# NSAPH-Projects/weather2alert

Hardware: AMD Instinct MI355X
Metric: env_steps_per_sec (higher is better)
Workload: dtype f32 tables, fp64 logit accumulation, f32 sigmoid/reward

## Files before the change

### include/w2a.h

```cpp
#ifndef W2A_H
#define W2A_H

#include <stddef.h>
#include <stdint.h>

#ifdef __cplusplus
extern "C" {
#endif

#define W2A_ABI_VERSION 18
#define W2A_ROW_FLOATS 32

enum {
  W2A_OK = 0,
  W2A_ERR_ARG = -1,
  W2A_ERR_SCHEMA = -2,
  W2A_ERR_HIP = -3,
  W2A_ERR_STATE = -4
};

enum {
  W2A_ST_BAD_EPISODE = 1,
  W2A_ST_BAD_ACTION = 2,
  W2A_ST_STEP_AFTER_DONE = 4,
// ... 88 lines not shown
typedef struct w2a_policy {
  int32_t kind;
  float p;
  int32_t obs_col;
  float threshold;
  int32_t obs_lag;
  int32_t require_budget;
  const uint8_t *table;
  int32_t table_R;
  uint64_t seed;
} w2a_policy;
int w2a_rollout(w2a_env *env, const w2a_policy *policy, int32_t n_steps, float *ret_out, int32_t *alerts_out,
                int32_t *attempts_over_budget, uint32_t *alert_mask, uint32_t *attempt_mask, int32_t mask_words,
                float *last_return, float *ret_snapshot, void *stream);
typedef struct w2a_linear_policy {
  const float *weight;
  const float *bias;
  const int32_t *group;
  int32_t n_groups;
  int32_t sample;
  int32_t require_budget;
  uint64_t seed;
} w2a_linear_policy;
int w2a_rollout_linear(w2a_env *env, const w2a_linear_policy *policy, int32_t n_steps, float *obs, float *ret_out,
                       int32_t *alerts_out, int32_t *attempts_over_budget, uint32_t *alert_mask, uint32_t *attempt_mask,
                       int32_t mask_words, float *last_return, float *ret_snapshot, void *stream);
enum { W2A_MLP_TANH = 0, W2A_MLP_RELU = 1 };
#define W2A_MLP_STRIDE(width, n_layers) \
  (W2A_ROW_FLOATS * (width) + (width) + ((n_layers) == 2 ? (width) * (width) + (width) : 0) + (width) + 4)
#define W2A_MLP_HEADS_STRIDE(width, n_layers) (W2A_MLP_STRIDE(width, n_layers) + (width))
typedef struct w2a_mlp_policy {
  const float *params;
  const int32_t *group;
  const int32_t *order;
  int32_t n_groups;
  int32_t n_layers;
  int32_t width;
  int32_t activation;
  int32_t sample;
  int32_t require_budget;
  uint64_t seed;
} w2a_mlp_policy;
int w2a_rollout_mlp(w2a_env *env, const w2a_mlp_policy *policy, int32_t n_steps, float *obs, float *ret_out,
                    int32_t *alerts_out, int32_t *attempts_over_budget, uint32_t *alert_mask, uint32_t *attempt_mask,
                    int32_t mask_words, float *last_return, float *ret_snapshot, void *stream);
enum { W2A_TRAJ_VALID = 1, W2A_TRAJ_TERMINATED = 2, W2A_TRAJ_ALERT = 4 };
typedef struct w2a_trajectory {
  float *obs;
  float *logit;
  float *reward;
  uint8_t *action;
  uint8_t *flags;
} w2a_trajectory;
int w2a_rollout_linear_record(w2a_env *env, const w2a_linear_policy *policy, int32_t n_steps, float *obs,
                              float *ret_out, int32_t *alerts_out, int32_t *attempts_over_budget, uint32_t *alert_mask,
                              uint32_t *attempt_mask, int32_t mask_words, float *last_return, float *ret_snapshot,
                              void *stream, const w2a_trajectory *traj);
int w2a_rollout_mlp_record(w2a_env *env, const w2a_mlp_policy *policy, int32_t n_steps, float *obs, float *ret_out,
                           int32_t *alerts_out, int32_t *attempts_over_budget, uint32_t *alert_mask,
                           uint32_t *attempt_mask, int32_t mask_words, float *last_return, float *ret_snapshot,
                           void *stream, const w2a_trajectory *traj);
int w2a_posterior_returns(w2a_env *env, const w2a_state_view *start, const uint32_t *alert_mask, int32_t mask_words,
                          int32_t n_steps, float *out, void *stream);
size_t w2a_hindsight_workspace_bytes(const w2a_env *env, int32_t n_steps, int32_t max_remaining, int32_t big_envs);
int w2a_hindsight_optimum(w2a_env *env, const w2a_state_view *start, int32_t n_steps, float *ret_out,
                          uint32_t *alert_mask, int32_t mask_words, int32_t *alerts_out, void *workspace,
                          size_t workspace_bytes, void *stream);
enum { W2A_PG_BASELINE_NONE = 0, W2A_PG_BASELINE_NO_ALERT = 1 };
size_t w2a_policy_gradient_workspace_bytes(int64_t num_envs, int32_t n_steps);
int w2a_policy_gradient_linear(w2a_env *env, const w2a_linear_policy *policy, int32_t baseline, int32_t n_steps,
                               const float *obs, float *grad, void *workspace, size_t workspace_bytes, void *stream);
size_t w2a_policy_gradient_mlp_workspace_bytes(int64_t num_envs, int32_t n_steps, int32_t n_groups, int32_t width,
                                               int32_t n_layers);
int w2a_policy_gradient_mlp(w2a_env *env, const w2a_mlp_policy *policy, int32_t baseline, int32_t n_steps,
                            const float *obs, float *grad, void *workspace, size_t workspace_bytes, void *stream);
int w2a_imitation_gradient_linear(w2a_env *env, const w2a_linear_policy *policy, const uint32_t *alert_mask,
                                  int32_t mask_words, const float *env_weight, int32_t n_steps, const float *obs,
                                  float *grad, float *loglik, int32_t *days, void *stream);
size_t w2a_imitation_gradient_mlp_workspace_bytes(int64_t num_envs, int32_t n_steps, int32_t n_groups, int32_t width,
                                                  int32_t n_layers);
int w2a_imitation_gradient_mlp(w2a_env *env, const w2a_mlp_policy *policy, const uint32_t *alert_mask,
                               int32_t mask_words, const float *env_weight, int32_t n_steps, const float *obs,
                               float *grad, float *loglik, int32_t *days, void *workspace, size_t workspace_bytes,
                               void *stream);
int w2a_imitation_gradient_linear_weighted(w2a_env *env, const w2a_linear_policy *policy, const uint32_t *alert_mask,
                                           int32_t mask_words, const float *env_weight, const float *day_weight,
                                           int32_t day_weight_days, int32_t n_steps, const float *obs, float *grad,
                                           float *loglik, int32_t *days, void *stream);
int w2a_imitation_gradient_mlp_weighted(w2a_env *env, const w2a_mlp_policy *policy, const uint32_t *alert_mask,
                                        int32_t mask_words, const float *env_weight, const float *day_weight,
                                        int32_t day_weight_days, int32_t n_steps, const float *obs, float *grad,
                                        float *loglik, int32_t *days, void *workspace, size_t workspace_bytes,
                                        void *stream);
int w2a_surrogate_gradient_linear(w2a_env *env, const w2a_linear_policy *policy, const uint32_t *alert_mask,
                                  int32_t mask_words, const float *env_weight, const float *advantage,
                                  int32_t advantage_days, const float *old_log_prob, int32_t old_log_prob_days,
                                  double clip, double entropy_coef, int32_t n_steps, const float *obs, float *grad,
                                  float *surrogate, int32_t *clipped_days, float *approx_kl, float *entropy,
                                  int32_t *days, float *log_prob, void *stream);
size_t w2a_surrogate_gradient_mlp_workspace_bytes(int64_t num_envs, int32_t n_steps, int32_t n_groups, int32_t width,
                                                  int32_t n_layers);
int w2a_surrogate_gradient_mlp(w2a_env *env, const w2a_mlp_policy *policy, const uint32_t *alert_mask,
                               int32_t mask_words, const float *env_weight, const float *advantage,
                               int32_t advantage_days, const float *old_log_prob, int32_t old_log_prob_days,
                               double clip, double entropy_coef, int32_t n_steps, const float *obs, float *grad,
                               float *surrogate, int32_t *clipped_days, float *approx_kl, float *entropy,
                               int32_t *days, float *log_prob, void *workspace, size_t workspace_bytes, void *stream);
size_t w2a_value_gradient_linear_workspace_bytes(int64_t num_envs, int32_t n_steps);
int w2a_value_gradient_linear(w2a_env *env, const w2a_linear_policy *value, const uint32_t *alert_mask,
                              int32_t mask_words, const float *env_weight, int32_t n_steps, const float *obs,
                              float *grad, float *sq_error, int32_t *days, float *ret, float *advantage,
                              void *workspace, size_t workspace_bytes, void *stream);
size_t w2a_value_gradient_mlp_workspace_bytes(int64_t num_envs, int32_t n_steps, int32_t n_groups, int32_t width,
                                              int32_t n_layers);
int w2a_value_gradient_mlp(w2a_env *env, const w2a_mlp_policy *value, const uint32_t *alert_mask, int32_t mask_words,
                           const float *env_weight, int32_t n_steps, const float *obs, float *grad, float *sq_error,
                           int32_t *days, float *ret, float *advantage, void *workspace, size_t workspace_bytes,
                           void *stream);
size_t w2a_value_gradient_linear_gae_workspace_bytes(int64_t num_envs, int32_t n_steps);
int w2a_value_gradient_linear_gae(w2a_env *env, const w2a_linear_policy *value, const uint32_t *alert_mask,
                                  int32_t mask_words, const float *env_weight, int32_t n_steps, const float *obs,
                                  float *grad, float *sq_error, int32_t *days, float *ret, float *advantage,
                                  double gamma, double lambda, int32_t bootstrap, float *value_target,
                                  const float *target, int32_t target_days, void *workspace, size_t workspace_bytes,
                                  void *stream);
size_t w2a_value_gradient_mlp_gae_workspace_bytes(int64_t num_envs, int32_t n_steps, int32_t n_groups, int32_t width,
                                                  int32_t n_layers);
int w2a_value_gradient_mlp_gae(w2a_env *env, const w2a_mlp_policy *value, const uint32_t *alert_mask,
                               int32_t mask_words, const float *env_weight, int32_t n_steps, const float *obs,
                               float *grad, float *sq_error, int32_t *days, float *ret, float *advantage, double gamma,
                               double lambda, int32_t bootstrap, float *value_target, const float *target,
                               int32_t target_days, void *workspace, size_t workspace_bytes, void *stream);
size_t w2a_rollout_order_workspace_bytes(int64_t num_envs, int64_t table_rows);
int w2a_rollout_order_attach(w2a_env *env, void *workspace, size_t workspace_bytes);
int w2a_rollout_order(w2a_env *env, void *workspace, size_t workspace_bytes, void *stream);

size_t w2a_rollout_mfma_workspace_bytes(int64_t num_envs, int64_t table_rows, int32_t S, int32_t n_samples);
int w2a_rollout_mfma_prepare(w2a_env *env, void *workspace, size_t workspace_bytes, void *stream);

int w2a_rollout_posterior_mean(w2a_env *env, const w2a_policy *policy, int32_t n_steps, float *ret_out,
                               int32_t *alerts_out, int32_t *attempts_over_budget, uint32_t *alert_mask,
                               uint32_t *attempt_mask, int32_t mask_words, float *last_return, float *ret_snapshot,
                               void *stream);

int w2a_policy_actions(w2a_env *env, const w2a_policy *policy, int32_t *actions, int32_t *alerts,
                       int32_t *attempts_over_budget, uint32_t *alert_mask, uint32_t *attempt_mask, int32_t mask_words,
                       void *stream);

int w2a_get_state(w2a_env *env, const w2a_state_view *view, void *stream);

enum { W2A_Q_LOCKSTEP = 6,
       W2A_Q_LOCKSTEP_DAY = 0, W2A_Q_PACKED_ELIGIBLE = 1, W2A_Q_PACKED_CURRENT = 2, W2A_Q_CANONICAL_CURRENT = 3,
       W2A_Q_LAST_ROLLOUT_KERNEL = 4 ,
       W2A_Q_LAST_STEP_KERNEL = 5     };
int w2a_query(w2a_env *env, int what);

int w2a_invalidate(w2a_env *env, void *stream);

int w2a_read_status(w2a_env *env, int32_t *status_out, void *stream);

int w2a_alert_gate(w2a_env *env, int32_t obs_col, float threshold, const float *thresholds, int32_t n_steps,
                   uint32_t *allowed_days, int32_t allowed_words, void *stream);
int w2a_rollout_linear_gated(w2a_env *env, const w2a_linear_policy *policy, int32_t n_steps, float *obs, float *ret_out,
                             int32_t *alerts_out, int32_t *attempts_over_budget, uint32_t *alert_mask,
                             uint32_t *attempt_mask, int32_t mask_words, float *last_return, float *ret_snapshot,
                             void *stream, const w2a_trajectory *traj, const uint32_t *allowed_days,
                             int32_t allowed_words);
int w2a_policy_gradient_linear_gated(w2a_env *env, const w2a_linear_policy *policy, int32_t baseline, int32_t n_steps,
                                     const float *obs, float *grad, void *workspace, size_t workspace_bytes,
                                     void *stream, const uint32_t *allowed_days, int32_t allowed_words);
int w2a_imitation_gradient_linear_gated(w2a_env *env, const w2a_linear_policy *policy, const uint32_t *alert_mask,
                                        int32_t mask_words, const float *env_weight, const float *day_weight,
                                        int32_t day_weight_days, int32_t n_steps, const float *obs, float *grad,
                                        float *loglik, int32_t *days, void *stream, const uint32_t *allowed_days,
                                        int32_t allowed_words);
int w2a_surrogate_gradient_linear_gated(w2a_env *env, const w2a_linear_policy *policy, const uint32_t *alert_mask,
                                        int32_t mask_words, const float *env_weight, const float *advantage,
                                        int32_t advantage_days, const float *old_log_prob, int32_t old_log_prob_days,
                                        double clip, double entropy_coef, int32_t n_steps, const float *obs,
                                        float *grad, float *surrogate, int32_t *clipped_days, float *approx_kl,
                                        float *entropy, int32_t *days, float *log_prob, void *stream,
                                        const uint32_t *allowed_days, int32_t allowed_words);
int w2a_rollout_mlp_gated(w2a_env *env, const w2a_mlp_policy *policy, int32_t n_steps, float *obs, float *ret_out,
                          int32_t *alerts_out, int32_t *attempts_over_budget, uint32_t *alert_mask,
                          uint32_t *attempt_mask, int32_t mask_words, float *last_return, float *ret_snapshot,
                          void *stream, const w2a_trajectory *traj, const uint32_t *allowed_days, int32_t allowed_words);
int w2a_policy_gradient_mlp_gated(w2a_env *env, const w2a_mlp_policy *policy, int32_t baseline, int32_t n_steps,
                                  const float *obs, float *grad, void *workspace, size_t workspace_bytes, void *stream,
                                  const uint32_t *allowed_days, int32_t allowed_words);
int w2a_imitation_gradient_mlp_gated(w2a_env *env, const w2a_mlp_policy *policy, const uint32_t *alert_mask,
                                     int32_t mask_words, const float *env_weight, const float *day_weight,
                                     int32_t day_weight_days, int32_t n_steps, const float *obs, float *grad,
                                     float *loglik, int32_t *days, void *workspace, size_t workspace_bytes,
                                     void *stream, const uint32_t *allowed_days, int32_t allowed_words);
int w2a_surrogate_gradient_mlp_gated(w2a_env *env, const w2a_mlp_policy *policy, const uint32_t *alert_mask,
                                     int32_t mask_words, const float *env_weight, const float *advantage,
                                     int32_t advantage_days, const float *old_log_prob, int32_t old_log_prob_days,
                                     double clip, double entropy_coef, int32_t n_steps, const float *obs, float *grad,
                                     float *surrogate, int32_t *clipped_days, float *approx_kl, float *entropy,
                                     int32_t *days, float *log_prob, void *workspace, size_t workspace_bytes,
                                     void *stream, const uint32_t *allowed_days, int32_t allowed_words);
int w2a_hindsight_optimum_gated(w2a_env *env, const w2a_state_view *start, int32_t n_steps, float *ret_out,
                                uint32_t *alert_mask, int32_t mask_words, int32_t *alerts_out, void *workspace,
                                size_t workspace_bytes, void *stream, const uint32_t *allowed_days,
                                int32_t allowed_words);

int w2a_fisher_vector_product_linear(w2a_env *env, const w2a_linear_policy *policy, const float *vec_weight,
                                     const float *vec_bias, const uint32_t *alert_mask, int32_t mask_words,
                                     const float *env_weight, int32_t n_steps, const float *obs, float *fv,
                                     float *quadratic, int32_t *days, void *stream, const uint32_t *allowed_days,
                                     int32_t allowed_words);
size_t w2a_fisher_vector_product_mlp_workspace_bytes(int64_t num_envs, int32_t n_steps, int32_t n_groups, int32_t width,
                                                     int32_t n_layers);
int w2a_fisher_vector_product_mlp(w2a_env *env, const w2a_mlp_policy *policy, const float *vector,
                                  const uint32_t *alert_mask, int32_t mask_words, const float *env_weight,
                                  int32_t n_steps, const float *obs, float *fv, float *quadratic, int32_t *days,
                                  void *workspace, size_t workspace_bytes, void *stream, const uint32_t *allowed_days,
                                  int32_t allowed_words);
enum { W2A_Q_LOSS_SQUARED = 0, W2A_Q_LOSS_HUBER = 1 };
size_t w2a_q_gradient_mlp_workspace_bytes(int64_t num_envs, int32_t n_steps, int32_t n_groups, int32_t width,
                                          int32_t n_layers);
int w2a_q_gradient_mlp(w2a_env *env, const w2a_mlp_policy *q, const w2a_mlp_policy *target_net,
                       const uint32_t *alert_mask, int32_t mask_words, const float *env_weight, int32_t n_steps,
                       const float *obs, float *grad, float *loss_out, int32_t *days, float *ret, double gamma,
                       int32_t double_q, int32_t loss, double huber_delta, int32_t bootstrap, float *td_error,
                       float *td_target, void *workspace, size_t workspace_bytes, void *stream);

#ifdef __cplusplus
}
#endif
#endif
```

### weather2alert_amd/_ffi.py

```python
from __future__ import annotations

import ctypes as C
import os

from . import build as _build

ROW_FLOATS = 32

OK = 0
ST_BAD_EPISODE, ST_BAD_ACTION, ST_STEP_AFTER_DONE, ST_STALE_GRAPH = 1, 2, 4, 8
ACT_I32, ACT_I64, ACT_U8 = 0, 1, 2
STEP_AUTORESET, STEP_NO_OBS, STEP_CLASSIC, STEP_REWARD_GIVEN, STEP_WIDE, STEP_SKIP_FINISHED, STEP_UNPACKED, STEP_NEXT_STEP, STEP_NO_CAPTURE = 1, 2, 8, 16, 32, 64, 128, 256, 512
S64_MIN_ENVS = 131072
ABI_VERSION = 18
FIX_BITS = {"alert_2wks": 1, "lag": 2, "penalty": 4, "obs": 8, "augment": 16}
BUDGET_FIXED, BUDGET_LESS_THAN, BUDGET_CENTERED = 0, 1, 2

SYMBOLS = [
    "w2a_abi_version", "w2a_last_error", "w2a_state_bytes", "w2a_create", "w2a_destroy", "w2a_reset",
    "w2a_reset_device_rng", "w2a_set_autoreset", "w2a_step", "w2a_get_state", "w2a_read_status",
    "w2a_sort_workspace_bytes", "w2a_sort_episodes", "w2a_reset_device_rng_sorted", "w2a_observe", "w2a_rollout", "w2a_rollout_order_workspace_bytes", "w2a_rollout_order_attach", "w2a_rollout_order", "w2a_rollout_posterior_mean", "w2a_policy_actions", "w2a_set_semantics",
    "w2a_group_workspace_bytes", "w2a_group_by_column", "w2a_posterior_mean_reward", "w2a_set_posterior_kernel", "w2a_invalidate", "w2a_query", "w2a_rollout_mfma_workspace_bytes", "w2a_rollout_mfma_prepare",
    "w2a_rollout_linear", "w2a_rollout_mlp", "w2a_rollout_linear_record", "w2a_rollout_mlp_record",
    "w2a_posterior_returns", "w2a_hindsight_workspace_bytes", "w2a_hindsight_optimum",
    "w2a_policy_gradient_workspace_bytes", "w2a_policy_gradient_linear",
    "w2a_policy_gradient_mlp_workspace_bytes", "w2a_policy_gradient_mlp",
    "w2a_imitation_gradient_linear", "w2a_imitation_gradient_mlp_workspace_bytes", "w2a_imitation_gradient_mlp",
    "w2a_imitation_gradient_linear_weighted", "w2a_imitation_gradient_mlp_weighted",
    "w2a_value_gradient_linear_workspace_bytes", "w2a_value_gradient_linear",
    "w2a_value_gradient_mlp_workspace_bytes", "w2a_value_gradient_mlp",
    "w2a_value_gradient_linear_gae_workspace_bytes", "w2a_value_gradient_linear_gae",
    "w2a_value_gradient_mlp_gae_workspace_bytes", "w2a_value_gradient_mlp_gae",
    "w2a_surrogate_gradient_linear", "w2a_surrogate_gradient_mlp_workspace_bytes", "w2a_surrogate_gradient_mlp",
    "w2a_alert_gate", "w2a_rollout_linear_gated", "w2a_policy_gradient_linear_gated",
    "w2a_imitation_gradient_linear_gated", "w2a_surrogate_gradient_linear_gated", "w2a_hindsight_optimum_gated",
    "w2a_rollout_mlp_gated", "w2a_policy_gradient_mlp_gated", "w2a_imitation_gradient_mlp_gated",
    "w2a_surrogate_gradient_mlp_gated",
    "w2a_fisher_vector_product_linear", "w2a_fisher_vector_product_mlp_workspace_bytes",
    "w2a_fisher_vector_product_mlp",
    "w2a_q_gradient_mlp_workspace_bytes", "w2a_q_gradient_mlp",
]
Q_LOCKSTEP_DAY, Q_PACKED_ELIGIBLE, Q_PACKED_CURRENT, Q_CANONICAL_CURRENT, Q_LAST_ROLLOUT_KERNEL, Q_LAST_STEP_KERNEL, Q_LOCKSTEP = 0, 1, 2, 3, 4, 5, 6
ROLLOUT_KERNELS = {0: "k_rollout", 1: "k_rollout64", 2: "k_rollout_mfma", 3: "k_rollout_linear", 4: "k_rollout_mlp"}
PM_KERNELS = {"vector": 0, "matrix": 1, "matrix_i8": 2}
POLICY_KINDS = {"never": 0, "always": 1, "bernoulli": 2, "threshold": 3, "table": 4}


class Policy(C.Structure):
    _fields_ = [("kind", C.c_int32), ("p", C.c_float), ("obs_col", C.c_int32), ("threshold", C.c_float),
                ("obs_lag", C.c_int32), ("require_budget", C.c_int32), ("table", C.c_void_p),
                ("table_R", C.c_int32), ("seed", C.c_uint64)]


class LinearPolicy(C.Structure):
    _fields_ = [("weight", C.c_void_p), ("bias", C.c_void_p), ("group", C.c_void_p), ("n_groups", C.c_int32),
                ("sample", C.c_int32), ("require_budget", C.c_int32), ("seed", C.c_uint64)]


class MlpPolicy(C.Structure):
    _fields_ = [("params", C.c_void_p), ("group", C.c_void_p), ("order", C.c_void_p), ("n_groups", C.c_int32),
                ("n_layers", C.c_int32), ("width", C.c_int32), ("activation", C.c_int32), ("sample", C.c_int32),
                ("require_budget", C.c_int32), ("seed", C.c_uint64)]


MLP_ACTIVATIONS = {"tanh": 0, "relu": 1}


class Trajectory(C.Structure):
    _fields_ = [("obs", C.c_void_p), ("logit", C.c_void_p), ("reward", C.c_void_p), ("action", C.c_void_p),
                ("flags", C.c_void_p)]


TRAJ_VALID, TRAJ_TERMINATED, TRAJ_ALERT = 1, 2, 4
Q_LOSSES = {"squared": 0, "huber": 1}
PG_BASELINES = {"none": 0, "no_alert": 1}


class Tables(C.Structure):
    _fields_ = [
        ("X", C.c_void_p), ("n_days", C.c_void_p), ("B0", C.c_void_p), ("W", C.c_void_p),
        ("fips_to_weather", C.c_void_p), ("sim_cnt", C.c_void_p),
        ("T", C.c_int32), ("S_w", C.c_int32), ("Y", C.c_int32), ("S", C.c_int32), ("n_samples", C.c_int32),
        ("n_obs", C.c_int32), ("obs_slot", C.c_int32 * ROW_FLOATS), ("slot_heat_qi", C.c_int32),
        ("sim_ptr", C.c_void_p), ("sim_idx", C.c_void_p), ("slot_alerts_2wks", C.c_int32),
        ("gate_bits", C.c_void_p), ("gate_words", C.c_int32),
    ]


STATE_FIELDS = ["t", "used", "streak", "hist14", "last_actual", "at_budget", "budget", "n_days", "county_w",
                "year_i", "coef_col", "sample", "sticky_budget", "episode_no", "finished", "episode_return"]


class StateView(C.Structure):
    _fields_ = [(k, C.c_void_p) for k in STATE_FIELDS]


class W2AError(RuntimeError):
    pass


_lib = None


def lib_path() -> str:
    return os.environ.get("W2A_LIB") or _build.LIB


def load(build_if_missing: bool = True):
    global _lib
    if _lib is not None:
        return _lib
    path = lib_path()
    if build_if_missing and not os.environ.get("W2A_LIB") and _build.needs_build():
        try:
            _build.build_lib()
        except Exception as e:
            raise W2AError(f"libw2a.so is out of date (or missing) and could not be rebuilt: {e}") from e
    if not os.path.exists(path):
        raise W2AError(f"{path} not found: run `python -m weather2alert_amd.build` (there is no CPU fallback)")
    lib = C.CDLL(path)
    vp, i32, i64, u64 = C.c_void_p, C.c_int32, C.c_int64, C.c_uint64
    lib.w2a_abi_version.restype = C.c_int
    lib.w2a_abi_version.argtypes = []
    lib.w2a_last_error.restype = C.c_char_p
    lib.w2a_last_error.argtypes = []
    lib.w2a_state_bytes.restype = C.c_size_t
    lib.w2a_state_bytes.argtypes = [i64]
    lib.w2a_create.restype = C.c_int
    lib.w2a_create.argtypes = [C.POINTER(Tables), i64, i64, vp, C.c_size_t, vp, C.POINTER(vp)]
    lib.w2a_destroy.restype = None
    lib.w2a_destroy.argtypes = [vp]
    lib.w2a_reset.restype = C.c_int
    lib.w2a_reset.argtypes = [vp, vp, vp, vp, vp, vp, vp, vp, vp]
    lib.w2a_reset_device_rng.restype = C.c_int
    lib.w2a_reset_device_rng.argtypes = [vp, u64, i32, C.c_int, i32, C.c_int, C.c_int, C.c_int, vp, vp, vp]
    lib.w2a_set_autoreset.restype = C.c_int
    lib.w2a_set_autoreset.argtypes = [vp, u64, i32, C.c_int, i32, C.c_int, C.c_int]
    lib.w2a_step.restype = C.c_int
    lib.w2a_step.argtypes = [vp, vp, C.c_int, vp, vp, vp, vp, C.c_int, vp]
    lib.w2a_get_state.restype = C.c_int
    lib.w2a_get_state.argtypes = [vp, C.POINTER(StateView), vp]
    lib.w2a_read_status.restype = C.c_int
    lib.w2a_read_status.argtypes = [vp, C.POINTER(i32), vp]
    lib.w2a_sort_workspace_bytes.restype = C.c_size_t
    lib.w2a_sort_workspace_bytes.argtypes = [i64]
    lib.w2a_sort_episodes.restype = C.c_int
    lib.w2a_sort_episodes.argtypes = [vp, vp, C.c_size_t, vp]
    lib.w2a_reset_device_rng_sorted.restype = C.c_int
    lib.w2a_reset_device_rng_sorted.argtypes = [vp, u64, i32, C.c_int, i32, C.c_int, C.c_int, C.c_int, vp, vp, C.c_size_t, vp]
    lib.w2a_group_workspace_bytes.restype = C.c_size_t
    lib.w2a_group_workspace_bytes.argtypes = [i64, C.c_int32, C.c_int32]
    lib.w2a_group_by_column.restype = C.c_int
    lib.w2a_group_by_column.argtypes = [vp, vp, C.c_size_t, vp]
    lib.w2a_posterior_mean_reward.restype = C.c_int
    lib.w2a_posterior_mean_reward.argtypes = [vp, vp, C.c_int, vp, vp]
    lib.w2a_set_posterior_kernel.restype = C.c_int
    lib.w2a_set_posterior_kernel.argtypes = [vp, C.c_int]
    lib.w2a_rollout_mfma_workspace_bytes.restype = C.c_size_t
    lib.w2a_rollout_mfma_workspace_bytes.argtypes = [i64, i64, i32, i32]
    lib.w2a_rollout_mfma_prepare.restype = C.c_int
    lib.w2a_rollout_mfma_prepare.argtypes = [vp, vp, C.c_size_t, vp]
    lib.w2a_query.restype = C.c_int
    lib.w2a_query.argtypes = [vp, C.c_int]
    lib.w2a_invalidate.restype = C.c_int
    lib.w2a_invalidate.argtypes = [vp, vp]
    lib.w2a_observe.restype = C.c_int
    lib.w2a_observe.argtypes = [vp, vp, vp]
    lib.w2a_set_semantics.restype = C.c_int
    lib.w2a_set_semantics.argtypes = [vp, C.c_uint32]
    lib.w2a_rollout.restype = C.c_int
    lib.w2a_rollout.argtypes = [vp, C.POINTER(Policy), i32, vp, vp, vp, vp, vp, i32, vp, vp, vp]
    lib.w2a_rollout_order_workspace_bytes.restype = C.c_size_t
    lib.w2a_rollout_order_workspace_bytes.argtypes = [i64, i64]
    lib.w2a_rollout_order.restype = C.c_int
    lib.w2a_rollout_order.argtypes = [vp, vp, C.c_size_t, vp]
    lib.w2a_rollout_order_attach.restype = C.c_int
    lib.w2a_rollout_order_attach.argtypes = [vp, vp, C.c_size_t]
    lib.w2a_rollout_posterior_mean.restype = C.c_int
    lib.w2a_rollout_posterior_mean.argtypes = [vp, C.POINTER(Policy), i32, vp, vp, vp, vp, vp, i32, vp, vp, vp]
    lib.w2a_rollout_linear.restype = C.c_int
    lib.w2a_rollout_linear.argtypes = [vp, C.POINTER(LinearPolicy), i32, vp, vp, vp, vp, vp, vp, i32, vp, vp, vp]
    lib.w2a_rollout_mlp.restype = C.c_int
    lib.w2a_rollout_mlp.argtypes = [vp, C.POINTER(MlpPolicy), i32, vp, vp, vp, vp, vp, vp, i32, vp, vp, vp]
    lib.w2a_rollout_linear_record.restype = C.c_int
    lib.w2a_rollout_linear_record.argtypes = lib.w2a_rollout_linear.argtypes + [C.POINTER(Trajectory)]
    lib.w2a_rollout_mlp_record.restype = C.c_int
    lib.w2a_rollout_mlp_record.argtypes = lib.w2a_rollout_mlp.argtypes + [C.POINTER(Trajectory)]
    lib.w2a_posterior_returns.restype = C.c_int
    lib.w2a_posterior_returns.argtypes = [vp, C.POINTER(StateView), vp, i32, i32, vp, vp]
    lib.w2a_hindsight_workspace_bytes.restype = C.c_size_t
    lib.w2a_hindsight_workspace_bytes.argtypes = [vp, i32, i32, i32]
    lib.w2a_hindsight_optimum.restype = C.c_int
    lib.w2a_hindsight_optimum.argtypes = [vp, C.POINTER(StateView), i32, vp, vp, i32, vp, vp, C.c_size_t, vp]
    lib.w2a_policy_gradient_workspace_bytes.restype = C.c_size_t
    lib.w2a_policy_gradient_workspace_bytes.argtypes = [i64, i32]
    lib.w2a_policy_gradient_linear.restype = C.c_int
    lib.w2a_policy_gradient_linear.argtypes = [vp, C.POINTER(LinearPolicy), i32, i32, vp, vp, vp, C.c_size_t, vp]
    lib.w2a_policy_gradient_mlp_workspace_bytes.restype = C.c_size_t
    lib.w2a_policy_gradient_mlp_workspace_bytes.argtypes = [i64, i32, i32, i32, i32]
    lib.w2a_policy_gradient_mlp.restype = C.c_int
    lib.w2a_policy_gradient_mlp.argtypes = [vp, C.POINTER(MlpPolicy), i32, i32, vp, vp, vp, C.c_size_t, vp]
    lib.w2a_imitation_gradient_linear.restype = C.c_int
    lib.w2a_imitation_gradient_linear.argtypes = [vp, C.POINTER(LinearPolicy), vp, i32, vp, i32, vp, vp, vp, vp, vp]
    lib.w2a_imitation_gradient_mlp_workspace_bytes.restype = C.c_size_t
    lib.w2a_imitation_gradient_mlp_workspace_bytes.argtypes = [i64, i32, i32, i32, i32]
    lib.w2a_imitation_gradient_mlp.restype = C.c_int
    lib.w2a_imitation_gradient_mlp.argtypes = [vp, C.POINTER(MlpPolicy), vp, i32, vp, i32, vp, vp, vp, vp, vp, C.c_size_t, vp]
    lib.w2a_imitation_gradient_linear_weighted.restype = C.c_int
    lib.w2a_imitation_gradient_linear_weighted.argtypes = [vp, C.POINTER(LinearPolicy), vp, i32, vp, vp, i32, i32, vp, vp, vp, vp, vp]
    lib.w2a_imitation_gradient_mlp_weighted.restype = C.c_int
    lib.w2a_imitation_gradient_mlp_weighted.argtypes = [vp, C.POINTER(MlpPolicy), vp, i32, vp, vp, i32, i32, vp, vp, vp, vp, vp, C.c_size_t, vp]
    lib.w2a_value_gradient_linear_workspace_bytes.restype = C.c_size_t
    lib.w2a_value_gradient_linear_workspace_bytes.argtypes = [i64, i32]
    lib.w2a_value_gradient_linear.restype = C.c_int
    lib.w2a_value_gradient_linear.argtypes = [vp, C.POINTER(LinearPolicy), vp, i32, vp, i32, vp, vp, vp, vp, vp, vp, vp, C.c_size_t, vp]
    lib.w2a_value_gradient_mlp_workspace_bytes.restype = C.c_size_t
    lib.w2a_value_gradient_mlp_workspace_bytes.argtypes = [i64, i32, i32, i32, i32]
    lib.w2a_value_gradient_mlp.restype = C.c_int
    lib.w2a_value_gradient_mlp.argtypes = [vp, C.POINTER(MlpPolicy), vp, i32, vp, i32, vp, vp, vp, vp, vp, vp, vp, C.c_size_t, vp]
    gae = [C.c_double, C.c_double, i32, vp, vp, i32]
    lib.w2a_value_gradient_linear_gae_workspace_bytes.restype = C.c_size_t
    lib.w2a_value_gradient_linear_gae_workspace_bytes.argtypes = [i64, i32]
    lib.w2a_value_gradient_linear_gae.restype = C.c_int
    lib.w2a_value_gradient_linear_gae.argtypes = [vp, C.POINTER(LinearPolicy), vp, i32, vp, i32, vp, vp, vp, vp, vp, vp, *gae, vp, C.c_size_t, vp]
    lib.w2a_value_gradient_mlp_gae_workspace_bytes.restype = C.c_size_t
    lib.w2a_value_gradient_mlp_gae_workspace_bytes.argtypes = [i64, i32, i32, i32, i32]
    lib.w2a_value_gradient_mlp_gae.restype = C.c_int
    lib.w2a_value_gradient_mlp_gae.argtypes = [vp, C.POINTER(MlpPolicy), vp, i32, vp, i32, vp, vp, vp, vp, vp, vp, *gae, vp, C.c_size_t, vp]
    lib.w2a_surrogate_gradient_linear.restype = C.c_int
    lib.w2a_surrogate_gradient_linear.argtypes = [vp, C.POINTER(LinearPolicy), vp, i32, vp, vp, i32, vp, i32, C.c_double,
                                                  C.c_double, i32, vp, vp, vp, vp, vp, vp, vp, vp, vp]
    lib.w2a_surrogate_gradient_mlp_workspace_bytes.restype = C.c_size_t
    lib.w2a_surrogate_gradient_mlp_workspace_bytes.argtypes = [i64, i32, i32, i32, i32]
    lib.w2a_surrogate_gradient_mlp.restype = C.c_int
    lib.w2a_surrogate_gradient_mlp.argtypes = [vp, C.POINTER(MlpPolicy), vp, i32, vp, vp, i32, vp, i32, C.c_double,
                                               C.c_double, i32, vp, vp, vp, vp, vp, vp, vp, vp, vp, C.c_size_t, vp]
    gate = [vp, i32]
    lib.w2a_alert_gate.restype = C.c_int
    lib.w2a_alert_gate.argtypes = [vp, i32, C.c_float, vp, i32, vp, i32, vp]
    lib.w2a_rollout_linear_gated.restype = C.c_int
    lib.w2a_rollout_linear_gated.argtypes = lib.w2a_rollout_linear.argtypes + [C.POINTER(Trajectory)] + gate
    lib.w2a_policy_gradient_linear_gated.restype = C.c_int
    lib.w2a_policy_gradient_linear_gated.argtypes = lib.w2a_policy_gradient_linear.argtypes + gate
    lib.w2a_imitation_gradient_linear_gated.restype = C.c_int
    lib.w2a_imitation_gradient_linear_gated.argtypes = lib.w2a_imitation_gradient_linear_weighted.argtypes + gate
    lib.w2a_surrogate_gradient_linear_gated.restype = C.c_int
    lib.w2a_surrogate_gradient_linear_gated.argtypes = lib.w2a_surrogate_gradient_linear.argtypes + gate
    lib.w2a_rollout_mlp_gated.restype = C.c_int
    lib.w2a_rollout_mlp_gated.argtypes = lib.w2a_rollout_mlp.argtypes + [C.POINTER(Trajectory)] + gate
    lib.w2a_policy_gradient_mlp_gated.restype = C.c_int
    lib.w2a_policy_gradient_mlp_gated.argtypes = lib.w2a_policy_gradient_mlp.argtypes + gate
    lib.w2a_imitation_gradient_mlp_gated.restype = C.c_int
    lib.w2a_imitation_gradient_mlp_gated.argtypes = lib.w2a_imitation_gradient_mlp_weighted.argtypes + gate
    lib.w2a_surrogate_gradient_mlp_gated.restype = C.c_int
    lib.w2a_surrogate_gradient_mlp_gated.argtypes = lib.w2a_surrogate_gradient_mlp.argtypes + gate
    lib.w2a_hindsight_optimum_gated.restype = C.c_int
    lib.w2a_hindsight_optimum_gated.argtypes = lib.w2a_hindsight_optimum.argtypes + gate
    lib.w2a_fisher_vector_product_linear.restype = C.c_int
    lib.w2a_fisher_vector_product_linear.argtypes = [vp, C.POINTER(LinearPolicy), vp, vp, vp, i32, vp, i32, vp, vp, vp,
                                                     vp, vp] + gate
    lib.w2a_fisher_vector_product_mlp_workspace_bytes.restype = C.c_size_t
    lib.w2a_fisher_vector_product_mlp_workspace_bytes.argtypes = [i64, i32, i32, i32, i32]
    lib.w2a_fisher_vector_product_mlp.restype = C.c_int
    lib.w2a_fisher_vector_product_mlp.argtypes = [vp, C.POINTER(MlpPolicy), vp, vp, i32, vp, i32, vp, vp, vp, vp, vp,
                                                  C.c_size_t, vp] + gate
    lib.w2a_q_gradient_mlp_workspace_bytes.restype = C.c_size_t
    lib.w2a_q_gradient_mlp_workspace_bytes.argtypes = [i64, i32, i32, i32, i32]
    lib.w2a_q_gradient_mlp.restype = C.c_int
    lib.w2a_q_gradient_mlp.argtypes = [vp, C.POINTER(MlpPolicy), C.POINTER(MlpPolicy), vp, i32, vp, i32, vp, vp, vp, vp,
                                       vp, C.c_double, i32, i32, C.c_double, i32, vp, vp, vp, C.c_size_t, vp]
    lib.w2a_policy_actions.restype = C.c_int
    lib.w2a_policy_actions.argtypes = [vp, C.POINTER(Policy), vp, vp, vp, vp, vp, i32, vp]
    if lib.w2a_abi_version() != ABI_VERSION:
        raise W2AError(f"libw2a.so ABI {lib.w2a_abi_version()} != {ABI_VERSION}; rebuild")
    _lib = lib
    return lib


def check(rc: int, what: str = ""):
    if rc != OK:
        msg = load().w2a_last_error().decode("utf-8", "replace")
        raise W2AError(f"{what} failed ({rc}): {msg}")
```

### weather2alert_amd/build.py

```python
from __future__ import annotations

import os
import shutil
import subprocess
import sys

PKG = os.path.dirname(os.path.abspath(__file__))
ROOT = os.path.dirname(PKG)
SRC = os.path.join(PKG, "csrc", "w2a_kernels.hip")
INC = os.path.join(ROOT, "include")
LIB_DIR = os.path.join(PKG, "_lib")
LIB = os.path.join(LIB_DIR, "libw2a.so")


def hipcc_path() -> str:
    for c in (os.environ.get("HIPCC"), shutil.which("hipcc"), "/opt/rocm/bin/hipcc"):
        if c and os.path.exists(c):
            return c
    raise RuntimeError("hipcc not found (need the ROCm toolchain to build libw2a.so)")


HASH_FILE = LIB + ".srchash"


def _dep_files() -> list:
    csrc = os.path.dirname(SRC)
    return sorted(os.path.join(csrc, f) for f in os.listdir(csrc) if f.endswith((".hip", ".hip.h", ".h"))) + \
        [os.path.join(INC, "w2a.h")]


def build_hash() -> str:
    import hashlib

    h = hashlib.sha256()
    for path in _dep_files():
        h.update(os.path.basename(path).encode())
        h.update(open(path, "rb").read())
    h.update(os.environ.get("W2A_CXXFLAGS", "").encode())
    return h.hexdigest()


def needs_build() -> bool:
    if not os.path.exists(LIB):
        return True
    if os.path.exists(HASH_FILE):
        try:
            return open(HASH_FILE).read().strip() != build_hash()
        except OSError:
            return True
    m = os.path.getmtime(LIB)
    return any(os.path.getmtime(d) > m for d in _dep_files())


STEP_SOURCES = ("w2a_common.hip.h", "w2a_step.hip.h", "w2a_step64.hip.h", "w2a_step_dispatch.hip.h", "w2a_bookkeeping.h")


def source_sha(files: tuple = STEP_SOURCES) -> str:
    import hashlib

    h = hashlib.sha256()
    csrc = os.path.dirname(SRC)
    for path in [os.path.join(csrc, f) for f in sorted(files)]:
        h.update(os.path.basename(path).encode())
        h.update(open(path, "rb").read())
    return h.hexdigest()[:16]


def build_lib(force: bool = False, verbose: bool = False) -> str:
    if not force and not needs_build():
        return LIB
    os.makedirs(LIB_DIR, exist_ok=True)
    tmp = f"{LIB}.{os.getpid()}.tmp"
    src_hash = build_hash()
    cmd = [hipcc_path(), "--offload-arch=gfx950", "-O3", "-std=c++17", "-fPIC", "-shared", f"-I{INC}", SRC,
           "-o", tmp]
    cmd += os.environ.get("W2A_CXXFLAGS", "").split()
    if verbose:
        cmd.insert(1, "-Rpass-analysis=kernel-resource-usage")
        print(" ".join(cmd))
    r = subprocess.run(cmd, capture_output=True, text=True)
    if r.returncode != 0:
        raise RuntimeError(f"hipcc failed ({r.returncode}):\n{r.stdout}\n{r.stderr}")
    if verbose:
        print(r.stderr)
    try:
        os.remove(HASH_FILE)
    except OSError:
        pass
    os.replace(tmp, LIB)
    htmp = f"{HASH_FILE}.{os.getpid()}.tmp"
    with open(htmp, "w") as f:
        f.write(src_hash + "\n")
    os.replace(htmp, HASH_FILE)
    return LIB


PROBE_SRC = os.path.join(ROOT, "tools", "fabric_probe.hip")
PROBE_LIB = os.path.join(LIB_DIR, "libw2a_probe.so")
PROBE_FLAGS = ("-DPROBE_LIB", "-DPROBE_F64", "-DPROBE_DEP", "-DPROBE_DAYS", "-DPROBE_RANDOM_DATA", "-DPROBE_INPLACE")


def build_probe_lib(force: bool = False, packed: bool = True) -> str:
    out = PROBE_LIB if packed else PROBE_LIB.replace(".so", "_unpacked.so")
    if not force and os.path.exists(out) and os.path.getmtime(out) >= os.path.getmtime(PROBE_SRC):
        return out
    os.makedirs(LIB_DIR, exist_ok=True)
    tmp = f"{out}.{os.getpid()}.tmp"
    cmd = [hipcc_path(), "--offload-arch=gfx950", "-O3", "-std=c++17", "-fPIC", "-shared", *PROBE_FLAGS,
           *(["-DPROBE_PACKED"] if packed else []), PROBE_SRC, "-o", tmp]
    r = subprocess.run(cmd, capture_output=True, text=True)
    if r.returncode != 0:
        raise RuntimeError(f"hipcc failed on the probe library ({r.returncode}):\n{r.stdout}\n{r.stderr}")
    os.replace(tmp, out)
    return out


if __name__ == "__main__":
    print(build_lib(force="--force" in sys.argv, verbose=True))
    print(build_probe_lib(force="--force" in sys.argv))
    print(build_probe_lib(force="--force" in sys.argv, packed=False))
```

### weather2alert_amd/csrc/w2a_common.hip.h

```cpp
#ifndef W2A_COMMON_HIP_H
#define W2A_COMMON_HIP_H

#include "w2a_bookkeeping.h"

#ifndef LANES
#define LANES 4
#endif
#define ROWF 32
#define QUADS (ROWF / 4 / LANES)
#ifndef BLOCK
#define BLOCK 256
#endif
#define ENVS_PER_BLOCK (BLOCK / LANES)
#define ENVS_PER_WAVE (64 / LANES)
#define HDR_BYTES 256
#ifndef W2A_NT_OBS
#define W2A_NT_OBS 1
#endif
#ifndef W2A_NT_W
#define W2A_NT_W 0
#endif
#ifndef W2A_XCD_SWIZZLE
#define W2A_XCD_SWIZZLE 1
#endif
__device__ __forceinline__ uint32_t logical_block(uint32_t b, uint32_t per_xcd) {
#if W2A_XCD_SWIZZLE
  return (b & 7u) * per_xcd + (b >> 3);
#else
  return b;
#endif
}
typedef float v4f __attribute__((ext_vector_type(4)));
typedef uint32_t v4u __attribute__((ext_vector_type(4)));
__device__ __forceinline__ float4 ld_w(const float4 *p) {
#if W2A_NT_W
  v4f v = __builtin_nontemporal_load(reinterpret_cast<const v4f *>(p));
  return make_float4(v.x, v.y, v.z, v.w);
#else
  return *p;
#endif
}
#define RT_QUAD 6
#define GATE_QUAD 7

struct u3 { uint32_t a, b, c; };
struct StateArrays {
  uint4 *cold;
  u3 *hot3;
  u3 *stepc;
  uint2 *pk_hot;
  uint2 *pk_c;
  uint32_t *pk_day;
};
#define W2A_PK_DAY_POISON 0xFFFFFFFFu
#define PK_BUDGET_ESCAPE 0xFFFFu
__device__ __forceinline__ uint32_t pk_budget16(uint32_t budget) { return budget < PK_BUDGET_ESCAPE ? budget : PK_BUDGET_ESCAPE; }
#define PK_USED(w) ((w) & 255u)
#define PK_STREAK(w) (((w) >> 8) & 255u)
#define PK_HIST(w) (((w) >> 16) & 0x3FFFu)
#define PK_FIN(w) (((w) >> 30) & 1u)
__device__ __forceinline__ uint32_t pk_pack_hot(uint32_t used, uint32_t streak, uint32_t hist, uint32_t fin) {
  return (used & 255u) | ((streak & 255u) << 8) | ((hist & 0x3FFFu) << 16) | (fin << 30);
}
__device__ __forceinline__ void load_step_state(const StateArrays &s, uint32_t e, uint4 &cold, uint4 &hot) {
  const u3 h = s.hot3[e];
  const u3 c = s.stepc[e];
  hot = make_uint4(h.a, h.b, h.c, c.a);
  cold = make_uint4(c.b, c.c, 0u, 0u);
}
__device__ __forceinline__ uint4 load_cold(const StateArrays &s, uint32_t e) { return s.cold[e]; }
__device__ __forceinline__ void store_hot(const StateArrays &s, uint32_t e, const uint4 hot) {
  u3 h; h.a = hot.x; h.b = hot.y; h.c = hot.z;
  s.hot3[e] = h;
}
__device__ __forceinline__ void store_episode(const StateArrays &s, uint32_t e, const uint4 cold, const uint4 hot) {
  s.cold[e] = cold;
  u3 c; c.a = hot.w; c.b = cold.x; c.c = cold.y;
  s.stepc[e] = c;
  store_hot(s, e, hot);
}
#define D0_T(d) ((d) & 1023u)
#define D0_USED(d) (((d) >> 10) & 1023u)
#define D0_STREAK(d) (((d) >> 20) & 1023u)
#define D0_LAST(d) (((d) >> 30) & 1u)
#define D0_ATB(d) (((d) >> 31) & 1u)
#define D1_HIST(d) ((d) & 0x3FFFu)
#define D1_NDAYS(d) (((d) >> 16) & 1023u)
#define D1_FIN(d) (((d) >> 31) & 1u)

__device__ __forceinline__ uint32_t pack_d0(uint32_t t, uint32_t used, uint32_t streak, uint32_t last, uint32_t atb) {
  return (t & 1023u) | ((used > 1023u ? 1023u : used) << 10) | ((streak > 1023u ? 1023u : streak) << 20) |
         (last << 30) | (atb << 31);
}
__device__ __forceinline__ uint32_t pack_d1(uint32_t hist, uint32_t ndays, uint32_t fin) {
  return (hist & 0x3FFFu) | ((ndays & 1023u) << 16) | (fin << 31);
}

struct DevTables {
  const float4 *X;
  const int32_t *n_days;
  const int32_t *B0;
  const float4 *W;
  const int32_t *fips_to_weather;
  const int32_t *sim_cnt;
  const uint32_t *gate_bits;
  int32_t gate_words;
  const int32_t *sim_ptr;
  const int32_t *sim_idx;
  int32_t T, S_w, Y, S, n_samples, n_obs;
  int32_t slot_hist2w;
  uint32_t fixes;
};
__device__ __forceinline__ void set_comp(float4 *x, int idx, float v) {
#pragma unroll
  for (int q = 0; q < QUADS; ++q) {
    if (idx == 4 * q) x[q].x = v;
    if (idx == 4 * q + 1) x[q].y = v;
    if (idx == 4 * q + 2) x[q].z = v;
    if (idx == 4 * q + 3) x[q].w = v;
  }
}
#define SAMPLE_BITS 12
#define PACK_W(coef_col, sample) (((uint32_t)(coef_col) << SAMPLE_BITS) | (uint32_t)(sample))
#define W_COL(y) ((y) >> SAMPLE_BITS)
#define W_SAMPLE(y) ((y) & ((1u << SAMPLE_BITS) - 1u))

struct ResetCfg {
  uint64_t seed;
  int32_t location;
  int32_t augment;
  int32_t budget_kw;
  int32_t sample_mode;
  int32_t sticky;
};

struct w2a_env {
  DevTables tb;
  int64_t n;
  int64_t gid0;
  const int32_t *slot_obs;
  StateArrays st;
  int32_t *status;
  ResetCfg autoreset;
  int has_autoreset;
  int32_t obs_slot_host[ROWF];
  const uint32_t *perm;
  uint4 *prep;
  const uint32_t *inv;
  const double *wd;
  const uint4 *tiles;
  const uint32_t *n_tiles;
  const uint4 *tiles_i8;
  const uint32_t *n_tiles_i8;
  const uint32_t *wq;
  const float *wscale;
  const uint32_t *colflag;
  const float *xs;
  const void *xmax_ws;
  void *order_ws;
  uint32_t *order_cnt, *order_rank, *order_start, *order_tile_start;
  const void *rm_ws;
  const uint4 *rm_tiles;
  const uint32_t *rm_n_tiles;
  const uint32_t *rm_wq;
  const float *rm_xs;
  const uint32_t *order;
  W2aBook bk;
  int pm_kernel;
  int w_tail_used;
  uint32_t s64_launches;
};

static thread_local char g_err[512] = "";
static int fail(int code, const char *fmt, const char *a = "") {
  snprintf(g_err, sizeof(g_err), fmt, a);
  return code;
}

__device__ __forceinline__ uint64_t w2a_mix64(uint64_t z) {
  z ^= z >> 30;
  z *= 0xBF58476D1CE4E5B9ull;
  z ^= z >> 27;
  z *= 0x94D049BB133111EBull;
  z ^= z >> 31;
  return z;
}
__device__ __forceinline__ uint64_t rng_stream(uint64_t seed, uint64_t gid, uint64_t episode) {
  uint64_t h = w2a_mix64(seed + 0x9E3779B97F4A7C15ull * (gid + 1));
  return w2a_mix64(h ^ (episode * 0xBF58476D1CE4E5B9ull + 0x94D049BB133111EBull));
}
__device__ __forceinline__ uint32_t rng_bounded(uint64_t stream, uint32_t slot, uint32_t n) {
  uint64_t u = w2a_mix64(stream + (uint64_t)(slot + 1) * 0x9E3779B97F4A7C15ull) >> 32;
  return (uint32_t)((u * (uint64_t)n) >> 32);
}

template <int CTRL>
__device__ __forceinline__ double dpp_f64(double v) {
  int lo = __double2loint(v), hi = __double2hiint(v);
  lo = __builtin_amdgcn_update_dpp(0, lo, CTRL, 0xF, 0xF, true);
  hi = __builtin_amdgcn_update_dpp(0, hi, CTRL, 0xF, 0xF, true);
  return __hiloint2double(hi, lo);
}
__device__ __forceinline__ double group_sum(double v) {
  if (LANES >= 2) v += dpp_f64<0xB1>(v);
  if (LANES >= 4) v += dpp_f64<0x4E>(v);
  if (LANES >= 8) v += dpp_f64<0x141>(v);
  return v;
}

__device__ __forceinline__ float sigmoid_f32(float z) {
  float e = __expf(-z);
  return __builtin_amdgcn_rcpf(1.0f + e);
}

__device__ __forceinline__ float reward_from_logits(double zb, double ze, uint32_t actual) {
  const float base = sigmoid_f32((float)zb);
  const float eff = sigmoid_f32((float)ze);
  return -(1000.0f / 152.0f) * base * (1.0f - eff * (float)actual);
}

struct Episode {
  uint32_t ep_row, ep_w, ndays;
  int32_t budget, sticky;
  uint32_t bad;
};

__device__ __forceinline__ Episode draw_episode(const DevTables &tb, const ResetCfg &rc, uint64_t gid,
                                                uint32_t episode_no, int32_t sticky_in) {
  Episode e;
  uint64_t st = rng_stream(rc.seed, gid, episode_no);
  uint32_t bad = 0;
  uint32_t county = rc.location < 0 ? rng_bounded(st, 0, (uint32_t)tb.S) : (uint32_t)rc.location;
  if (county >= (uint32_t)tb.S) { county = 0; bad = 1; }
  uint32_t coef_col = county;
  if (rc.augment) {
    int32_t ns = tb.sim_cnt[county];
    if (ns <= 0) { bad = 1; ns = 1; }
    coef_col = rng_bounded(st, 1, (uint32_t)ns);
    if ((tb.fixes & W2A_FIX_AUGMENT) && tb.sim_idx) {
      if (!bad) county = (uint32_t)tb.sim_idx[tb.sim_ptr[county] + (int32_t)coef_col];
      if (county >= (uint32_t)tb.S) { county = 0; bad = 1; }
      coef_col = county;
    }
  }
  uint32_t year_i = rng_bounded(st, 2, (uint32_t)tb.Y);
  uint32_t sample = rng_bounded(st, 3, (uint32_t)tb.n_samples);
  int32_t cw = tb.fips_to_weather[county];
  if (cw < 0) { cw = 0; bad = 1; }
  e.ep_row = (uint32_t)cw * (uint32_t)tb.Y + year_i;
  e.ep_w = PACK_W(coef_col, sample);
  int32_t nd = tb.n_days[e.ep_row];
  if (nd <= 0) { bad = 1; nd = 1; }
  e.ndays = (uint32_t)nd;
  int32_t b = (rc.sticky && sticky_in >= 0) ? sticky_in : (rc.budget_kw < 0 ? tb.B0[e.ep_row] : rc.budget_kw);
  if (b < 0) b = 0;
  if (rc.sample_mode == W2A_BUDGET_LESS_THAN) {
    b = (int32_t)rng_bounded(st, 4, (uint32_t)b + 1u);
  } else if (rc.sample_mode == W2A_BUDGET_CENTERED) {
    int32_t lo = (int32_t)(0.5 * (double)b), hi = (int32_t)(1.5 * (double)b + 1.0);
    b = lo + (int32_t)rng_bounded(st, 4, (uint32_t)(hi - lo));
  }
  e.budget = b;
  e.sticky = rc.sticky ? b : -1;
  e.bad = bad;
  return e;
}

__device__ __forceinline__ void store_obs_tile(void *__restrict__ obs_any, float *tile, int64_t wave_env0, int64_t n,
                                               int n_obs, int lane, int grp, const float4 *x, const int4 *so,
                                               bool write_me) {
  float *obs = reinterpret_cast<float *>(obs_any);
  const int base = grp * n_obs;
  const int trash = ENVS_PER_WAVE * n_obs + (lane & 15);
#pragma unroll
  for (int q = 0; q < QUADS; ++q) {
    tile[so[q].x >= 0 ? base + so[q].x : trash] = x[q].x;
    tile[so[q].y >= 0 ? base + so[q].y : trash] = x[q].y;
    tile[so[q].z >= 0 ? base + so[q].z : trash] = x[q].z;
    tile[so[q].w >= 0 ? base + so[q].w : trash] = x[q].w;
  }
  __builtin_amdgcn_fence(__ATOMIC_RELEASE, "wavefront");
  __builtin_amdgcn_wave_barrier();
  __builtin_amdgcn_fence(__ATOMIC_ACQUIRE, "wavefront");
  const bool full = (wave_env0 + ENVS_PER_WAVE <= n);
  const bool all_write = __all(write_me || (wave_env0 + grp >= n));
  float *dst = obs + wave_env0 * n_obs;
  if (full && all_write) {
    const int chunks = (ENVS_PER_WAVE * n_obs) >> 2;
#pragma unroll
    for (int c0 = 0; c0 < (ENVS_PER_WAVE * ROWF) / 4; c0 += 64) {
      const int c = c0 + lane;
      if (c < chunks) {
        v4f v = reinterpret_cast<const v4f *>(tile)[c];
#if W2A_NT_OBS
        __builtin_nontemporal_store(v, reinterpret_cast<v4f *>(dst) + c);
#else
        reinterpret_cast<v4f *>(dst)[c] = v;
#endif
      }
    }
  } else {
    const int total = ENVS_PER_WAVE * n_obs;
    const unsigned long long wm = __ballot(write_me);
    for (int i = lane; i < total; i += 64) {
      int g = i / n_obs;
      bool w = (wm >> (g * LANES)) & 1ull;
      if (w && wave_env0 + g < n) dst[i] = tile[i];
    }
  }
  __builtin_amdgcn_wave_barrier();
}

#endif
```

### weather2alert_amd/csrc/w2a_kernels.hip

```cpp

#include <hip/hip_runtime.h>
#include <hipcub/hipcub.hpp>
#include <math.h>
#include <stdint.h>
#include <stdio.h>
#include <string.h>
#include <type_traits>

#include "w2a.h"

#include "w2a_common.hip.h"
#include "w2a_step.hip.h"
#include "w2a_step64.hip.h"
#include "w2a_posterior.hip.h"
#include "w2a_posterior_i8.hip.h"
#include "w2a_reset.hip.h"
#include "w2a_rollout.hip.h"
#include "w2a_rollout_linear.hip.h"
#include "w2a_rollout_mlp.hip.h"
#include "w2a_rollout_i8.hip.h"
#include "w2a_rollout_mfma.hip.h"
#include "w2a_posterior_returns.hip.h"
#include "w2a_policy_gradient.hip.h"
#include "w2a_policy_gradient_mlp.hip.h"
#include "w2a_imitation.hip.h"
#include "w2a_surrogate.hip.h"
#include "w2a_fisher.hip.h"
#include "w2a_value.hip.h"
#include "w2a_gae.hip.h"
#include "w2a_qlearn.hip.h"
#include "w2a_hindsight.hip.h"
#include "w2a_gate.hip.h"
#include "w2a_sort.hip.h"

#define HIP_TRY(expr)                                                   \
  do {                                                                  \
    hipError_t _e = (expr);                                             \
    if (_e != hipSuccess) return fail(W2A_ERR_HIP, #expr ": %s", hipGetErrorString(_e)); \
  } while (0)

template <int KIND>
static void launch_pm_rollout_kind(bool masks, unsigned grid, hipStream_t s, const PmRolloutArgs &a) {
  if (masks) hipLaunchKernelGGL((k_pm_rollout<7, KIND, true>), dim3(grid), dim3(PMV_THREADS), 0, s, a);
  else hipLaunchKernelGGL((k_pm_rollout<7, KIND, false>), dim3(grid), dim3(PMV_THREADS), 0, s, a);
}
static void launch_pm_rollout(int kind, bool masks, unsigned grid, hipStream_t s, const PmRolloutArgs &a) {
  switch (kind) {
    case W2A_POLICY_ALWAYS: launch_pm_rollout_kind<W2A_POLICY_ALWAYS>(masks, grid, s, a); break;
    case W2A_POLICY_BERNOULLI: launch_pm_rollout_kind<W2A_POLICY_BERNOULLI>(masks, grid, s, a); break;
    case W2A_POLICY_THRESHOLD: launch_pm_rollout_kind<W2A_POLICY_THRESHOLD>(masks, grid, s, a); break;
    case W2A_POLICY_TABLE: launch_pm_rollout_kind<W2A_POLICY_TABLE>(masks, grid, s, a); break;
    default: launch_pm_rollout_kind<W2A_POLICY_NEVER>(masks, grid, s, a); break;
  }
}

#ifndef W2A_ROLLOUT_MFMA
#define W2A_ROLLOUT_MFMA 1
#endif
#ifndef W2A_ROLLOUT_WIDE
#define W2A_ROLLOUT_WIDE 1
#endif
template <int KIND>
static void launch_rollout_kind(bool masks, bool fixes, unsigned grid, hipStream_t s, const RolloutArgs &a) {
  if (W2A_ROLLOUT_WIDE && a.order) {
    const unsigned g64 = (unsigned)((((a.n + BLOCK - 1) / BLOCK) + 7) / 8 * 8);
    if (masks && fixes) hipLaunchKernelGGL((k_rollout64<KIND, true, true>), dim3(g64), dim3(BLOCK), 0, s, a);
    else if (masks) hipLaunchKernelGGL((k_rollout64<KIND, true, false>), dim3(g64), dim3(BLOCK), 0, s, a);
    else if (fixes) hipLaunchKernelGGL((k_rollout64<KIND, false, true>), dim3(g64), dim3(BLOCK), 0, s, a);
    else hipLaunchKernelGGL((k_rollout64<KIND, false, false>), dim3(g64), dim3(BLOCK), 0, s, a);
    return;
  }
  if (masks && fixes) hipLaunchKernelGGL((k_rollout<KIND, true, true>), dim3(grid), dim3(BLOCK), 0, s, a);
  else if (masks) hipLaunchKernelGGL((k_rollout<KIND, true, false>), dim3(grid), dim3(BLOCK), 0, s, a);
  else if (fixes) hipLaunchKernelGGL((k_rollout<KIND, false, true>), dim3(grid), dim3(BLOCK), 0, s, a);
  else hipLaunchKernelGGL((k_rollout<KIND, false, false>), dim3(grid), dim3(BLOCK), 0, s, a);
}
static void launch_rollout(int kind, bool masks, bool fixes, unsigned grid, hipStream_t s, const RolloutArgs &a) {
  switch (kind) {
    case W2A_POLICY_ALWAYS: launch_rollout_kind<W2A_POLICY_ALWAYS>(masks, fixes, grid, s, a); break;
    case W2A_POLICY_BERNOULLI: launch_rollout_kind<W2A_POLICY_BERNOULLI>(masks, fixes, grid, s, a); break;
    case W2A_POLICY_THRESHOLD: launch_rollout_kind<W2A_POLICY_THRESHOLD>(masks, fixes, grid, s, a); break;
    case W2A_POLICY_TABLE: launch_rollout_kind<W2A_POLICY_TABLE>(masks, fixes, grid, s, a); break;
    default: launch_rollout_kind<W2A_POLICY_NEVER>(masks, fixes, grid, s, a); break;
  }
}

template <int KIND>
static void launch_rollout_mfma_kind(bool masks, unsigned grid, hipStream_t s, const RmArgs &ra) {
  if (masks) hipLaunchKernelGGL((k_rollout_mfma<KIND, true>), dim3(grid), dim3(64 * RM_WAVES), 0, s, ra);
  else hipLaunchKernelGGL((k_rollout_mfma<KIND, false>), dim3(grid), dim3(64 * RM_WAVES), 0, s, ra);
}
static void launch_rollout_mfma(int kind, bool masks, unsigned grid, hipStream_t s, const RmArgs &ra) {
  switch (kind) {
    case W2A_POLICY_ALWAYS: launch_rollout_mfma_kind<W2A_POLICY_ALWAYS>(masks, grid, s, ra); break;
    case W2A_POLICY_BERNOULLI: launch_rollout_mfma_kind<W2A_POLICY_BERNOULLI>(masks, grid, s, ra); break;
    case W2A_POLICY_THRESHOLD: launch_rollout_mfma_kind<W2A_POLICY_THRESHOLD>(masks, grid, s, ra); break;
    case W2A_POLICY_TABLE: launch_rollout_mfma_kind<W2A_POLICY_TABLE>(masks, grid, s, ra); break;
    default: launch_rollout_mfma_kind<W2A_POLICY_NEVER>(masks, grid, s, ra); break;
  }
}

extern "C" {

int w2a_abi_version(void) { return W2A_ABI_VERSION; }
const char *w2a_last_error(void) { return g_err; }

static size_t align256(size_t x) { return (x + 255) & ~(size_t)255; }

size_t w2a_state_bytes(int64_t num_envs) {
  if (num_envs <= 0) return 0;
  const size_t n = (size_t)num_envs;
  return HDR_BYTES + align256(16 * n) + 2 * align256(12 * n) + 2 * align256(8 * n) + align256(4 * ((n + 63) / 64));
}

struct HipDev {
  w2a_env *env;
  hipStream_t s;
  void pack_state() {
    hipLaunchKernelGGL(k_pack_state, dim3((unsigned)((env->n + 255) / 256)), dim3(256), 0, s, env->st, env->n);
  }
  void unpack_state(int32_t n_days) {
    hipLaunchKernelGGL(k_unpack_state, dim3((unsigned)((env->n + 255) / 256)), dim3(256), 0, s, env->st, env->n, n_days);
  }
  void poison_mirror() {
    const int64_t tiles = (env->n + 63) / 64;
    hipLaunchKernelGGL(k_poison_mirror, dim3((unsigned)((tiles + 255) / 256)), dim3(256), 0, s, env->st, env->n);
  }
};
static void end_call(w2a_env *env, hipStream_t s) {
  HipDev d{env, s};
  bk_end_call(env->bk, d);
}
static bool stream_is_capturing(hipStream_t s) {
  hipStreamCaptureStatus cs = hipStreamCaptureStatusNone;
  if (s && hipStreamIsCapturing(s, &cs) == hipSuccess) return cs != hipStreamCaptureStatusNone;
  (void)hipGetLastError();
  return false;
}
#define REFUSE_WHILE_CAPTURING(who, stream)                                                                            \
  do {                                                                                                                 \
    if (stream_is_capturing((hipStream_t)(stream)))                                                                    \
      return fail(W2A_ERR_STATE, who ": the stream is recording a hipGraph; only w2a_step can be recorded (episode "    \
                                     "boundaries inside a graph: W2A_STEP_AUTORESET)");                                \
  } while (0)
static bool ensure_canonical(w2a_env *env, hipStream_t s, const char *who) {
  if (!env->bk.canon_valid && stream_is_capturing(s)) {
    fail(W2A_ERR_STATE, "%s: the state is in its packed lock-step form and a conversion cannot be recorded into a hipGraph", who);
    return false;
  }
  HipDev d{env, s};
  bk_ensure_canonical(env->bk, d);
  return true;
}
__global__ void k_table_scan(const int32_t *n_days, int32_t rows, int32_t *out) {
  const int i = blockIdx.x * blockDim.x + threadIdx.x;
  if (i >= rows) return;
  atomicMin(&out[0], n_days[i]);
  atomicMax(&out[1], n_days[i]);
}

int w2a_create(const w2a_tables *t, int64_t num_envs, int64_t env_gid0, void *state, size_t state_bytes,
               int32_t *status, w2a_env **out) {
  if (!t || !state || !status || !out) return fail(W2A_ERR_ARG, "w2a_create: NULL argument");
  if (num_envs <= 0 || env_gid0 < 0) return fail(W2A_ERR_ARG, "w2a_create: num_envs must be > 0 and env_gid0 >= 0");
  if (!t->X || !t->n_days || !t->B0 || !t->W || !t->fips_to_weather || !t->sim_cnt)
    return fail(W2A_ERR_ARG, "w2a_create: NULL table pointer");
  if (t->T <= 0 || t->T > 1023 || t->S_w <= 0 || t->Y <= 0 || t->S <= 0 || t->n_samples <= 0)
    return fail(W2A_ERR_SCHEMA, "w2a_create: table dims out of range (need 0 < T <= 1023, positive S_w, Y, S, n_samples)");
  if ((int64_t)t->S_w * t->Y > 0x7FFFFFFFll / 2 || (int64_t)t->S * t->n_samples > 0x7FFFFFFFll / 2 ||
      (int64_t)t->T * t->S_w * t->Y > 0x7FFFFFFFll)
    return fail(W2A_ERR_SCHEMA, "w2a_create: table too large for 32-bit row indices");
  if ((int64_t)t->T * t->S_w * t->Y * (ROWF / 4) > 0x7FFFFFFFll || (int64_t)t->S * t->n_samples * (2 * ROWF / 4) > 0x7FFFFFFFll ||
      num_envs > (1ll << 27))
    return fail(W2A_ERR_SCHEMA, "w2a_create: tables / env count exceed the 32-bit offset range of the kernels");
  if (t->n_samples > (1 << SAMPLE_BITS) || t->S >= (1 << (32 - SAMPLE_BITS)))
    return fail(W2A_ERR_SCHEMA, "w2a_create: need n_samples <= 4096 and S < 2^20");
  if (t->n_obs <= 0 || t->n_obs > W2A_ROW_FLOATS - 1)
    return fail(W2A_ERR_SCHEMA, "w2a_create: n_obs must be in 1..31 (the observation tile keeps one scratch column)");
  if (state_bytes < w2a_state_bytes(num_envs)) return fail(W2A_ERR_STATE, "w2a_create: state buffer too small");
  if (((uintptr_t)state & 255) || ((uintptr_t)t->X & 15) || ((uintptr_t)t->W & 15))
    return fail(W2A_ERR_STATE, "w2a_create: state must be 256-B aligned, X and W 16-B aligned");
  int32_t slot_obs[ROWF];
  for (int i = 0; i < ROWF; ++i) slot_obs[i] = -1;
  for (int j = 0; j < t->n_obs; ++j) {
    int s = t->obs_slot[j];
    if (s < 0 || s >= ROWF || slot_obs[s] != -1) return fail(W2A_ERR_SCHEMA, "w2a_create: obs_slot is not an injective map into 0..31");
    slot_obs[s] = j;
  }
  w2a_env *h = new w2a_env();
  h->tb.X = reinterpret_cast<const float4 *>(t->X);
  h->tb.n_days = t->n_days;
  h->tb.B0 = t->B0;
  h->tb.W = reinterpret_cast<const float4 *>(t->W);
  h->tb.fips_to_weather = t->fips_to_weather;
  h->tb.sim_cnt = t->sim_cnt;
  h->tb.sim_ptr = t->sim_ptr;
  h->tb.sim_idx = t->sim_idx;
  h->tb.slot_hist2w = t->slot_alerts_2wks;
  h->tb.gate_bits = t->gate_bits;
  h->tb.gate_words = t->gate_words;
  if (t->gate_bits && (int64_t)t->gate_words * 32 < (int64_t)t->S_w * t->Y) {
    delete h;
    return fail(W2A_ERR_SCHEMA, "w2a_create: gate_words * 32 must cover S_w * Y rows");
  }
  h->tb.fixes = 0;
  h->tb.T = t->T; h->tb.S_w = t->S_w; h->tb.Y = t->Y; h->tb.S = t->S; h->tb.n_samples = t->n_samples;
  h->tb.n_obs = t->n_obs;
  h->n = num_envs;
  h->gid0 = env_gid0;
  h->slot_obs = reinterpret_cast<const int32_t *>(state);
  h->st.cold = reinterpret_cast<uint4 *>((char *)state + HDR_BYTES);
  h->st.hot3 = reinterpret_cast<u3 *>((char *)h->st.cold + align256(16 * (size_t)num_envs));
  h->st.stepc = reinterpret_cast<u3 *>((char *)h->st.hot3 + align256(12 * (size_t)num_envs));
  h->st.pk_hot = reinterpret_cast<uint2 *>((char *)h->st.stepc + align256(12 * (size_t)num_envs));
  h->st.pk_c = reinterpret_cast<uint2 *>((char *)h->st.pk_hot + align256(8 * (size_t)num_envs));
  h->st.pk_day = reinterpret_cast<uint32_t *>((char *)h->st.pk_c + align256(8 * (size_t)num_envs));
  bk_init(h->bk, t->T <= 255 && t->S < 65536 && t->n_samples <= 1024 && (int64_t)t->S_w * t->Y < (1 << 22), -1);
  h->status = status;
  h->has_autoreset = 0;
  h->perm = nullptr;
  h->order = nullptr;
  h->prep = nullptr;
  h->pm_kernel = W2A_PM_VECTOR;
  h->xmax_ws = nullptr;
  h->order_ws = nullptr; h->order_cnt = h->order_rank = h->order_start = h->order_tile_start = nullptr; h->rm_ws = nullptr;
  for (int j = 0; j < ROWF; ++j) h->obs_slot_host[j] = j < t->n_obs ? t->obs_slot[j] : -1;
  hipError_t e1 = hipMemcpy(state, slot_obs, sizeof(slot_obs), hipMemcpyHostToDevice);
  hipError_t e2 = hipMemset(status, 0, sizeof(int32_t));
  if (e1 != hipSuccess || e2 != hipSuccess) { delete h; return fail(W2A_ERR_HIP, "w2a_create: header upload failed: %s", hipGetErrorString(e1 != hipSuccess ? e1 : e2)); }
  int64_t blocks = (num_envs + 255) / 256;
  hipLaunchKernelGGL(k_init_state, dim3((unsigned)blocks), dim3(256), 0, 0, h->st, num_envs);
  hipError_t e0 = hipGetLastError();
  if (e0 != hipSuccess) { delete h; return fail(W2A_ERR_HIP, "w2a_create: k_init_state launch failed: %s", hipGetErrorString(e0)); }
  int32_t *scan_flag = reinterpret_cast<int32_t *>(state) + ROWF;
  const int64_t w_rows = (int64_t)t->S * t->n_samples * 2;
  hipError_t e4 = hipMemset(scan_flag, 0, sizeof(int32_t));
  hipLaunchKernelGGL(k_scan_tail_slots, dim3((unsigned)((w_rows + 255) / 256)), dim3(256), 0, 0, h->tb.W, w_rows, scan_flag);
  hipError_t e3 = hipDeviceSynchronize();
  int32_t tail_used = 1;
  if (e3 == hipSuccess && e4 == hipSuccess) e3 = hipMemcpy(&tail_used, scan_flag, sizeof(int32_t), hipMemcpyDeviceToHost);
  if (e3 != hipSuccess || e4 != hipSuccess) { delete h; return fail(W2A_ERR_HIP, "w2a_create: init kernels failed: %s", hipGetErrorString(e3 != hipSuccess ? e3 : e4)); }
  h->w_tail_used = tail_used;
  {
    int32_t scan[2] = {0x7FFFFFFF, 0};
    int32_t *d_scan = reinterpret_cast<int32_t *>(state) + ROWF + 1;
    hipError_t e5 = hipMemcpy(d_scan, scan, sizeof(scan), hipMemcpyHostToDevice);
    const int32_t rows = t->S_w * t->Y;
    hipLaunchKernelGGL(k_table_scan, dim3((unsigned)((rows + 255) / 256)), dim3(256), 0, 0, t->n_days, rows, d_scan);
    if (e5 == hipSuccess) e5 = hipMemcpy(scan, d_scan, sizeof(scan), hipMemcpyDeviceToHost);
    if (e5 != hipSuccess) { delete h; return fail(W2A_ERR_HIP, "w2a_create: table scan failed: %s", hipGetErrorString(e5)); }
    h->bk.uni_nd = (scan[0] == scan[1] && scan[0] > 0) ? scan[0] : -1;
  }
  *out = h;
  return W2A_OK;
}

void w2a_destroy(w2a_env *env) { delete env; }

static unsigned grid_for(int64_t n) {
  int64_t tiles = (n + ENVS_PER_BLOCK - 1) / ENVS_PER_BLOCK;
  return (unsigned)(((tiles + 7) / 8) * 8);
}

static int launch_reset(w2a_env *env, ResetArgs &a, void *stream) {
  if (a.obs && ((uintptr_t)a.obs & 15)) return fail(W2A_ERR_ARG, "reset: obs must be 16-B aligned");
  REFUSE_WHILE_CAPTURING("reset / observe", stream);
  const W2aBook before = env->bk;
  {
    HipDev d{env, (hipStream_t)stream};
    bk_reset(env->bk, d, a.from_tuples == 2, a.mask != nullptr);
  }
  a.tb = env->tb; a.slot_obs = env->slot_obs; a.st = env->st;
  a.status = env->status; a.n = env->n; a.gid0 = env->gid0;
  hipError_t e = hipSuccess;
  if (env->bk.hist_valid && a.from_tuples != 2) {
    e = hipMemsetAsync(env->order_cnt, 0, 4 * (size_t)env->tb.S_w * env->tb.Y, (hipStream_t)stream);
    a.order_cnt = env->order_cnt; a.order_rank = env->order_rank;
  }
  if (e == hipSuccess) {
    hipLaunchKernelGGL(k_reset, dim3(grid_for(env->n)), dim3(BLOCK), 0, (hipStream_t)stream, a);
    e = hipGetLastError();
  }
  if (e != hipSuccess) {
    bk_reset_rollback(env->bk, before, a.from_tuples == 2, a.mask != nullptr);
    end_call(env, (hipStream_t)stream);
    return fail(W2A_ERR_HIP, "reset: launch failed: %s", hipGetErrorString(e));
  }
  end_call(env, (hipStream_t)stream);
  return W2A_OK;
}

int w2a_reset(w2a_env *env, const int32_t *county_w, const int32_t *year_i, const int32_t *coef_col,
              const int32_t *sample, const int32_t *budget, const uint8_t *mask, float *obs, void *stream) {
  if (!env || !county_w || !year_i || !coef_col || !sample) return fail(W2A_ERR_ARG, "w2a_reset: NULL argument");
  ResetArgs a;
  memset(&a, 0, sizeof(a));
  a.county_w = county_w; a.year_i = year_i; a.coef_col = coef_col; a.sample = sample; a.budget = budget;
  a.mask = mask; a.obs = obs; a.from_tuples = 1;
  return launch_reset(env, a, stream);
}

static int fill_cfg(const w2a_env *env, ResetCfg &rc, uint64_t seed, int32_t location, int augment, int32_t budget_kw,
                    int mode, int sticky) {
  if (location >= env->tb.S) return fail(W2A_ERR_ARG, "reset: location index outside fips_list");
  if (mode < W2A_BUDGET_FIXED || mode > W2A_BUDGET_CENTERED) return fail(W2A_ERR_ARG, "reset: bad sample_budget_mode");
  rc.seed = seed; rc.location = location; rc.augment = augment ? 1 : 0; rc.budget_kw = budget_kw;
  rc.sample_mode = mode; rc.sticky = sticky ? 1 : 0;
  return W2A_OK;
}

int w2a_reset_device_rng(w2a_env *env, uint64_t seed, int32_t location, int augment, int32_t budget_kw,
                         int sample_budget_mode, int sticky, int restart_episodes, const uint8_t *mask, float *obs,
                         void *stream) {
  if (!env) return fail(W2A_ERR_ARG, "w2a_reset_device_rng: NULL handle");
  ResetArgs a;
  memset(&a, 0, sizeof(a));
  int rc = fill_cfg(env, a.rc, seed, location, augment, budget_kw, sample_budget_mode, sticky);
  if (rc) return rc;
  a.mask = mask; a.obs = obs; a.from_tuples = 0; a.restart = restart_episodes ? 1 : 0;
  return launch_reset(env, a, stream);
}

int w2a_set_autoreset(w2a_env *env, uint64_t seed, int32_t location, int augment, int32_t budget_kw,
                      int sample_budget_mode, int sticky) {
  if (!env) return fail(W2A_ERR_ARG, "w2a_set_autoreset: NULL handle");
  int rc = fill_cfg(env, env->autoreset, seed, location, augment, budget_kw, sample_budget_mode, sticky);
  if (rc) return rc;
  env->has_autoreset = 1;
  return W2A_OK;
}

#include "w2a_step_dispatch.hip.h"

static size_t cub_sort_bytes(int64_t n) {
  size_t b = 0;
  (void)hipcub::DeviceRadixSort::SortPairs(nullptr, b, (const uint64_t *)nullptr, (uint64_t *)nullptr,
                                           (const uint32_t *)nullptr, (uint32_t *)nullptr, (int)n);
  return b;
}

using Sort32Config =
    rocprim::radix_sort_config<rocprim::default_config, rocprim::default_config,
                               rocprim::radix_sort_onesweep_config<rocprim::kernel_config<1024, 8>, rocprim::kernel_config<1024, 8>, 9,
                                                                   rocprim::block_radix_rank_algorithm::match>,
                               0>;
static hipError_t sort32_pairs(void *tmp, size_t &bytes, const uint32_t *k_in, uint32_t *k_out, const uint32_t *v_in,
                               uint32_t *v_out, size_t n, unsigned end_bit, hipStream_t s) {
  return rocprim::radix_sort_pairs<Sort32Config>(tmp, bytes, k_in, k_out, v_in, v_out, n, 0u, end_bit, s);
}
static size_t cub_sort32_bytes(int64_t n) {
  size_t b = 0;
  (void)sort32_pairs(nullptr, b, nullptr, nullptr, nullptr, nullptr, (size_t)n, 32u, nullptr);
  return b;
}
static size_t sorted_reset_bytes(int64_t num_envs) {
  const size_t n = (size_t)num_envs;
  return 4 * align256(4 * n) + align256(8 * n) + align256(cub_sort32_bytes(num_envs));
}

size_t w2a_sort_workspace_bytes(int64_t num_envs) {
  if (num_envs <= 0 || num_envs > (1ll << 27)) return 0;
  size_t n = (size_t)num_envs;
  const size_t relabel = align256(8 * n) * 2 + align256(4 * n) * 2 + align256(16 * n) + align256(12 * n) * 2 +
                         align256(cub_sort_bytes(num_envs));
  const size_t fused = sorted_reset_bytes(num_envs);
  return relabel > fused ? relabel : fused;
}

int w2a_sort_episodes(w2a_env *env, void *workspace, size_t workspace_bytes, void *stream) {
  if (!env || !workspace) return fail(W2A_ERR_ARG, "w2a_sort_episodes: NULL argument");
// ... 59 lines not shown
  hipStream_t s = (hipStream_t)stream;
  hipLaunchKernelGGL(k_reset_keys, dim3((unsigned)((n + 255) / 256)), dim3(256), 0, s, env->tb, a.rc, env->st, env->n, env->gid0,
                     restart_episodes ? 1 : 0, k_in, i_in, zw);
  HIP_TRY(hipGetLastError());
  HIP_TRY(sort32_pairs(p, cub_bytes, k_in, k_out, i_in, i_out, n, (unsigned)end_bit, s));
  const W2aBook before = env->bk;
  {
    HipDev d{env, s};
    bk_reset_sorted(env->bk, d);
  }
  a.obs = obs; a.from_tuples = 3; a.src_idx = i_out; a.src_zw = zw;
  a.tb = env->tb; a.slot_obs = env->slot_obs; a.st = env->st;
  a.status = env->status; a.n = env->n; a.gid0 = env->gid0;
  hipLaunchKernelGGL(k_reset, dim3(grid_for(env->n)), dim3(BLOCK), 0, s, a);
  const hipError_t e = hipGetLastError();
  if (e != hipSuccess) {
    bk_reset_rollback(env->bk, before, false, false);
    end_call(env, s);
    return fail(W2A_ERR_HIP, "w2a_reset_device_rng_sorted: launch failed: %s", hipGetErrorString(e));
  }
  end_call(env, s);
  return W2A_OK;
}

static size_t cub_group_bytes(int64_t n) { return cub_sort32_bytes(n); }

static size_t wd_bytes(int32_t S, int32_t n_samples) { return align256((size_t)S * n_samples * 2 * ROWF * sizeof(double)); }
static size_t max_tiles(int64_t n, int32_t S) { return (size_t)((n + PMV_THREADS - 1) / PMV_THREADS) + (size_t)S; }
static size_t tile_bytes(int64_t n, int32_t S) { return align256(16 * max_tiles(n, S)) + 2 * align256(4 * (size_t)S) + 256; }
static size_t max_tiles_i8(int64_t n, int32_t S) { return (size_t)((n + PI8_ROWS - 1) / PI8_ROWS) + (size_t)S; }
static size_t i8_bytes(int64_t n, int32_t S, int32_t n_samples) {
  const size_t rows = (size_t)S * n_samples * 2;
  return align256(16 * max_tiles_i8(n, S)) + 256 + align256(rows * ROWF * 4) + align256(rows * 4) + align256(4 * (size_t)S) + 3 * 256;
}

size_t w2a_group_workspace_bytes(int64_t num_envs, int32_t S, int32_t n_samples) {
  if (num_envs <= 0 || num_envs > (1ll << 27) || S <= 0 || n_samples <= 0) return 0;
  return align256(4 * (size_t)num_envs) * 4 + align256(16 * (size_t)num_envs) + wd_bytes(S, n_samples) +
         tile_bytes(num_envs, S) + i8_bytes(num_envs, S, n_samples) + align256(cub_group_bytes(num_envs));
}

int w2a_group_by_column(w2a_env *env, void *workspace, size_t workspace_bytes, void *stream) {
  if (!env || !workspace) return fail(W2A_ERR_ARG, "w2a_group_by_column: NULL argument");
  if (workspace_bytes < w2a_group_workspace_bytes(env->n, env->tb.S, env->tb.n_samples)) return fail(W2A_ERR_STATE, "w2a_group_by_column: workspace too small");
  if ((uintptr_t)workspace & 255) return fail(W2A_ERR_STATE, "w2a_group_by_column: workspace must be 256-B aligned");
  REFUSE_WHILE_CAPTURING("w2a_group_by_column", stream);
  const size_t n = (size_t)env->n;
  char *p = (char *)workspace;
  uint32_t *perm = (uint32_t *)p;  p += align256(4 * n);
  env->prep = (uint4 *)p;          p += align256(16 * n);
  double *wd = (double *)p;        p += wd_bytes(env->tb.S, env->tb.n_samples);
  uint4 *tiles = (uint4 *)p;       p += align256(16 * max_tiles(env->n, env->tb.S));
  uint32_t *col_start = (uint32_t *)p; p += align256(4 * (size_t)env->tb.S);
  uint32_t *col_end = (uint32_t *)p;   p += align256(4 * (size_t)env->tb.S);
  uint32_t *n_tiles = (uint32_t *)p;   p += 256;
  const size_t w_rows = (size_t)env->tb.S * env->tb.n_samples * 2;
  uint4 *tiles_i8 = (uint4 *)p;        p += align256(16 * max_tiles_i8(env->n, env->tb.S));
  uint32_t *n_tiles_i8 = (uint32_t *)p; p += 256;
  uint32_t *wq = (uint32_t *)p;        p += align256(w_rows * ROWF * 4);
  float *wscale = (float *)p;          p += align256(w_rows * 4);
  uint32_t *colflag = (uint32_t *)p;   p += align256(4 * (size_t)env->tb.S);
  uint32_t *xmax_bits = (uint32_t *)p; p += 256;
  uint32_t *bmax = (uint32_t *)p;      p += 256;
  float *xs = (float *)p;              p += 256;
  uint32_t *k_in = (uint32_t *)p;  p += align256(4 * n);
  uint32_t *k_out = (uint32_t *)p; p += align256(4 * n);
  uint32_t *i_in = (uint32_t *)p;  p += align256(4 * n);
  size_t cub_bytes = cub_group_bytes(env->n);
  hipStream_t s = (hipStream_t)stream;
  hipLaunchKernelGGL(k_group_keys, dim3((unsigned)((n + 255) / 256)), dim3(256), 0, s, env->st.stepc, k_in, i_in, env->n);
  HIP_TRY(hipGetLastError());
  int bits = 1;
  while ((1 << bits) < env->tb.S) ++bits;
  HIP_TRY(sort32_pairs(p, cub_bytes, k_in, k_out, i_in, perm, n, (unsigned)bits, s));
  HIP_TRY(hipMemsetAsync(col_start, 0, 2 * align256(4 * (size_t)env->tb.S), s));
  hipLaunchKernelGGL(k_tile_bounds, dim3((unsigned)((n + 255) / 256)), dim3(256), 0, s, k_out, col_start, col_end, env->n);
  HIP_TRY(hipGetLastError());
  hipLaunchKernelGGL(k_tile_list, dim3(1), dim3(1024), 0, s, col_start, col_end, env->tb.S, tiles, n_tiles, (uint32_t)PMV_THREADS);
  hipLaunchKernelGGL(k_tile_list, dim3(1), dim3(1024), 0, s, col_start, col_end, env->tb.S, tiles_i8, n_tiles_i8, (uint32_t)PI8_ROWS);
  HIP_TRY(hipGetLastError());
  env->tiles = tiles;
  env->n_tiles = n_tiles;
  if (env->xmax_ws != workspace) {
    HIP_TRY(hipMemsetAsync(xmax_bits, 0, 256, s));
    hipLaunchKernelGGL(k_pi8_slot_max, dim3(2048), dim3(256), 0, s, env->tb.X,
                       (int64_t)env->tb.T * env->tb.S_w * env->tb.Y * (ROWF / 4), xmax_bits);
    HIP_TRY(hipGetLastError());
    env->xmax_ws = workspace;
  }
  HIP_TRY(hipMemsetAsync(bmax, 0, 4, s));
  HIP_TRY(hipMemsetAsync(colflag, 0, 4 * (size_t)env->tb.S, s));
  hipLaunchKernelGGL(k_pi8_budget_max, dim3((unsigned)((n + 255) / 256)), dim3(256), 0, s, env->st.stepc, env->n, bmax);
  hipLaunchKernelGGL(k_pi8_scales, dim3(1), dim3(64), 0, s, xmax_bits, bmax, env->tb.T, xs);
  hipLaunchKernelGGL(k_pi8_wq, dim3((unsigned)((w_rows + 255) / 256)), dim3(256), 0, s,
                     reinterpret_cast<const float *>(env->tb.W), xs, (int64_t)w_rows, env->tb.n_samples, wq, wscale, colflag);
  HIP_TRY(hipGetLastError());
  env->tiles_i8 = tiles_i8; env->n_tiles_i8 = n_tiles_i8; env->wq = wq; env->wscale = wscale; env->colflag = colflag;
  env->xs = xs;
  const int64_t w_count = (int64_t)env->tb.S * env->tb.n_samples * 2 * ROWF;
  hipLaunchKernelGGL(k_pm_wd, dim3((unsigned)((w_count + 255) / 256)), dim3(256), 0, s,
                     reinterpret_cast<const float *>(env->tb.W), wd, w_count);
  HIP_TRY(hipGetLastError());
  env->wd = wd;
  hipLaunchKernelGGL(k_group_inverse, dim3((unsigned)((n + 255) / 256)), dim3(256), 0, s, perm, k_in, env->n);
  HIP_TRY(hipGetLastError());
  env->inv = k_in;
  env->perm = perm;
  bk_grouped(env->bk);
  return W2A_OK;
}

int w2a_posterior_mean_reward(w2a_env *env, const void *actions, int action_dtype, float *reward, void *stream) {
  if (!env || !actions || !reward) return fail(W2A_ERR_ARG, "w2a_posterior_mean_reward: NULL argument");
  if (action_dtype < W2A_ACT_I32 || action_dtype > W2A_ACT_U8) return fail(W2A_ERR_ARG, "w2a_posterior_mean_reward: bad action_dtype");
  if (!env->bk.perm_valid)
    return fail(W2A_ERR_STATE, "w2a_posterior_mean_reward: call w2a_group_by_column after every reset (the grouping of "
                               "envs by coefficient column is stale)");
  if (env->tb.fixes) return fail(W2A_ERR_ARG, "w2a_posterior_mean_reward: not available with corrected-semantics flags");
  PosteriorArgs a;
  memset(&a, 0, sizeof(a));
  a.tb = env->tb; a.st = env->st; a.inv = env->inv; a.perm = env->perm; a.prep = env->prep; a.actions = actions; a.act_dtype = action_dtype;
  a.reward = reward; a.status = env->status; a.n = env->n; a.wd = env->wd; a.tiles = env->tiles; a.n_tiles = env->n_tiles;
  if (!ensure_canonical(env, (hipStream_t)stream, "w2a_posterior_mean_reward")) return W2A_ERR_STATE;
  hipLaunchKernelGGL(k_pm_prep, dim3((unsigned)((env->n + 255) / 256)), dim3(256), 0, (hipStream_t)stream, a);
  HIP_TRY(hipGetLastError());
  if (env->pm_kernel == W2A_PM_MATRIX_I8) {
    PmI8Args b;
    b.p = a; b.tiles = env->tiles_i8; b.n_tiles = env->n_tiles_i8; b.wq = env->wq; b.wscale = env->wscale;
    b.colflag = env->colflag; b.xs = env->xs;
    const unsigned grid = (unsigned)((max_tiles_i8(env->n, env->tb.S) + 7) / 8 * 8);
    hipLaunchKernelGGL(k_posterior_mean_i8, dim3(grid), dim3(PI8_THREADS), 0, (hipStream_t)stream, b);
  } else if (env->pm_kernel == W2A_PM_MATRIX_F64) {
    const unsigned grid = (unsigned)((env->n + PM_ROWS - 1) / PM_ROWS);
    if (env->w_tail_used) hipLaunchKernelGGL(k_posterior_mean<8>, dim3(grid), dim3(BLOCK), 0, (hipStream_t)stream, a);
    else hipLaunchKernelGGL(k_posterior_mean<7>, dim3(grid), dim3(BLOCK), 0, (hipStream_t)stream, a);
  } else {
    const unsigned grid = (unsigned)((max_tiles(env->n, env->tb.S) + 7) / 8 * 8);
    if (env->w_tail_used) hipLaunchKernelGGL(k_posterior_mean_v<8>, dim3(grid), dim3(PMV_THREADS), 0, (hipStream_t)stream, a);
    else hipLaunchKernelGGL(k_posterior_mean_v<7>, dim3(grid), dim3(PMV_THREADS), 0, (hipStream_t)stream, a);
  }
  HIP_TRY(hipGetLastError());
  end_call(env, (hipStream_t)stream);
  return W2A_OK;
}

int w2a_set_posterior_kernel(w2a_env *env, int kernel) {
  if (!env) return fail(W2A_ERR_ARG, "w2a_set_posterior_kernel: NULL handle");
  if (kernel != W2A_PM_VECTOR && kernel != W2A_PM_MATRIX_F64 && kernel != W2A_PM_MATRIX_I8)
    return fail(W2A_ERR_ARG, "w2a_set_posterior_kernel: kernel must be W2A_PM_VECTOR, W2A_PM_MATRIX_F64 or W2A_PM_MATRIX_I8");
  env->pm_kernel = kernel;
  return W2A_OK;
}

int w2a_observe(w2a_env *env, float *obs, void *stream) {
  if (!env || !obs) return fail(W2A_ERR_ARG, "w2a_observe: NULL argument");
  ResetArgs a;
  memset(&a, 0, sizeof(a));
  a.obs = obs; a.from_tuples = 2;
  return launch_reset(env, a, stream);
}

int w2a_set_semantics(w2a_env *env, uint32_t fixes) {
  if (!env) return fail(W2A_ERR_ARG, "w2a_set_semantics: NULL handle");
  if (fixes & ~(uint32_t)W2A_FIX_ALL) return fail(W2A_ERR_ARG, "w2a_set_semantics: unknown W2A_FIX_* bit");
  if ((fixes & W2A_FIX_AUGMENT) && (!env->tb.sim_ptr || !env->tb.sim_idx))
    return fail(W2A_ERR_ARG, "w2a_set_semantics: W2A_FIX_AUGMENT needs sim_ptr/sim_idx in the tables");
  if ((fixes & W2A_FIX_ALERTS_2WKS) && env->tb.slot_hist2w >= W2A_ROW_FLOATS)
    return fail(W2A_ERR_SCHEMA, "w2a_set_semantics: slot_alerts_2wks out of range");
  env->tb.fixes = fixes;
  return W2A_OK;
}

size_t w2a_rollout_order_workspace_bytes(int64_t num_envs, int64_t table_rows) {
  if (num_envs <= 0 || num_envs > (1ll << 27) || table_rows <= 0 || table_rows > 0x7FFFFFFFll) return 0;
  return 2 * align256(4 * (size_t)num_envs) + align256(4 * (size_t)table_rows) + 2 * align256(4 * ((size_t)table_rows + 1));
}

static int order_attach(w2a_env *env, void *workspace, size_t workspace_bytes, const char *who) {
  const int64_t rows = (int64_t)env->tb.S_w * env->tb.Y;
  if (workspace_bytes < w2a_rollout_order_workspace_bytes(env->n, rows)) return fail(W2A_ERR_STATE, "%s: workspace too small", who);
  if ((uintptr_t)workspace & 255) return fail(W2A_ERR_STATE, "%s: workspace must be 256-B aligned", who);
  if (env->order_ws == workspace) return W2A_OK;
  const size_t n = (size_t)env->n;
  char *p = (char *)workspace;
  uint32_t *order = (uint32_t *)p;         p += align256(4 * n);
  env->order_rank = (uint32_t *)p;         p += align256(4 * n);
  env->order_cnt = (uint32_t *)p;          p += align256(4 * (size_t)rows);
  env->order_start = (uint32_t *)p;        p += align256(4 * ((size_t)rows + 1));
  env->order_tile_start = (uint32_t *)p;
  env->order_ws = workspace;
  const bool drops = env->order && env->order != order;
  if (drops) env->order = nullptr;
  bk_order_attach(env->bk, drops);
  return W2A_OK;
}

int w2a_rollout_order_attach(w2a_env *env, void *workspace, size_t workspace_bytes) {
  if (!env || !workspace) return fail(W2A_ERR_ARG, "w2a_rollout_order_attach: NULL argument");
  return order_attach(env, workspace, workspace_bytes, "w2a_rollout_order_attach");
}

int w2a_rollout_order(w2a_env *env, void *workspace, size_t workspace_bytes, void *stream) {
  if (!env || !workspace) return fail(W2A_ERR_ARG, "w2a_rollout_order: NULL argument");
  REFUSE_WHILE_CAPTURING("w2a_rollout_order", stream);
  const int rc = order_attach(env, workspace, workspace_bytes, "w2a_rollout_order");
  if (rc) return rc;
  const int64_t rows = (int64_t)env->tb.S_w * env->tb.Y;
  const size_t n = (size_t)env->n;
  uint32_t *order = (uint32_t *)workspace;
  hipStream_t s = (hipStream_t)stream;
  const unsigned blocks = (unsigned)((n + 255) / 256);
  if (!env->bk.hist_valid) {
    HIP_TRY(hipMemsetAsync(env->order_cnt, 0, 4 * (size_t)rows, s));
    hipLaunchKernelGGL(k_order_rank, dim3(blocks), dim3(256), 0, s, env->st.cold, env->order_cnt, env->order_rank, env->n);
  }
  hipLaunchKernelGGL(k_order_scan, dim3(1), dim3(1024), 0, s, env->order_cnt, (int32_t)rows, env->order_start, env->order_tile_start);
  hipLaunchKernelGGL(k_order_place, dim3(blocks), dim3(256), 0, s, env->st.cold, env->order_start, env->order_rank, order, env->n);
  HIP_TRY(hipGetLastError());
  env->order = order;
  bk_order_set(env->bk);
  return W2A_OK;
}

static size_t rm_max_tiles(int64_t n, int64_t rows) { return (size_t)((n + 15) / 16) + (size_t)rows; }
size_t w2a_rollout_mfma_workspace_bytes(int64_t num_envs, int64_t table_rows, int32_t S, int32_t n_samples) {
  if (num_envs <= 0 || num_envs > (1ll << 27) || table_rows <= 0 || table_rows > 0x7FFFFFFFll || S <= 0 || n_samples <= 0) return 0;
  const size_t w_rows = (size_t)S * n_samples * 2;
  return align256(16 * rm_max_tiles(num_envs, table_rows)) + 256 + align256(w_rows * ROWF * 4) + 3 * 256;
}

int w2a_rollout_mfma_prepare(w2a_env *env, void *workspace, size_t workspace_bytes, void *stream) {
  if (!env || !workspace) return fail(W2A_ERR_ARG, "w2a_rollout_mfma_prepare: NULL argument");
  REFUSE_WHILE_CAPTURING("w2a_rollout_mfma_prepare", stream);
  const int64_t rows = (int64_t)env->tb.S_w * env->tb.Y;
  if (workspace_bytes < w2a_rollout_mfma_workspace_bytes(env->n, rows, env->tb.S, env->tb.n_samples))
    return fail(W2A_ERR_STATE, "w2a_rollout_mfma_prepare: workspace too small");
  if ((uintptr_t)workspace & 255) return fail(W2A_ERR_STATE, "w2a_rollout_mfma_prepare: workspace must be 256-B aligned");
  if (!env->order || !env->order_start)
    return fail(W2A_ERR_STATE, "w2a_rollout_mfma_prepare: call w2a_rollout_order for this episode first");
  const size_t w_rows = (size_t)env->tb.S * env->tb.n_samples * 2;
  char *p = (char *)workspace;
  uint4 *tiles = (uint4 *)p;            p += align256(16 * rm_max_tiles(env->n, rows));
  uint32_t *n_tiles = (uint32_t *)p;    p += 256;
  uint32_t *wq = (uint32_t *)p;         p += align256(w_rows * ROWF * 4);
  uint32_t *xmax_bits = (uint32_t *)p;  p += 256;
  uint32_t *bmax = (uint32_t *)p;       p += 256;
  float *xs = (float *)p;               p += 256;
  hipStream_t s = (hipStream_t)stream;
  if (env->rm_ws != workspace) {
    HIP_TRY(hipMemsetAsync(xmax_bits, 0, 512, s));
    hipLaunchKernelGGL(k_pi8_slot_max, dim3(2048), dim3(256), 0, s, env->tb.X,
                       (int64_t)env->tb.T * env->tb.S_w * env->tb.Y * (ROWF / 4), xmax_bits);
    hipLaunchKernelGGL(k_pi8_scales, dim3(1), dim3(64), 0, s, xmax_bits, bmax, env->tb.T, xs);
    hipLaunchKernelGGL(k_rm_wq, dim3((unsigned)((w_rows + 255) / 256)), dim3(256), 0, s,
                       reinterpret_cast<const float *>(env->tb.W), xs, (int64_t)w_rows, wq);
    HIP_TRY(hipGetLastError());
    env->rm_ws = workspace;
  }
  hipLaunchKernelGGL(k_rm_tiles, dim3((unsigned)((rows + 255) / 256)), dim3(256), 0, s, env->order_start, env->order_tile_start,
                     (int32_t)rows, tiles, n_tiles);
  HIP_TRY(hipGetLastError());
  env->rm_tiles = tiles; env->rm_n_tiles = n_tiles; env->rm_wq = wq;
  env->rm_xs = xs;
  bk_rm_prepared(env->bk);
  return W2A_OK;
}

int w2a_rollout(w2a_env *env, const w2a_policy *policy, int32_t n_steps, float *ret_out, int32_t *alerts_out,
                int32_t *attempts_over_budget, uint32_t *alert_mask, uint32_t *attempt_mask, int32_t mask_words,
                float *last_return, float *ret_snapshot, void *stream) {
  if (!env || !policy) return fail(W2A_ERR_ARG, "w2a_rollout: NULL argument");
  if (n_steps <= 0) return fail(W2A_ERR_ARG, "w2a_rollout: n_steps must be positive");
  REFUSE_WHILE_CAPTURING("w2a_rollout", stream);
  if (policy->kind < W2A_POLICY_NEVER || policy->kind > W2A_POLICY_TABLE) return fail(W2A_ERR_ARG, "w2a_rollout: bad policy kind");
  if (policy->kind == W2A_POLICY_TABLE && (!policy->table || policy->table_R <= 0))
    return fail(W2A_ERR_ARG, "w2a_rollout: tabular policy needs table [T][table_R] and table_R > 0");
  if ((alert_mask || attempt_mask) && mask_words * 32 < env->tb.T)
    return fail(W2A_ERR_ARG, "w2a_rollout: alert_mask / attempt_mask need ceil(T/32) words per env");
  RolloutArgs a;
  memset(&a, 0, sizeof(a));
  a.tb = env->tb; a.st = env->st; a.status = env->status; a.n = env->n; a.gid0 = env->gid0;
  a.pol = *policy;
  a.pol_slot = 0;
  if (policy->kind == W2A_POLICY_THRESHOLD) {
    if (policy->obs_col < 0 || policy->obs_col >= env->tb.n_obs) return fail(W2A_ERR_ARG, "w2a_rollout: obs_col outside the observation");
    int slot = env->obs_slot_host[policy->obs_col];
    if (slot >= 24 && slot <= 27) return fail(W2A_ERR_ARG, "w2a_rollout: threshold policies read table-sourced columns only");
    a.pol_slot = slot;
  }
  a.n_steps = n_steps; a.ret_out = ret_out; a.alerts_out = alerts_out; a.attempts_over_budget = attempts_over_budget;
  a.alert_mask = alert_mask; a.attempt_mask = attempt_mask; a.mask_words = mask_words; a.last_return = last_return;
  a.ret_snapshot = ret_snapshot;
  a.order = env->order;
  hipStream_t s = (hipStream_t)stream;
  HipDev dv{env, s};
  const bool lock = bk_rollout_begin(env->bk, dv, n_steps);
  const int rkernel = bk_rollout_kernel(env->bk, lock, env->tb.fixes != 0, W2A_ROLLOUT_MFMA != 0, W2A_ROLLOUT_WIDE != 0);
  if (alert_mask) HIP_TRY(hipMemsetAsync(alert_mask, 0, (size_t)env->n * mask_words * sizeof(uint32_t), s));
  if (attempt_mask) HIP_TRY(hipMemsetAsync(attempt_mask, 0, (size_t)env->n * mask_words * sizeof(uint32_t), s));
  if (rkernel == W2A_BK_ROLLOUT_MFMA) {
    RmArgs ra;
    ra.r = a; ra.tiles = env->rm_tiles; ra.n_tiles = env->rm_n_tiles; ra.wq = env->rm_wq; ra.xs = env->rm_xs;
    const size_t wgs = ((rm_max_tiles(env->n, (int64_t)env->tb.S_w * env->tb.Y) + 3) / 4 + RM_WAVES - 1) / RM_WAVES;
    launch_rollout_mfma(policy->kind, alert_mask || attempt_mask || ret_snapshot, (unsigned)((wgs + 7) / 8 * 8), s, ra);
    HIP_TRY(hipGetLastError());
    end_call(env, s);
// ... 146 lines not shown
}

int w2a_hindsight_optimum(w2a_env *env, const w2a_state_view *start, int32_t n_steps, float *ret_out,
                          uint32_t *alert_mask, int32_t mask_words, int32_t *alerts_out, void *workspace,
                          size_t workspace_bytes, void *stream) {
  return hindsight_optimum("w2a_hindsight_optimum", env, start, n_steps, ret_out, alert_mask, mask_words, alerts_out, workspace, workspace_bytes,
                           stream, false, nullptr, 0);
}

int w2a_hindsight_optimum_gated(w2a_env *env, const w2a_state_view *start, int32_t n_steps, float *ret_out,
                                uint32_t *alert_mask, int32_t mask_words, int32_t *alerts_out, void *workspace,
                                size_t workspace_bytes, void *stream, const uint32_t *allowed_days,
                                int32_t allowed_words) {
  return hindsight_optimum("w2a_hindsight_optimum_gated", env, start, n_steps, ret_out, alert_mask, mask_words, alerts_out, workspace, workspace_bytes,
                           stream, true, allowed_days, allowed_words);
}

int w2a_alert_gate(w2a_env *env, int32_t obs_col, float threshold, const float *thresholds, int32_t n_steps,
                   uint32_t *allowed_days, int32_t allowed_words, void *stream) {
  if (!allowed_days) return fail(W2A_ERR_ARG, "w2a_alert_gate: NULL allowed_days");
  if (n_steps <= 0) return fail(W2A_ERR_ARG, "w2a_alert_gate: n_steps must be positive");
  if (!thresholds && threshold != threshold) return fail(W2A_ERR_ARG, "w2a_alert_gate: threshold is NaN");
  if (!env) return fail(W2A_ERR_ARG, "w2a_alert_gate: NULL handle");
  if (allowed_words <= 0 || (int64_t)allowed_words * 32 < env->tb.T)
    return fail(W2A_ERR_ARG, "w2a_alert_gate: allowed_days needs ceil(T/32) words per env");
  if (obs_col < 0 || obs_col >= env->tb.n_obs) return fail(W2A_ERR_ARG, "w2a_alert_gate: obs_col outside the observation");
  const int slot = env->obs_slot_host[obs_col];
  if (slot < 0 || slot >= ROWF) return fail(W2A_ERR_SCHEMA, "w2a_alert_gate: the column has no slot in the feature row");
  if (slot >= 24 && slot <= 27) return fail(W2A_ERR_ARG, "w2a_alert_gate: threshold policies read table-sourced columns only");
  if ((env->tb.fixes & W2A_FIX_ALERTS_2WKS) && slot == env->tb.slot_hist2w)
    return fail(W2A_ERR_ARG, "w2a_alert_gate: with W2A_FIX_ALERTS_2WKS this column holds the agent's own count: threshold "
                             "policies read table-sourced columns only");
  REFUSE_WHILE_CAPTURING("w2a_alert_gate", stream);
  GateArgs a;
  memset(&a, 0, sizeof(a));
  a.tb = env->tb; a.st = env->st; a.n = env->n;
  a.slot = slot;
  a.lag = (env->tb.fixes & W2A_FIX_OBS) ? 0 : 1;
  a.n_steps = n_steps; a.words = allowed_words;
  a.threshold = threshold; a.thresholds = thresholds; a.out = allowed_days;
  hipStream_t s = (hipStream_t)stream;
  if (!ensure_canonical(env, s, "w2a_alert_gate")) return W2A_ERR_STATE;
  hipLaunchKernelGGL(k_alert_gate, dim3((unsigned)((env->n + BLOCK - 1) / BLOCK)), dim3(BLOCK), 0, s, a);
  HIP_TRY(hipGetLastError());
  return W2A_OK;
}

int w2a_rollout_posterior_mean(w2a_env *env, const w2a_policy *policy, int32_t n_steps, float *ret_out,
                               int32_t *alerts_out, int32_t *attempts_over_budget, uint32_t *alert_mask,
                               uint32_t *attempt_mask, int32_t mask_words, float *last_return, float *ret_snapshot,
                               void *stream) {
  if (!env || !policy) return fail(W2A_ERR_ARG, "w2a_rollout_posterior_mean: NULL argument");
  if (n_steps <= 0) return fail(W2A_ERR_ARG, "w2a_rollout_posterior_mean: n_steps must be positive");
  REFUSE_WHILE_CAPTURING("w2a_rollout_posterior_mean", stream);
  if (policy->kind < W2A_POLICY_NEVER || policy->kind > W2A_POLICY_TABLE) return fail(W2A_ERR_ARG, "w2a_rollout_posterior_mean: bad policy kind");
  if (policy->kind == W2A_POLICY_TABLE && (!policy->table || policy->table_R <= 0))
    return fail(W2A_ERR_ARG, "w2a_rollout_posterior_mean: tabular policy needs table [T][table_R] and table_R > 0");
  if ((alert_mask || attempt_mask) && mask_words * 32 < env->tb.T)
    return fail(W2A_ERR_ARG, "w2a_rollout_posterior_mean: alert_mask / attempt_mask need ceil(T/32) words per env");
  if (!env->bk.perm_valid)
    return fail(W2A_ERR_STATE, "w2a_rollout_posterior_mean: call w2a_group_by_column after every reset");
  if (env->tb.fixes) return fail(W2A_ERR_ARG, "w2a_rollout_posterior_mean: not available with corrected-semantics flags");
  const bool i8 = env->pm_kernel == W2A_PM_MATRIX_I8;
  if (env->pm_kernel == W2A_PM_MATRIX_F64 || (i8 && env->tb.n_samples > PI8_NPAD) ||
      (!i8 && (env->tb.n_samples > W2A_PMV_NPAD || env->w_tail_used)))
    return 1;
  PmRolloutArgs pa;
  memset(&pa, 0, sizeof(pa));
  RolloutArgs &a = pa.r;
  a.tb = env->tb; a.st = env->st; a.status = env->status; a.n = env->n; a.gid0 = env->gid0;
  a.pol = *policy;
  if (policy->kind == W2A_POLICY_THRESHOLD) {
    if (policy->obs_col < 0 || policy->obs_col >= env->tb.n_obs) return fail(W2A_ERR_ARG, "w2a_rollout_posterior_mean: obs_col outside the observation");
    int slot = env->obs_slot_host[policy->obs_col];
    if (slot >= 24 && slot <= 27) return fail(W2A_ERR_ARG, "w2a_rollout_posterior_mean: threshold policies read table-sourced columns only");
    a.pol_slot = slot;
  }
  a.n_steps = n_steps; a.ret_out = ret_out; a.alerts_out = alerts_out; a.attempts_over_budget = attempts_over_budget;
  a.alert_mask = alert_mask; a.attempt_mask = attempt_mask; a.mask_words = mask_words; a.last_return = last_return;
  a.ret_snapshot = ret_snapshot;
  pa.perm = env->perm; pa.tiles = env->tiles; pa.n_tiles = env->n_tiles; pa.wd = env->wd;
  hipStream_t s = (hipStream_t)stream;
  {
    HipDev dv{env, s};
    (void)bk_rollout_begin(env->bk, dv, n_steps);
  }
  if (alert_mask) HIP_TRY(hipMemsetAsync(alert_mask, 0, (size_t)env->n * mask_words * sizeof(uint32_t), s));
  if (attempt_mask) HIP_TRY(hipMemsetAsync(attempt_mask, 0, (size_t)env->n * mask_words * sizeof(uint32_t), s));
  if (i8) {
    PmI8RolloutArgs ia;
    ia.r = a; ia.perm = env->perm; ia.tiles = env->tiles_i8; ia.n_tiles = env->n_tiles_i8; ia.wq = env->wq;
    ia.wscale = env->wscale; ia.colflag = env->colflag; ia.xs = env->xs;
    const unsigned grid8 = (unsigned)((max_tiles_i8(env->n, env->tb.S) + 7) / 8 * 8);
    hipLaunchKernelGGL(k_pm_rollout_i8, dim3(grid8), dim3(PI8_THREADS), 0, s, ia);
    HIP_TRY(hipGetLastError());
    end_call(env, s);
    return W2A_OK;
  }
  const unsigned grid = (unsigned)((max_tiles(env->n, env->tb.S) + 7) / 8 * 8);
  launch_pm_rollout(policy->kind, alert_mask || attempt_mask || ret_snapshot, grid, s, pa);
  HIP_TRY(hipGetLastError());
  end_call(env, s);
  return W2A_OK;
}

int w2a_policy_actions(w2a_env *env, const w2a_policy *policy, int32_t *actions, int32_t *alerts,
                       int32_t *attempts_over_budget, uint32_t *alert_mask, uint32_t *attempt_mask, int32_t mask_words,
                       void *stream) {
  if (!env || !policy || !actions) return fail(W2A_ERR_ARG, "w2a_policy_actions: NULL argument");
  if (policy->kind < W2A_POLICY_NEVER || policy->kind > W2A_POLICY_TABLE) return fail(W2A_ERR_ARG, "w2a_policy_actions: bad policy kind");
  if (policy->kind == W2A_POLICY_TABLE && (!policy->table || policy->table_R <= 0))
    return fail(W2A_ERR_ARG, "w2a_policy_actions: tabular policy needs table [T][table_R] and table_R > 0");
  if ((alert_mask || attempt_mask) && mask_words * 32 < env->tb.T)
    return fail(W2A_ERR_ARG, "w2a_policy_actions: alert_mask / attempt_mask need ceil(T/32) words per env");
  PolicyArgs a;
  memset(&a, 0, sizeof(a));
  a.tb = env->tb; a.st = env->st; a.n = env->n; a.gid0 = env->gid0;
  a.pol = *policy;
  if (policy->kind == W2A_POLICY_THRESHOLD) {
    if (policy->obs_col < 0 || policy->obs_col >= env->tb.n_obs) return fail(W2A_ERR_ARG, "w2a_policy_actions: obs_col outside the observation");
    int slot = env->obs_slot_host[policy->obs_col];
    if (slot >= 24 && slot <= 27) return fail(W2A_ERR_ARG, "w2a_policy_actions: threshold policies read table-sourced columns only");
    a.pol_slot = slot;
  }
  a.actions = actions; a.alerts = alerts; a.attempts_over_budget = attempts_over_budget;
  a.alert_mask = alert_mask; a.attempt_mask = attempt_mask; a.mask_words = mask_words;
  if (!ensure_canonical(env, (hipStream_t)stream, "w2a_policy_actions")) return W2A_ERR_STATE;
  hipLaunchKernelGGL(k_policy_actions, dim3((unsigned)((env->n + 255) / 256)), dim3(256), 0, (hipStream_t)stream, a);
  HIP_TRY(hipGetLastError());
  end_call(env, (hipStream_t)stream);
  return W2A_OK;
}

int w2a_get_state(w2a_env *env, const w2a_state_view *view, void *stream) {
  if (!env || !view) return fail(W2A_ERR_ARG, "w2a_get_state: NULL argument");
  int64_t blocks = (env->n + 255) / 256;
  if (!ensure_canonical(env, (hipStream_t)stream, "w2a_get_state")) return W2A_ERR_STATE;
  hipLaunchKernelGGL(k_get_state, dim3((unsigned)blocks), dim3(256), 0, (hipStream_t)stream, env->st, env->n, env->tb.Y, env->tb.n_samples, *view);
  HIP_TRY(hipGetLastError());
  end_call(env, (hipStream_t)stream);
  return W2A_OK;
}

int w2a_query(w2a_env *env, int what) {
  if (!env) return fail(W2A_ERR_ARG, "w2a_query: NULL handle");
  switch (what) {
    case W2A_Q_LOCKSTEP_DAY: return env->bk.uni_t;
    case W2A_Q_LOCKSTEP: return env->bk.lock;
    case W2A_Q_PACKED_ELIGIBLE: return bk_packed_eligible(env->bk) ? 1 : 0;
    case W2A_Q_PACKED_CURRENT: return env->bk.pk_valid;
    case W2A_Q_CANONICAL_CURRENT: return env->bk.canon_valid;
    case W2A_Q_LAST_ROLLOUT_KERNEL: return env->bk.last_rollout_kernel;
    case W2A_Q_LAST_STEP_KERNEL: return env->bk.last_step_kernel;
    default: return fail(W2A_ERR_ARG, "w2a_query: unknown item");
  }
}

int w2a_invalidate(w2a_env *env, void *stream) {
  if (!env) return fail(W2A_ERR_ARG, "w2a_invalidate: NULL handle");
  hipStream_t s = (hipStream_t)stream;
  REFUSE_WHILE_CAPTURING("w2a_invalidate", s);
  bk_invalidate(env->bk);
  end_call(env, s);
  return W2A_OK;
}

int w2a_read_status(w2a_env *env, int32_t *status_out, void *stream) {
  if (!env || !status_out) return fail(W2A_ERR_ARG, "w2a_read_status: NULL argument");
  hipStream_t s = (hipStream_t)stream;
  HIP_TRY(hipMemcpyAsync(status_out, env->status, sizeof(int32_t), hipMemcpyDeviceToHost, s));
  HIP_TRY(hipMemsetAsync(env->status, 0, sizeof(int32_t), s));
  HIP_TRY(hipStreamSynchronize(s));
  return W2A_OK;
}

}
```

### weather2alert_amd/csrc/w2a_step.hip.h

```cpp
#ifndef W2A_STEP_HIP_H
#define W2A_STEP_HIP_H

struct StepArgs {
  DevTables tb;
  const int32_t *slot_obs;
  StateArrays st;
  const void *actions;
  void *obs;
  float *reward;
  uint8_t *done;
  float *last_return;
  int32_t *status;
  int64_t n;
  int64_t gid0;
  ResetCfg rc;
  int32_t act_dtype;
  int32_t uni_nd;
  int32_t skip_finished;
  int32_t next_step;
  uint32_t walk_rev;
};

#ifndef W2A_MIN_WAVES
#define W2A_MIN_WAVES 7
#endif
__device__ __forceinline__ int32_t load_action_raw(const void *actions, int32_t dtype, uint32_t e) {
  if (dtype == W2A_ACT_I32) return reinterpret_cast<const int32_t *>(actions)[e];
  if (dtype == W2A_ACT_I64) return (int32_t) reinterpret_cast<const int64_t *>(actions)[e];
  return reinterpret_cast<const uint8_t *>(actions)[e];
}
__device__ __forceinline__ int32_t load_action(const StepArgs &a, uint32_t e) {
  return load_action_raw(a.actions, a.act_dtype, e);
}

template <bool AUTORESET, bool WRITE_OBS, bool FIXES>
__device__ __forceinline__ void step_tile(const StepArgs &a, float *s_tile_wave, int64_t wave_env0, int lane, int l,
                                          int grp, bool valid, uint32_t e, const uint4 cold, const uint4 hot,
                                          int32_t act) {
  uint32_t st_bits = 0;
  const bool restart_in = AUTORESET && a.next_step && D1_FIN(hot.y);
  if (restart_in) act = 0;
  if (act != 0 && act != 1) { st_bits |= W2A_ST_BAD_ACTION; act = 1; }

  const uint32_t t = D0_T(hot.x), used = D0_USED(hot.x), streak = D0_STREAK(hot.x);
  const uint32_t hist = D1_HIST(hot.y), ndays = D1_NDAYS(hot.y);
  const int32_t budget = (int32_t)hot.w;
  if (D1_FIN(hot.y) && !restart_in) st_bits |= W2A_ST_STEP_AFTER_DONE;

  const uint32_t atb = ((int32_t)used == budget) ? 1u : 0u;
  const uint32_t actual = (act == 1 && atb) ? 0u : (uint32_t)act;
  const uint32_t used2 = used + actual;
  const uint32_t hist2 = ((hist << 1) | actual) & 0x3FFFu;

  const uint32_t rows_per_day = (uint32_t)(a.tb.S_w * a.tb.Y);
  const uint32_t day_row = t * rows_per_day + cold.x;
  const uint32_t wrow = W_COL(cold.y) * (uint32_t)a.tb.n_samples + W_SAMPLE(cold.y);
  float4 x[QUADS];
  int4 so[QUADS];
#pragma unroll
  for (int q = 0; q < QUADS; ++q) {
    x[q] = make_float4(0.f, 0.f, 0.f, 0.f);
    x[q] = a.tb.X[day_row * (ROWF / 4) + l * QUADS + q];
    if (WRITE_OBS) so[q] = reinterpret_cast<const int4 *>(a.slot_obs)[l * QUADS + q];
  }
  const uint32_t fx = FIXES ? a.tb.fixes : 0u;
  const float f_lag1 = (t > 0) ? (float)((fx & W2A_FIX_LAG) ? D0_LAST(hot.x) : actual) : 0.0f;
  const float f_streak = (float)streak;
  const float f_rem = (float)(budget - (int32_t)used2);
  const float f_a2w = (float)__popc(hist2);
  if (l == RT_QUAD / QUADS) x[RT_QUAD % QUADS] = make_float4(f_lag1, f_streak, f_rem, f_a2w);
  if ((fx & W2A_FIX_ALERTS_2WKS) && a.tb.slot_hist2w >= 0 && l == a.tb.slot_hist2w / (4 * QUADS))
    set_comp(x, a.tb.slot_hist2w % (4 * QUADS), f_a2w);
  double zb, ze;
  {
    const float4 *wp = a.tb.W + wrow * (2 * ROWF / 4) + l * QUADS;
    float4 wb[QUADS], we[QUADS];
    const int eff_off = (actual != 0u) ? ROWF / 4 : 0;
#pragma unroll
    for (int q = 0; q < QUADS; ++q) {
      wb[q] = ld_w(wp + q);
      we[q] = ld_w(wp + eff_off + q);
    }
    zb = 0.0;
    ze = 0.0;
#pragma unroll
    for (int q = 0; q < QUADS; ++q) {
      const double x0 = (double)x[q].x, x1 = (double)x[q].y, x2 = (double)x[q].z, x3 = (double)x[q].w;
      zb = fma(x0, (double)wb[q].x, zb);
      zb = fma(x1, (double)wb[q].y, zb);
      zb = fma(x2, (double)wb[q].z, zb);
      zb = fma(x3, (double)wb[q].w, zb);
      ze = fma(x0, (double)we[q].x, ze);
      ze = fma(x1, (double)we[q].y, ze);
      ze = fma(x2, (double)we[q].z, ze);
      ze = fma(x3, (double)we[q].w, ze);
    }
    if (l == GATE_QUAD / QUADS && !(x[GATE_QUAD % QUADS].z > 0.5f)) ze = -__builtin_inf();
    zb = group_sum(zb);
    ze = group_sum(ze);
  }
  float r = reward_from_logits(zb, ze, actual);
  if ((fx & W2A_FIX_PENALTY) && act == 1 && atb) r = -1.0f;

  const bool done = (t + 1 >= ndays);
  const uint32_t t2 = done ? t : t + 1;
  const uint32_t streak2 = done ? streak : (actual ? streak + 1 : 0);
  const float ret = __uint_as_float(hot.z) + r;

  uint4 hot2 = make_uint4(pack_d0(t2, used2, streak2, actual, atb), pack_d1(hist2, ndays, done ? 1u : 0u),
                          __float_as_uint(ret), (uint32_t)budget);
  uint4 cold2 = cold;
  bool write_row = !done;
  if (WRITE_OBS && (fx & W2A_FIX_OBS)) {
    write_row = true;
    if (!done) {
#pragma unroll
      for (int q = 0; q < QUADS; ++q) x[q] = a.tb.X[(day_row + rows_per_day) * (ROWF / 4) + l * QUADS + q];
      if (l == RT_QUAD / QUADS) x[RT_QUAD % QUADS] = make_float4((float)actual, (float)streak2, f_rem, f_a2w);
      if ((fx & W2A_FIX_ALERTS_2WKS) && a.tb.slot_hist2w >= 0 && l == a.tb.slot_hist2w / (4 * QUADS))
        set_comp(x, a.tb.slot_hist2w % (4 * QUADS), f_a2w);
    }
  }
  if (AUTORESET) {
    if (a.next_step ? restart_in : done) {
      Episode ep = draw_episode(a.tb, a.rc, (uint64_t)(a.gid0 + e), cold.w + 1, (int32_t)cold.z);
      if (ep.bad) st_bits |= W2A_ST_BAD_EPISODE;
      cold2 = make_uint4(ep.ep_row, ep.ep_w, (uint32_t)ep.sticky, cold.w + 1);
      hot2 = make_uint4(pack_d0(0, 0, 0, 0, 0), pack_d1(0, ep.ndays, 0), __float_as_uint(0.0f), (uint32_t)ep.budget);
      if (WRITE_OBS) {
#pragma unroll
        for (int q = 0; q < QUADS; ++q) x[q] = a.tb.X[ep.ep_row * (ROWF / 4) + l * QUADS + q];
        if (l == RT_QUAD / QUADS) x[RT_QUAD % QUADS] = make_float4(0.0f, 0.0f, (float)ep.budget, 0.0f);
        if ((fx & W2A_FIX_ALERTS_2WKS) && a.tb.slot_hist2w >= 0 && l == a.tb.slot_hist2w / (4 * QUADS))
          set_comp(x, a.tb.slot_hist2w % (4 * QUADS), 0.0f);
      }
      write_row = true;
    }
  }
  if (valid && l == 0) {
    if (AUTORESET && (a.next_step ? restart_in : done)) store_episode(a.st, e, cold2, hot2);
    else store_hot(a.st, e, hot2);
    a.reward[e] = restart_in ? 0.0f : r;
    a.done[e] = (done && !restart_in) ? 1 : 0;
    if (done && !restart_in) {
      if (a.last_return) a.last_return[e] = ret;
    }
    if (st_bits) atomicOr(a.status, (int)st_bits);
  }
  if (WRITE_OBS) {
    store_obs_tile(a.obs, s_tile_wave, wave_env0, a.n, a.tb.n_obs, lane, grp, x, so, write_row);
  }
}

template <bool AUTORESET, bool WRITE_OBS, bool FIXES>
__global__ __launch_bounds__(BLOCK, (AUTORESET || FIXES) ? 1 : W2A_MIN_WAVES) void k_step(const StepArgs a) {
  __shared__ __attribute__((aligned(16))) float s_tile[BLOCK / 64][ENVS_PER_WAVE * ROWF];
  const int tid = threadIdx.x;
  const int lane = tid & 63;
  const int wave = __builtin_amdgcn_readfirstlane(tid >> 6);
  const int l = lane & (LANES - 1);
  const int grp = lane / LANES;
  const uint32_t lb = logical_block(blockIdx.x, gridDim.x >> 3);
  const int64_t wave_env0 = ((int64_t)lb * (BLOCK / 64) + wave) * ENVS_PER_WAVE;
  if (wave_env0 >= a.n) return;
  const int64_t env = wave_env0 + grp;
  const bool valid = env < a.n;
  const uint32_t e = (uint32_t)(valid ? env : (a.n - 1));
  uint4 cold, hot;
  load_step_state(a.st, e, cold, hot);
  if (AUTORESET) {
    const uint4 full = load_cold(a.st, e);
    cold.z = full.z;
    cold.w = full.w;
// ... 7 lines not shown
```

### weather2alert_amd/csrc/w2a_step64.hip.h

```cpp
#ifndef W2A_STEP64_HIP_H
#define W2A_STEP64_HIP_H

#ifndef W2A_S64_MIN_ENVS
#define W2A_S64_MIN_ENVS 131072
#endif
#define S64_ENVS 64
#define S64_WAVES (BLOCK / 64)
#define S64_PASS_ENVS 32
#define S64_ROUNDS 4

struct Day {
  uint32_t t, used, streak, hist, ndays, atb, actual, used2, hist2, st_bits, last;
  int32_t budget, act;
  bool done;
};
__device__ __forceinline__ Day derive_day(const u3 h, const u3 c, int32_t act) {
  Day d;
  d.st_bits = 0;
  if (act != 0 && act != 1) { d.st_bits |= W2A_ST_BAD_ACTION; act = 1; }
  d.act = act;
  d.last = D0_LAST(h.a);
  d.t = D0_T(h.a); d.used = D0_USED(h.a); d.streak = D0_STREAK(h.a);
  d.hist = D1_HIST(h.b); d.ndays = D1_NDAYS(h.b);
  d.budget = (int32_t)c.a;
  if (D1_FIN(h.b)) d.st_bits |= W2A_ST_STEP_AFTER_DONE;
  d.atb = ((int32_t)d.used == d.budget) ? 1u : 0u;
  d.actual = (act == 1 && d.atb) ? 0u : (uint32_t)act;
  d.used2 = d.used + d.actual;
  d.hist2 = ((d.hist << 1) | d.actual) & 0x3FFFu;
  d.done = (d.t + 1 >= d.ndays);
  return d;
}
__device__ __forceinline__ float4 runtime_fields(const Day &d, bool fix_lag = false) {
  return make_float4((d.t > 0) ? (float)(fix_lag ? d.last : d.actual) : 0.0f, (float)d.streak,
                     (float)(d.budget - (int32_t)d.used2), (float)__popc(d.hist2));
}
__device__ __forceinline__ void set_comp4(float4 &x, int idx, float v) {
  if (idx == 0) x.x = v;
  if (idx == 1) x.y = v;
  if (idx == 2) x.z = v;
  if (idx == 3) x.w = v;
}

template <bool FIXES>
struct S64WaveT {
  uint2 desc[S64_ENVS];
  float4 rt[S64_ENVS];
  float4 rt2[FIXES ? S64_ENVS : 1];
  float2 z[S64_ENVS];
  float tile[S64_PASS_ENVS * ROWF];
};

#ifndef W2A_S64_SC1
#define W2A_S64_SC1 0
#endif
#ifndef W2A_S64_SKIP_EFF
#define W2A_S64_SKIP_EFF 1
#endif
#ifndef W2A_S64_NT_STATE
#define W2A_S64_NT_STATE 0
#endif
typedef uint32_t v3u __attribute__((ext_vector_type(3)));
__device__ __forceinline__ void st16_sc1(void *p, v4f v) {
  asm volatile("global_store_dwordx4 %0, %1, off sc1" ::"v"(p), "v"(v) : "memory");
}
__device__ __forceinline__ void st12_sc1(void *p, v3u v) {
  asm volatile("global_store_dwordx3 %0, %1, off sc1" ::"v"(p), "v"(v) : "memory");
}
typedef uint32_t v2u __attribute__((ext_vector_type(2)));
__device__ __forceinline__ void st8_sc1(void *p, v2u v) {
  asm volatile("global_store_dwordx2 %0, %1, off sc1" ::"v"(p), "v"(v) : "memory");
}
__device__ __forceinline__ void st4_sc1(void *p, uint32_t v) {
  asm volatile("global_store_dword %0, %1, off sc1" ::"v"(p), "v"(v) : "memory");
}
__device__ __forceinline__ void st1_sc1(void *p, uint32_t v) {
  asm volatile("global_store_byte %0, %1, off sc1" ::"v"(p), "v"(v) : "memory");
}

#ifndef W2A_S64_MIN_WAVES
#define W2A_S64_MIN_WAVES 4
#endif
#ifndef W2A_S64_PRIO
#define W2A_S64_PRIO 3
#endif
#ifndef W2A_S64_TILES
#define W2A_S64_TILES 1
#endif
#ifndef W2A_S64_SERPENTINE
#define W2A_S64_SERPENTINE 1
#endif
__device__ __forceinline__ uint32_t logical_block_rev(uint32_t b, uint32_t per_xcd) {
#if W2A_XCD_SWIZZLE
  return (b & 7u) * per_xcd + (per_xcd - 1u - (b >> 3));
#else
  return 8u * per_xcd - 1u - b;
#endif
}
template <bool WRITE_OBS, bool REWARD_GIVEN, bool PACKED, bool AUTORESET = false, bool FIXES = false>
__device__ __forceinline__ void s64_tile(const StepArgs &a, S64WaveT<FIXES> &sw, const int lane, const int64_t wave_env0,
                                         const bool valid, const uint32_t e, const u3 h, const u3 c, const int32_t act,
                                         const int4 so) {
  const Day d = derive_day(h, c, act);
  const uint32_t t = d.t, used2 = d.used2, hist2 = d.hist2, streak = d.streak, ndays = d.ndays;
  const uint32_t actual = d.actual, atb = d.atb, st_bits = d.st_bits;
  const int32_t budget = d.budget;
  const bool done = d.done;
  const bool restart_in = AUTORESET && a.next_step && D1_FIN(h.b);
  const uint32_t fx = FIXES ? a.tb.fixes : 0u;
  const bool fix_obs = FIXES && WRITE_OBS && (fx & W2A_FIX_OBS);
  uint32_t need_eff = actual;
  if (a.tb.gate_bits && actual)
    need_eff = (a.tb.gate_bits[t * (uint32_t)a.tb.gate_words + (c.b >> 5)] >> (c.b & 31u)) & 1u;
  {
    const uint32_t day_row = t * (uint32_t)(a.tb.S_w * a.tb.Y) + c.b;
    const uint32_t wrow = W_COL(c.c) * (uint32_t)a.tb.n_samples + W_SAMPLE(c.c);
    sw.desc[lane] = make_uint2((day_row * (ROWF / 4)) | ((fix_obs && !done) ? 0x80000000u : 0u),
                               (wrow * (2 * ROWF / 4)) | (need_eff << 31));
    sw.rt[lane] = runtime_fields(d, (fx & W2A_FIX_LAG) != 0u);
    if (fix_obs)
      sw.rt2[FIXES ? lane : 0] = make_float4((float)actual, (float)(actual ? streak + 1 : 0), (float)(budget - (int32_t)used2),
                                 (float)__popc(hist2));
  }
  __builtin_amdgcn_fence(__ATOMIC_RELEASE, "wavefront");
  __builtin_amdgcn_wave_barrier();
  __builtin_amdgcn_fence(__ATOMIC_ACQUIRE, "wavefront");

  const int p = lane & 7;
  const int g = lane >> 3;
  const int n_obs = a.tb.n_obs;
  const bool write_me = valid && (!done || fix_obs) && !restart_in;
  const uint32_t next_day = (uint32_t)(a.tb.S_w * a.tb.Y) * (ROWF / 4);
#pragma unroll 1
  for (int pass = 0; pass < S64_ENVS / S64_PASS_ENVS; ++pass) {
    if (REWARD_GIVEN && !WRITE_OBS) break;
    if (wave_env0 + pass * S64_PASS_ENVS >= a.n) break;
    float4 x[S64_ROUNDS], wb[S64_ROUNDS], we[S64_ROUNDS], xo[FIXES ? S64_ROUNDS : 1];
    bool need[S64_ROUNDS], nxt[S64_ROUNDS];
#pragma unroll
    for (int r = 0; r < S64_ROUNDS; ++r) {
      uint2 ds = sw.desc[pass * S64_PASS_ENVS + r * 8 + g];
      need[r] = (ds.y >> 31) != 0u;
      nxt[r] = FIXES && (ds.x >> 31) != 0u;
      if (FIXES) ds.x &= 0x7FFFFFFFu;
      const uint32_t wq = ds.y & 0x7FFFFFFFu;
      x[r] = a.tb.X[ds.x + p];
      if (fix_obs) xo[r] = a.tb.X[ds.x + (nxt[r] ? next_day : 0u) + p];
      wb[r] = we[r] = make_float4(0.f, 0.f, 0.f, 0.f);
      if (!REWARD_GIVEN) {
        wb[r] = a.tb.W[wq + p];
        we[r] = a.tb.W[wq + (need[r] ? ROWF / 4 : 0) + p];
      }
    }
#if W2A_S64_PRIO
    __builtin_amdgcn_s_setprio(W2A_S64_PRIO);
#endif
#pragma unroll
    for (int r = 0; r < S64_ROUNDS; ++r) {
      const int j = pass * S64_PASS_ENVS + r * 8 + g;
      if (p == RT_QUAD) x[r] = sw.rt[j];
      if (FIXES && (fx & W2A_FIX_ALERTS_2WKS) && a.tb.slot_hist2w >= 0) {
        const float a2w = sw.rt[j].w;
        if (p == (a.tb.slot_hist2w >> 2)) set_comp4(x[r], a.tb.slot_hist2w & 3, a2w);
        if (fix_obs && p == (a.tb.slot_hist2w >> 2)) set_comp4(xo[r], a.tb.slot_hist2w & 3, a2w);
      }
      if (fix_obs && p == RT_QUAD) xo[r] = nxt[r] ? sw.rt2[FIXES ? j : 0] : sw.rt[j];
      if (!REWARD_GIVEN) {
      const double x0 = (double)x[r].x, x1 = (double)x[r].y, x2 = (double)x[r].z, x3 = (double)x[r].w;
      double zb = x0 * (double)wb[r].x;
      zb = fma(x1, (double)wb[r].y, zb);
      zb = fma(x2, (double)wb[r].z, zb);
      zb = fma(x3, (double)wb[r].w, zb);
      zb += dpp_f64<0xB1>(zb);
      zb += dpp_f64<0x4E>(zb);
      zb += dpp_f64<0x141>(zb);
      double ze = 0.0;
#if W2A_S64_SKIP_EFF
      if (__any(need[r]))
#endif
      {
        ze = x0 * (double)we[r].x;
        ze = fma(x1, (double)we[r].y, ze);
        ze = fma(x2, (double)we[r].z, ze);
        ze = fma(x3, (double)we[r].w, ze);
        if (p == GATE_QUAD && !(x[r].z > 0.5f)) ze = -__builtin_inf();
        ze += dpp_f64<0xB1>(ze);
        ze += dpp_f64<0x4E>(ze);
        ze += dpp_f64<0x141>(ze);
      }
      if (p == 0) sw.z[j] = make_float2((float)zb, (float)ze);
      }
      if (WRITE_OBS) {
        const int base = (r * 8 + g) * n_obs;
        const int trash = S64_PASS_ENVS * n_obs + (lane & 31);
        const float4 ov = fix_obs ? xo[FIXES ? r : 0] : x[r];
        sw.tile[so.x >= 0 ? base + so.x : trash] = ov.x;
        sw.tile[so.y >= 0 ? base + so.y : trash] = ov.y;
        sw.tile[so.z >= 0 ? base + so.z : trash] = ov.z;
        sw.tile[so.w >= 0 ? base + so.w : trash] = ov.w;
      }
    }
    if (WRITE_OBS) {
      __builtin_amdgcn_fence(__ATOMIC_RELEASE, "wavefront");
      __builtin_amdgcn_wave_barrier();
      __builtin_amdgcn_fence(__ATOMIC_ACQUIRE, "wavefront");
      const int64_t env0 = wave_env0 + pass * S64_PASS_ENVS;
      float *dst = reinterpret_cast<float *>(a.obs) + env0 * n_obs;
      const unsigned long long wm_all = __ballot(write_me);
      const uint32_t wm = (uint32_t)(wm_all >> (pass * S64_PASS_ENVS));
      const bool full = env0 + S64_PASS_ENVS <= a.n;
      if (full && wm == 0xFFFFFFFFu) {
        const int chunks = (S64_PASS_ENVS * n_obs) >> 2;
#pragma unroll
        for (int c0 = 0; c0 < (S64_PASS_ENVS * ROWF) / 4; c0 += 64) {
          const int ch = c0 + lane;
          if (ch < chunks) {
            const v4f v = reinterpret_cast<const v4f *>(sw.tile)[ch];
#if W2A_S64_SC1 & 1
            st16_sc1(reinterpret_cast<v4f *>(dst) + ch, v);
#elif W2A_NT_OBS
            __builtin_nontemporal_store(v, reinterpret_cast<v4f *>(dst) + ch);
#else
            reinterpret_cast<v4f *>(dst)[ch] = v;
#endif
          }
        }
      } else if (wm != 0u) {
        const int total = S64_PASS_ENVS * n_obs;
        for (int i = lane; i < total; i += 64) {
          const int jj = i / n_obs;
          if ((wm >> jj) & 1u) dst[i] = sw.tile[i];
        }
      }
      __builtin_amdgcn_fence(__ATOMIC_RELEASE, "wavefront");
      __builtin_amdgcn_wave_barrier();
      __builtin_amdgcn_fence(__ATOMIC_ACQUIRE, "wavefront");
    }
  }
  if (!WRITE_OBS) {
    __builtin_amdgcn_fence(__ATOMIC_RELEASE, "wavefront");
    __builtin_amdgcn_wave_barrier();
    __builtin_amdgcn_fence(__ATOMIC_ACQUIRE, "wavefront");
  }

#if W2A_S64_PRIO
  __builtin_amdgcn_s_setprio(0);
#endif
  if (AUTORESET && valid && restart_in) {
    a.reward[e] = 0.0f;
    a.done[e] = 0;
  } else if (valid && a.skip_finished && D1_FIN(h.b)) {
    a.reward[e] = 0.0f;
    a.done[e] = 1;
  } else if (valid) {
  float r;
  if (REWARD_GIVEN) {
    r = a.reward[e];
  } else {
    const float2 z = sw.z[lane];
    const float base = sigmoid_f32(z.x);
    const float eff = need_eff ? sigmoid_f32(z.y) : 0.0f;
    r = -(1000.0f / 152.0f) * base * (1.0f - eff);
    if (FIXES && (fx & W2A_FIX_PENALTY) && d.act == 1 && atb) r = -1.0f;
  }
  const uint32_t t2 = done ? t : t + 1;
  const uint32_t streak2 = done ? streak : (actual ? streak + 1 : 0);
  const float ret = __uint_as_float(h.c) + r;
  u3 h2;
  h2.a = pack_d0(t2, used2, streak2, actual, atb);
  h2.b = pack_d1(hist2, ndays, done ? 1u : 0u);
  h2.c = __float_as_uint(ret);
#if W2A_S64_SC1 & 2
  if (PACKED) st8_sc1(&a.st.pk_hot[e], v2u{pk_pack_hot(used2, streak2, hist2, done ? 1u : 0u), h2.c});
  else st12_sc1(&a.st.hot3[e], v3u{h2.a, h2.b, h2.c});
  if (!REWARD_GIVEN) st4_sc1(&a.reward[e], __float_as_uint(r));
  st1_sc1(&a.done[e], done ? 1u : 0u);
#else
  if (PACKED) a.st.pk_hot[e] = make_uint2(pk_pack_hot(used2, streak2, hist2, done ? 1u : 0u), h2.c);
  else a.st.hot3[e] = h2;
  if (!REWARD_GIVEN) a.reward[e] = r;
  a.done[e] = done ? 1 : 0;
#endif
  if (PACKED && lane == 0) a.st.pk_day[wave_env0 >> 6] = t2;
  if (done && a.last_return) a.last_return[e] = ret;
  if (st_bits) atomicOr(a.status, (int)st_bits);
  }
  if (AUTORESET) {
    const bool rs = valid && (a.next_step ? restart_in : done);
    const unsigned long long rs_mask = __ballot(rs);
    if (rs_mask) {
      uint2 ds = make_uint2(0xFFFFFFFFu, 0u);
      if (rs) {
        const uint4 cold = load_cold(a.st, e);
        const Episode ep = draw_episode(a.tb, a.rc, (uint64_t)(a.gid0 + e), cold.w + 1, (int32_t)cold.z);
        if (ep.bad) atomicOr(a.status, (int)W2A_ST_BAD_EPISODE);
        store_episode(a.st, e, make_uint4(ep.ep_row, ep.ep_w, (uint32_t)ep.sticky, cold.w + 1),
                      make_uint4(pack_d0(0, 0, 0, 0, 0), pack_d1(0, ep.ndays, 0), __float_as_uint(0.0f), (uint32_t)ep.budget));
        if (PACKED) {
          a.st.pk_hot[e] = make_uint2(pk_pack_hot(0u, 0u, 0u, 0u), __float_as_uint(0.0f));
          a.st.pk_c[e] = make_uint2(pk_budget16((uint32_t)ep.budget) | (W_COL(ep.ep_w) << 16),
                                    (ep.ep_row & 0x3FFFFFu) | (W_SAMPLE(ep.ep_w) << 22));
        }
        ds = make_uint2(ep.ep_row * (ROWF / 4), (uint32_t)ep.budget);
      }
      if (WRITE_OBS) {
        sw.desc[lane] = ds;
        __builtin_amdgcn_fence(__ATOMIC_RELEASE, "wavefront");
        __builtin_amdgcn_wave_barrier();
        __builtin_amdgcn_fence(__ATOMIC_ACQUIRE, "wavefront");
#pragma unroll 1
        for (int r = 0; r < S64_ENVS / 8; ++r) {
          if (!((rs_mask >> (r * 8)) & 0xFFull)) continue;
          const int j = r * 8 + g;
          const uint2 dj = sw.desc[j];
          if (dj.x != 0xFFFFFFFFu) {
            float4 v = a.tb.X[dj.x + p];
            if (p == RT_QUAD) v = make_float4(0.0f, 0.0f, (float)(int32_t)dj.y, 0.0f);
            if (FIXES && (fx & W2A_FIX_ALERTS_2WKS) && a.tb.slot_hist2w >= 0 && p == (a.tb.slot_hist2w >> 2))
              set_comp4(v, a.tb.slot_hist2w & 3, 0.0f);
            float *row = reinterpret_cast<float *>(a.obs) + (size_t)(wave_env0 + j) * n_obs;
            if (so.x >= 0) row[so.x] = v.x;
            if (so.y >= 0) row[so.y] = v.y;
            if (so.z >= 0) row[so.z] = v.z;
            if (so.w >= 0) row[so.w] = v.w;
          }
        }
      }
      if (PACKED && lane == 0) a.st.pk_day[wave_env0 >> 6] = 0u;
    }
  }
}

__device__ __forceinline__ void s64_load_packed(const StepArgs &a, uint32_t e, uint32_t day, u3 &h, u3 &c, int32_t &act) {
#if W2A_S64_NT_STATE & 4
  const v2u phv = __builtin_nontemporal_load(reinterpret_cast<const v2u *>(&a.st.pk_hot[e]));
  const v2u pcv = __builtin_nontemporal_load(reinterpret_cast<const v2u *>(&a.st.pk_c[e]));
  const uint2 ph = make_uint2(phv.x, phv.y), pc = make_uint2(pcv.x, pcv.y);
#else
  const uint2 ph = a.st.pk_hot[e];
  const uint2 pc = a.st.pk_c[e];
#endif
  h.a = pack_d0(day, PK_USED(ph.x), PK_STREAK(ph.x), PK_HIST(ph.x) & 1u, 0u);
  h.b = pack_d1(PK_HIST(ph.x), (uint32_t)a.uni_nd, PK_FIN(ph.x));
  h.c = ph.y;
  c.a = pc.x & 0xFFFFu;
  if (c.a == PK_BUDGET_ESCAPE) c.a = a.st.stepc[e].a;
  c.b = pc.y & 0x3FFFFFu;
  c.c = PACK_W(pc.x >> 16, pc.y >> 22);
  act = load_action(a, e);
}
__device__ __forceinline__ void s64_load_state(const StepArgs &a, uint32_t e, u3 &h, u3 &c, int32_t &act) {
#if W2A_S64_NT_STATE & 1
  const v3u hv = __builtin_nontemporal_load(reinterpret_cast<const v3u *>(&a.st.hot3[e]));
  h.a = hv.x; h.b = hv.y; h.c = hv.z;
#else
  h = a.st.hot3[e];
#endif
#if W2A_S64_NT_STATE & 2
  const v3u cv = __builtin_nontemporal_load(reinterpret_cast<const v3u *>(&a.st.stepc[e]));
  c.a = cv.x; c.b = cv.y; c.c = cv.z;
#else
  c = a.st.stepc[e];
#endif
  act = load_action(a, e);
}

template <bool WRITE_OBS, bool REWARD_GIVEN, bool PACKED = false, bool AUTORESET = false, bool FIXES = false>
__global__ __launch_bounds__(BLOCK, FIXES ? 3 : W2A_S64_MIN_WAVES) void k_step64(const StepArgs a) {
  __shared__ __attribute__((aligned(16))) S64WaveT<FIXES> s_w[S64_WAVES];
  const int tid = threadIdx.x;
  const int lane = tid & 63;
  const int wave = __builtin_amdgcn_readfirstlane(tid >> 6);
  S64WaveT<FIXES> &sw = s_w[wave];
  uint32_t lb = logical_block(blockIdx.x, gridDim.x >> 3);
  int wave_tile = wave;
#if W2A_S64_SERPENTINE
  if (a.walk_rev) {
    lb = logical_block_rev(blockIdx.x, gridDim.x >> 3);
    wave_tile = S64_WAVES - 1 - wave;
  }
#endif
  const int64_t wave_env0 = ((int64_t)lb * S64_WAVES + wave_tile) * (S64_ENVS * W2A_S64_TILES);
  if (wave_env0 >= a.n) return;
  uint32_t dayn = 0;
  if (PACKED) {
    dayn = a.st.pk_day[wave_env0 >> 6];
    if (dayn == W2A_PK_DAY_POISON) {
      if (lane == 0) atomicOr(a.status, (int)W2A_ST_STALE_GRAPH);
      return;
    }
  }
  u3 hn, cn;
  int32_t an;
  {
    const int64_t env = wave_env0 + lane;
    if (PACKED) s64_load_packed(a, (uint32_t)(env < a.n ? env : a.n - 1), dayn, hn, cn, an);
    else s64_load_state(a, (uint32_t)(env < a.n ? env : a.n - 1), hn, cn, an);
  }
  int4 so = make_int4(-1, -1, -1, -1);
  if (WRITE_OBS) so = reinterpret_cast<const int4 *>(a.slot_obs)[lane & 7];
#pragma unroll 1
  for (int i = 0; i < W2A_S64_TILES; ++i) {
    const int64_t env0 = wave_env0 + (int64_t)i * S64_ENVS;
    if (env0 >= a.n) break;
    const int64_t env = env0 + lane;
    const bool valid = env < a.n;
    const uint32_t e = (uint32_t)(valid ? env : (a.n - 1));
    const u3 h = hn, c = cn;
    const int32_t act = an;
    if (i + 1 < W2A_S64_TILES && env0 + S64_ENVS < a.n) {
      const int64_t en = env + S64_ENVS;
      if (PACKED) {
        dayn = a.st.pk_day[(env0 + S64_ENVS) >> 6];
        s64_load_packed(a, (uint32_t)(en < a.n ? en : a.n - 1), dayn == W2A_PK_DAY_POISON ? 0u : dayn, hn, cn, an);
      } else s64_load_state(a, (uint32_t)(en < a.n ? en : a.n - 1), hn, cn, an);
    }
    s64_tile<WRITE_OBS, REWARD_GIVEN, PACKED, AUTORESET, FIXES>(a, sw, lane, env0, valid, e, h, c, act, so);
    __builtin_amdgcn_fence(__ATOMIC_RELEASE, "wavefront");
    __builtin_amdgcn_wave_barrier();
    __builtin_amdgcn_fence(__ATOMIC_ACQUIRE, "wavefront");
  }
}

__global__ void k_pack_state(StateArrays st, int64_t n) {
  const int64_t i = (int64_t)blockIdx.x * blockDim.x + threadIdx.x;
  if (i >= n) return;
  const u3 h = st.hot3[i];
  const u3 c = st.stepc[i];
  st.pk_hot[i] = make_uint2(pk_pack_hot(D0_USED(h.a), D0_STREAK(h.a), D1_HIST(h.b), D1_FIN(h.b)), h.c);
  st.pk_c[i] = make_uint2(pk_budget16(c.a) | (W_COL(c.c) << 16), (c.b & 0x3FFFFFu) | (W_SAMPLE(c.c) << 22));
  if ((i & 63) == 0) st.pk_day[i >> 6] = D0_T(h.a);
}
__global__ void k_unpack_state(StateArrays st, int64_t n, int32_t n_days) {
  const int64_t i = (int64_t)blockIdx.x * blockDim.x + threadIdx.x;
  if (i >= n) return;
  const uint2 ph = st.pk_hot[i];
  const uint32_t t = st.pk_day[i >> 6];
  const uint32_t used = PK_USED(ph.x), hist = PK_HIST(ph.x), fin = PK_FIN(ph.x), last = hist & 1u;
  const uint32_t atb = ((t > 0 || fin) && (int32_t)(used - last) == (int32_t)st.stepc[i].a) ? 1u : 0u;
  u3 h;
  h.a = pack_d0(t, used, PK_STREAK(ph.x), last, atb);
  h.b = pack_d1(hist, (uint32_t)n_days, fin);
  h.c = ph.y;
  st.hot3[i] = h;
}
__global__ void k_poison_mirror(StateArrays st, int64_t n) {
  const int64_t i = (int64_t)blockIdx.x * blockDim.x + threadIdx.x;
  if (i < ((n + 63) >> 6)) st.pk_day[i] = W2A_PK_DAY_POISON;
}

#endif
```

### weather2alert_amd/csrc/w2a_step_dispatch.hip.h

```cpp
#ifndef W2A_STEP_DISPATCH_HIP_H
#define W2A_STEP_DISPATCH_HIP_H

int w2a_step(w2a_env *env, const void *actions, int action_dtype, float *obs, float *reward, uint8_t *done,
             float *last_return, int flags, void *stream) {
  if (!env || !actions || !reward || !done) return fail(W2A_ERR_ARG, "w2a_step: NULL argument");
  if (action_dtype < W2A_ACT_I32 || action_dtype > W2A_ACT_U8) return fail(W2A_ERR_ARG, "w2a_step: bad action_dtype");
  const bool no_obs = (flags & W2A_STEP_NO_OBS) != 0;
  const bool autoreset = (flags & W2A_STEP_AUTORESET) != 0;
  const bool given = (flags & W2A_STEP_REWARD_GIVEN) != 0;
  if (given && (autoreset || env->tb.fixes || (flags & W2A_STEP_CLASSIC)))
    return fail(W2A_ERR_ARG, "w2a_step: W2A_STEP_REWARD_GIVEN is served by the 64-envs-per-wave kernel only (no in-kernel "
                             "autoreset, no corrected-semantics flags)");
  if (!no_obs && !obs) return fail(W2A_ERR_ARG, "w2a_step: obs is NULL (pass W2A_STEP_NO_OBS for reward-only)");
  if (!no_obs && ((uintptr_t)obs & 15)) return fail(W2A_ERR_ARG, "w2a_step: obs must be 16-B aligned");
  if (autoreset && !env->has_autoreset) return fail(W2A_ERR_ARG, "w2a_step: W2A_STEP_AUTORESET needs w2a_set_autoreset first");
  StepArgs a;
  memset(&a, 0, sizeof(a));
  a.tb = env->tb; a.slot_obs = env->slot_obs; a.st = env->st;
  a.actions = actions; a.obs = obs; a.reward = reward; a.done = done; a.last_return = last_return;
  a.status = env->status; a.n = env->n; a.gid0 = env->gid0; a.rc = env->autoreset; a.act_dtype = action_dtype;
  a.skip_finished = (flags & W2A_STEP_SKIP_FINISHED) ? 1 : 0;
  a.next_step = (flags & W2A_STEP_NEXT_STEP) ? 1 : 0;
  if (a.next_step && !autoreset) return fail(W2A_ERR_ARG, "w2a_step: W2A_STEP_NEXT_STEP goes with W2A_STEP_AUTORESET");
  if (a.skip_finished && !given)
    return fail(W2A_ERR_ARG, "w2a_step: W2A_STEP_SKIP_FINISHED goes with W2A_STEP_REWARD_GIVEN (policy loops)");
  dim3 grid(grid_for(env->n)), block(BLOCK);
  hipStream_t s = (hipStream_t)stream;
  const bool capturing = stream_is_capturing(s);
  if (capturing && (flags & W2A_STEP_NO_CAPTURE))
    return fail(W2A_ERR_STATE, "w2a_step: the stream is recording a hipGraph, but this loop's episode boundaries are driven "
                               "from the host (W2A_STEP_NO_CAPTURE): a reset between two steps cannot be recorded. Let the "
                               "step kernel restart finished envs itself (W2A_STEP_AUTORESET; HeatAlertVecEnv(lockstep=False))");
  const bool wide = (given || (flags & W2A_STEP_WIDE) || env->n >= W2A_S64_MIN_ENVS) && !(flags & W2A_STEP_CLASSIC);
  HipDev dv{env, s};
  const W2aBook before = env->bk;
  const BkStepPlan plan = bk_step(env->bk, dv, wide, autoreset, given, (flags & W2A_STEP_UNPACKED) != 0, capturing);
  if (plan.kernel < 0)
    return fail(W2A_ERR_STATE, "w2a_step: this step runs on the canonical state words, which are not current (the state is "
                               "in its packed lock-step form), and a conversion cannot be recorded into a hipGraph; call "
                               "w2a_get_state before capturing -- or, on a handle with a recorded packed step, do not "
                               "record a step of another kind");
#define W2A_STEP_TRY(expr) \
  do { hipError_t _e = (expr); \
       if (_e != hipSuccess) { bk_step_rollback(env->bk, before, plan); if (!capturing) bk_end_call(env->bk, dv); \
                               return fail(W2A_ERR_HIP, #expr ": %s", hipGetErrorString(_e)); } } while (0)
  if (plan.kernel != W2A_BK_STEP_CLASSIC) {
    const int64_t per_wg = (int64_t)BLOCK * W2A_S64_TILES;
    const int64_t tiles = (env->n + per_wg - 1) / per_wg;
    dim3 grid64((unsigned)(((tiles + 7) / 8) * 8));
    a.walk_rev = env->s64_launches++ & 1u;
    if (plan.kernel == W2A_BK_STEP_PACKED) {
      a.uni_nd = plan.uni_nd;
      if (autoreset) {
        if (env->tb.fixes) {
          if (no_obs) hipLaunchKernelGGL((k_step64<false, false, true, true, true>), grid64, block, 0, s, a);
          else hipLaunchKernelGGL((k_step64<true, false, true, true, true>), grid64, block, 0, s, a);
        } else if (no_obs) hipLaunchKernelGGL((k_step64<false, false, true, true>), grid64, block, 0, s, a);
        else hipLaunchKernelGGL((k_step64<true, false, true, true>), grid64, block, 0, s, a);
      } else if (env->tb.fixes) {
        if (no_obs) hipLaunchKernelGGL((k_step64<false, false, true, false, true>), grid64, block, 0, s, a);
        else hipLaunchKernelGGL((k_step64<true, false, true, false, true>), grid64, block, 0, s, a);
      } else if (no_obs) hipLaunchKernelGGL((k_step64<false, false, true>), grid64, block, 0, s, a);
      else hipLaunchKernelGGL((k_step64<true, false, true>), grid64, block, 0, s, a);
      W2A_STEP_TRY(hipGetLastError());
      bk_end_call(env->bk, dv);
      return W2A_OK;
    }
    if (given) {
      if (no_obs) hipLaunchKernelGGL((k_step64<false, true>), grid64, block, 0, s, a);
      else hipLaunchKernelGGL((k_step64<true, true>), grid64, block, 0, s, a);
    } else if (env->tb.fixes) {
      if (autoreset) {
        if (no_obs) hipLaunchKernelGGL((k_step64<false, false, false, true, true>), grid64, block, 0, s, a);
        else hipLaunchKernelGGL((k_step64<true, false, false, true, true>), grid64, block, 0, s, a);
      } else {
        if (no_obs) hipLaunchKernelGGL((k_step64<false, false, false, false, true>), grid64, block, 0, s, a);
        else hipLaunchKernelGGL((k_step64<true, false, false, false, true>), grid64, block, 0, s, a);
      }
    } else if (autoreset) {
      if (no_obs) hipLaunchKernelGGL((k_step64<false, false, false, true>), grid64, block, 0, s, a);
      else hipLaunchKernelGGL((k_step64<true, false, false, true>), grid64, block, 0, s, a);
    } else {
      if (no_obs) hipLaunchKernelGGL((k_step64<false, false>), grid64, block, 0, s, a);
      else hipLaunchKernelGGL((k_step64<true, false>), grid64, block, 0, s, a);
    }
    W2A_STEP_TRY(hipGetLastError());
    if (!capturing) bk_end_call(env->bk, dv);
    return W2A_OK;
  }
#define W2A_LAUNCH(AR, OB) \
  do { if (env->tb.fixes) hipLaunchKernelGGL((k_step<AR, OB, true>), grid, block, 0, s, a); \
       else hipLaunchKernelGGL((k_step<AR, OB, false>), grid, block, 0, s, a); } while (0)
  if (autoreset) { if (no_obs) W2A_LAUNCH(true, false); else W2A_LAUNCH(true, true); }
  else { if (no_obs) W2A_LAUNCH(false, false); else W2A_LAUNCH(false, true); }
#undef W2A_LAUNCH
  W2A_STEP_TRY(hipGetLastError());
#undef W2A_STEP_TRY
  if (!capturing) bk_end_call(env->bk, dv);
  return W2A_OK;
}

#endif
```

### weather2alert_amd/env.py

```python
from __future__ import annotations

import ctypes as C
from typing import Literal

import numpy as np
import torch

from . import _ffi, policy as _policy, stats as _stats
from .info import _LazyInfo
from .options import KernelOptions
from .rng import numpy_parity_episode
from .spaces import Box, Discrete
from .tables import CompiledTables, DeviceTables, compile_from_files

_ACT_CODES = {torch.int32: _ffi.ACT_I32, torch.int64: _ffi.ACT_I64, torch.uint8: _ffi.ACT_U8,
              torch.bool: _ffi.ACT_U8}
_BUDGET_MODES = {"less_than": _ffi.BUDGET_LESS_THAN, "centered": _ffi.BUDGET_CENTERED}
_cur_device = getattr(torch._C, "_cuda_getDevice", torch.cuda.current_device)

try:
    from gymnasium.vector import VectorEnv as _VectorEnvBase
except ImportError:
    _VectorEnvBase = object
try:
    from gymnasium.vector import AutoresetMode as _AutoresetMode
except ImportError:
    _AutoresetMode = None


def _autoreset_metadata(mode: str):
    if _AutoresetMode is None:
        return mode
    return {"same_step": _AutoresetMode.SAME_STEP, "next_step": _AutoresetMode.NEXT_STEP,
            "disabled": _AutoresetMode.DISABLED}[mode]


class HeatAlertVecEnv(_VectorEnvBase):

    metadata = {"autoreset_mode": _autoreset_metadata("same_step")}
    spec = None
    render_mode = None
    closed = False

    def __init__(
        self,
        num_envs: int = 1,
        weights: str = "nn_full_medicare_all",
        years: list | None = None,
        fips_list: list | None = None,
        similar_climate_counties: bool = False,
        budget: int | None = None,
        data_dir: str | None = None,
        split: str = "65k",
        device: str | torch.device = "cuda:0",
        seed_mode: Literal["device", "numpy_parity"] = "device",
        autoreset: Literal["same_step", "next_step", "disabled"] = "same_step",
        tables: CompiledTables | DeviceTables | None = None,
        env_gid0: int = 0,
        episode_order: Literal["iid", "sorted"] = "iid",
        lockstep: bool | None = None,
        faithful: bool = True,
        fixes: set | list | None = None,
        reward_mode: Literal["sampled", "posterior_mean"] = "sampled",
        kernel: KernelOptions | None = None,
        pm_sync_group=None,
        **kernel_overrides,
    ):
        self.kernel = (kernel or KernelOptions()).with_overrides(**kernel_overrides)
        write_obs, step_kernel, pm_kernel = self.kernel.write_obs, self.kernel.step_kernel, self.kernel.pm_kernel
        rollout_order, rollout_mfma = self.kernel.rollout_order, self.kernel.rollout_mfma
        self._lib = _ffi.load()
        self.device = torch.device(device)
        if self.device.type != "cuda" or not torch.cuda.is_available():
            raise RuntimeError("HeatAlertVecEnv needs a ROCm GPU (device='cuda:N'); there is no CPU fallback")
        if self.device.index is None:
            self.device = torch.device("cuda", torch.cuda.current_device())
        if num_envs <= 0:
            raise ValueError("num_envs must be positive")
        if seed_mode not in ("device", "numpy_parity"):
            raise ValueError(f"seed_mode {seed_mode!r}")
        if autoreset not in ("same_step", "next_step", "disabled"):
            raise ValueError(f"autoreset {autoreset!r}")
        if autoreset == "next_step" and seed_mode != "device":
            raise ValueError("autoreset='next_step' needs seed_mode='device'")
        self.num_envs = int(num_envs)
        self.similar_climate_counties = bool(similar_climate_counties)
        self.seed_mode = seed_mode
        self.autoreset = autoreset
        self.metadata = {**type(self).metadata, "autoreset_mode": _autoreset_metadata(autoreset)}
        self.env_gid0 = int(env_gid0)
        self.write_obs = bool(write_obs)
        self._ctor_budget = budget
        if isinstance(tables, DeviceTables):
            if tables.device != self.device:
                raise ValueError(f"tables live on {tables.device}, the env on {self.device}")
            self.dtables = tables
        else:
            ct = tables if tables is not None else compile_from_files(data_dir, weights, split, years)
            self.dtables = DeviceTables(ct, self.device)
        reward_path = "gather"
        allf = set(_ffi.FIX_BITS) | {"budget"}
        self.fixes = set(allf) if (not faithful and fixes is None) else set(fixes or ())
        if self.fixes - allf:
            raise ValueError(f"unknown fixes {sorted(self.fixes - allf)}; choose from {sorted(allf)}")
        self.reward_path = reward_path
        self.step_kernel = step_kernel
        if reward_mode not in ("sampled", "posterior_mean"):
            raise ValueError(f"reward_mode {reward_mode!r}")
        if reward_mode == "posterior_mean" and (self.fixes or step_kernel == "classic"):
            raise ValueError("reward_mode='posterior_mean' needs faithful semantics and the 64-envs-per-wave step kernel")
        self.reward_mode = reward_mode
        self.pm_kernel = pm_kernel
        self.pm_kernel_choice = None if pm_kernel == "auto" else pm_kernel
        self.pm_kernel_timing_us: dict = {}
        self.pm_sync_group = pm_sync_group
        self.rollout_order = bool(rollout_order)
        self.rollout_mfma = bool(rollout_mfma)
        self._mfma_ws = None
        self.pm_rollout_kernel = True
        self.last_pm_rollout: str | None = None
        self._order_stale = True
        if episode_order not in ("iid", "sorted"):
            raise ValueError(f"episode_order {episode_order!r}")
        if episode_order == "sorted" and seed_mode != "device":
            raise ValueError("episode_order='sorted' needs seed_mode='device'")
        self.episode_order = episode_order
        ct = self.ct = self.dtables.ct
        self.fips_list = ct.fips_list
        self.valid_years = ct.years
        self.n_samples = ct.n_samples
        self.feature_names = ct.feature_names
        self._fips_pos = {f: i for i, f in enumerate(ct.fips_list)}
        self.single_observation_space = Box(-np.inf, np.inf, (ct.n_obs,), np.float32)
        self.single_action_space = Discrete(2)
        self.observation_space = Box(-np.inf, np.inf, (self.num_envs, ct.n_obs), np.float32)
        self.action_space = self.single_action_space

        n, dev = self.num_envs, self.device
        with torch.cuda.device(dev):
            nbytes = self._lib.w2a_state_bytes(n)
            self._state = torch.zeros(nbytes, dtype=torch.uint8, device=dev)
            self._status = torch.zeros(1, dtype=torch.int32, device=dev)
            self._obs = torch.zeros((n, ct.n_obs), dtype=torch.float32, device=dev)
            self._reward = torch.zeros(n, dtype=torch.float32, device=dev)
            self._done = torch.zeros(n, dtype=torch.uint8, device=dev)
            self._final_return = torch.zeros(n, dtype=torch.float32, device=dev)
            self._truncated = torch.zeros(n, dtype=torch.bool, device=dev)
            h = C.c_void_p()
            _ffi.check(self._lib.w2a_create(C.byref(self.dtables.struct), n, self.env_gid0, self._state.data_ptr(),
                                            nbytes, self._status.data_ptr(), C.byref(h)), "w2a_create")
        self._h = h
        bits = sum(_ffi.FIX_BITS[k] for k in self.fixes if k in _ffi.FIX_BITS)
        if bits:
            _ffi.check(self._lib.w2a_set_semantics(h, bits), "w2a_set_semantics")
        if reward_mode == "posterior_mean" and self.pm_kernel_choice is not None:
            _ffi.check(self._lib.w2a_set_posterior_kernel(h, _ffi.PM_KERNELS[self.pm_kernel_choice]),
                       "w2a_set_posterior_kernel")
        self._dev_index = self.device.index if self.device.index is not None else torch.cuda.current_device()
        self._obs_ptr = self._obs.data_ptr() if self.write_obs else None
        self._rew_ptr, self._done_ptr = self._reward.data_ptr(), self._done.data_ptr()
        self._fr_ptr = self._final_return.data_ptr()
        self._done_bool = self._done.view(torch.bool)
        self._sort_ws = None
        self._order_ws = None
        self._group_ws = None
        if reward_mode == "posterior_mean":
            with torch.cuda.device(dev):
                self._group_ws = torch.empty(self._lib.w2a_group_workspace_bytes(n, ct.S, ct.n_samples), dtype=torch.uint8,
                                             device=dev)
        nd = np.unique(ct.n_days)
        uniform = len(nd) == 1 and nd[0] > 0
        if episode_order == "sorted":
            if not uniform:
                raise ValueError("episode_order='sorted' needs one episode length for every (county, year)")
            if lockstep is False:
                raise ValueError("episode_order='sorted' implies lockstep")
            with torch.cuda.device(dev):
                self._sort_ws = torch.empty(self._lib.w2a_sort_workspace_bytes(n), dtype=torch.uint8, device=dev)
        if lockstep and not uniform:
            raise ValueError("lockstep=True needs one episode length for every (county, year)")
        self._episode_len = int(nd[0]) if uniform else 0
        self._lockstep = bool(uniform and self.seed_mode == "device" and lockstep is not False)
        self._steps_in_episode = 0
        self._pending_reset = False
        self._reset_cfg = None
        self._set_step_mode()
        self._w2a_step = self._lib.w2a_step
        self._raw_stream = getattr(torch._C, "_cuda_getCurrentRawStream", None)
        self._sticky = [budget] * n
        self._needs_reset = True
        self._obs_current = False
        self._last_opts: dict = {}
        self._np_random = None
        self._np_random_seed = None

    @property
    def unwrapped(self):
        return self

    @property
    def np_random(self) -> np.random.Generator:
        if self._np_random is None:
            self._np_random_seed = int(np.random.SeedSequence().entropy % (2**63))
            self._np_random = np.random.default_rng(self._np_random_seed)
        return self._np_random

    @np_random.setter
    def np_random(self, value: np.random.Generator):
        self._np_random, self._np_random_seed = value, -1

    @property
    def np_random_seed(self):
        self.np_random
        return self._np_random_seed

    def _set_step_mode(self):
        auto = self.autoreset in ("same_step", "next_step") and self.seed_mode == "device"
        self._dev_auto = auto and not self._lockstep
        self._host_auto = auto and self._lockstep and self.autoreset == "same_step"
        self._host_next = auto and self._lockstep and self.autoreset == "next_step"
        if not self._host_next:
            self._pending_reset = False
        if self.reward_mode == "posterior_mean" and self._dev_auto:
            raise ValueError("reward_mode='posterior_mean' cannot run with the in-kernel autoreset (batches that left "
                             "lock step); use autoreset='disabled' or whole-batch resets")
        self._pm = self.reward_mode == "posterior_mean"
        host_driven = self._host_auto or self._host_next or (self.autoreset == "same_step" and not self._dev_auto)
        self._step_flags = ((0 if self.write_obs else _ffi.STEP_NO_OBS) |
                            (_ffi.STEP_NO_CAPTURE if host_driven else 0) |
                            (_ffi.STEP_REWARD_GIVEN if self._pm else 0) |
                            (_ffi.STEP_CLASSIC if self.step_kernel == "classic" else 0) |
                            (_ffi.STEP_WIDE if self.step_kernel == "wide" else 0) |
                            (_ffi.STEP_UNPACKED if self.step_kernel == "unpacked" else 0) |
                            (_ffi.STEP_AUTORESET if self._dev_auto else 0) |
                            (_ffi.STEP_NEXT_STEP if self._dev_auto and self.autoreset == "next_step" else 0))

    @property
    def step_kernel_name(self) -> str:
        wide = self._pm or self.step_kernel == "wide" or (self.step_kernel in ("auto", "unpacked") and
                                                          self.num_envs >= _ffi.S64_MIN_ENVS)
        return "k_step64" if (wide and self.step_kernel != "classic") else "k_step"

    @property
    def last_step_kernel(self) -> str | None:
        return {0: "k_step", 1: "k_step64", 2: "k_step64<packed>"}.get(
            self._lib.w2a_query(self._h, _ffi.Q_LAST_STEP_KERNEL))

    @property
    def packed_state(self) -> bool:
        return bool(self._lib.w2a_query(self._h, _ffi.Q_PACKED_CURRENT)) and not bool(
            self._lib.w2a_query(self._h, _ffi.Q_CANONICAL_CURRENT))

    @property
    def last_rollout_kernel(self) -> str | None:
        return _ffi.ROLLOUT_KERNELS.get(self._lib.w2a_query(self._h, _ffi.Q_LAST_ROLLOUT_KERNEL))

    def _stream(self):
        if self._raw_stream is not None:
            return self._raw_stream(self._dev_index)
        return torch.cuda.current_stream(self.device).cuda_stream

    def close(self, **kwargs):
        if getattr(self, "_h", None):
            torch.cuda.synchronize(self.device)
            self._lib.w2a_destroy(self._h)
            self._h = None
        self.closed = True

    def __del__(self):
        try:
            self.close()
        except Exception:
            pass

    def check_status(self) -> int:
        out = C.c_int32(0)
        with torch.cuda.device(self.device):
            _ffi.check(self._lib.w2a_read_status(self._h, C.byref(out), self._stream()), "w2a_read_status")
        return self._raise_for_status(out.value)

    @property
    def status_word(self) -> torch.Tensor:
        return self._status

    @staticmethod
    def _raise_for_status(bits: int) -> int:
        if bits & _ffi.ST_BAD_EPISODE:
            raise KeyError("reset: an episode tuple is out of range or has no data "
                           "(reference: KeyError at env.py:127 / ValueError at env.py:121)")
        if bits & _ffi.ST_BAD_ACTION:
            raise ValueError("step: actions must be 0 or 1 (action_space = Discrete(2))")
        if bits & _ffi.ST_STALE_GRAPH:
            raise RuntimeError("a replayed hipGraph holds step() calls on the packed lock-step form of this env's state, "
                               "which could not be kept current (a masked reset or a restored checkpoint since the "
                               "capture took the batch out of lock step): those replayed steps did nothing. Reset the "
                               "whole batch (or capture again) before replaying (include/w2a.h, w2a_state_bytes)")
        return bits

    def state(self) -> dict[str, torch.Tensor]:
        return self._state_packed()[1]

    def _state_packed(self, fields=None):
        v = _ffi.StateView()
        names = _ffi.STATE_FIELDS if fields is None else [k for k in _ffi.STATE_FIELDS if k in fields]
        buf = torch.empty((len(names), self.num_envs), dtype=torch.int32, device=self.device)
        out = {}
        for i, k in enumerate(names):
            out[k] = buf[i].view(torch.float32) if k == "episode_return" else buf[i]
            setattr(v, k, buf[i].data_ptr())
        with torch.cuda.device(self.device):
            _ffi.check(self._lib.w2a_get_state(self._h, C.byref(v), self._stream()), "w2a_get_state")
        return buf, out

    def state_dict(self) -> dict:
        self.state()
        return {
            "state": self._state.clone(), "obs": self._obs.clone(), "final_return": self._final_return.clone(),
            "reward": self._reward.clone(), "done": self._done.clone(),
            "host": {"sticky": list(self._sticky), "steps_in_episode": self._steps_in_episode,
                     "lockstep": self._lockstep, "reset_cfg": self._reset_cfg, "last_opts": dict(self._last_opts),
                     "needs_reset": self._needs_reset, "pending_reset": self._pending_reset, "info_location": list(getattr(self, "_info_location", [])),
                     "num_envs": self.num_envs, "env_gid0": self.env_gid0,
                     "abi_version": _ffi.ABI_VERSION, "state_bytes": int(self._state.numel()),
                     "pm_kernel_choice": self.pm_kernel_choice},
        }

    def load_state_dict(self, sd: dict) -> None:
        h = sd["host"]
        if h["num_envs"] != self.num_envs or h["env_gid0"] != self.env_gid0:
            raise ValueError("state_dict belongs to a different env batch (num_envs / env_gid0 differ)")
        hdr = self._state[:256].clone()
        src = sd["state"]
        if src.numel() == self._state.numel():
            self._state.copy_(src)
        else:
            a256 = lambda x: (x + 255) & ~255
            canon = 256 + a256(16 * self.num_envs) + 2 * a256(12 * self.num_envs)
            if src.numel() < canon or self._state.numel() < canon:
                raise ValueError(f"state_dict['state'] holds {src.numel()} bytes (written by ABI {h.get('abi_version', '<= 17')}); "
                                 f"this build (ABI {_ffi.ABI_VERSION}) needs at least the {canon} canonical bytes of "
                                 f"{self.num_envs} envs: not a checkpoint of this env batch")
            self._state[:canon].copy_(src[:canon])
        self._state[:256].copy_(hdr)
        self._obs_current = False
        with torch.cuda.device(self.device):
            _ffi.check(self._lib.w2a_invalidate(self._h, self._stream()), "w2a_invalidate")
        self._obs.copy_(sd["obs"])
        self._final_return.copy_(sd["final_return"])
        self._reward.copy_(sd["reward"])
        self._done.copy_(sd["done"])
        self._sticky = list(h["sticky"])
        self._steps_in_episode, self._lockstep = h["steps_in_episode"], h["lockstep"]
        self._reset_cfg, self._last_opts, self._needs_reset = h["reset_cfg"], dict(h["last_opts"]), h["needs_reset"]
        if h["info_location"]:
            self._info_location = list(h["info_location"])
        self._set_step_mode()
        self._pending_reset = bool(h.get("pending_reset", False)) and self._host_next
        if self._reset_cfg is not None:
            with torch.cuda.device(self.device):
                _ffi.check(self._lib.w2a_set_autoreset(self._h, *self._reset_cfg), "w2a_set_autoreset")
        if self._pm and h.get("pm_kernel_choice") in _ffi.PM_KERNELS:
            self.pm_kernel_choice = h["pm_kernel_choice"]
            _ffi.check(self._lib.w2a_set_posterior_kernel(self._h, _ffi.PM_KERNELS[self.pm_kernel_choice]),
                       "w2a_set_posterior_kernel")
        self._regroup()

    def _opt(self, options, key, default):
        v = None if options is None else options.get(key)
        return default if v is None else v

    def reset(self, seed: int | list | None = None, options: dict | None = None):
        options = dict(options or {})
        if seed is not None and not isinstance(seed, (list, tuple, np.ndarray)):
            self._np_random, self._np_random_seed = np.random.default_rng(int(seed)), int(seed)
        mask = options.get("mask")
        mask_t = None
        if mask is not None:
            mask_t = torch.as_tensor(np.asarray(mask), dtype=torch.uint8, device=self.device)
        obs_ptr = self._obs.data_ptr() if self.write_obs else None
        self._last_opts = {k: v for k, v in options.items() if k not in ("mask", "episodes")}
        if self._lockstep and (mask is not None or "episodes" in options):
            if self.episode_order == "sorted":
                raise ValueError("episode_order='sorted' resets the whole batch with the device RNG only")
            self._lockstep = False
            self._set_step_mode()
        if "episodes" in options:
            self._reset_tuples(options["episodes"], mask_t, obs_ptr)
            if self.seed_mode == "device" and self.autoreset in ("same_step", "next_step"):
                self._reset_cfg = self._device_cfg(seed, self._last_opts)
                with torch.cuda.device(self.device):
                    _ffi.check(self._lib.w2a_set_autoreset(self._h, *self._reset_cfg), "w2a_set_autoreset")
        elif self.seed_mode == "numpy_parity":
            self._reset_numpy_parity(seed, options, mask, mask_t, obs_ptr)
        else:
            self._reset_device(seed, options, mask_t, obs_ptr)
        self._needs_reset = False
        if mask is None:
            self._obs_current = self.write_obs
        return self._obs, self._info()

    def _reset_tuples(self, ep: dict, mask_t, obs_ptr):
        ct, n = self.ct, self.num_envs
        arrs = {}
        for k in ("county_w", "year_i", "coef_col", "sample"):
# ... 1007 lines not shown
```

### weather2alert_amd/options.py

```python
from __future__ import annotations

from dataclasses import dataclass, fields, replace
from typing import Literal


@dataclass(frozen=True)
class KernelOptions:
    step_kernel: Literal["auto", "classic", "wide", "unpacked"] = "auto"
    write_obs: bool = True
    reward_path: Literal["gather", "auto", "table"] = "gather"
    rollout_order: bool = True
    rollout_mfma: bool = True
    pm_kernel: Literal["auto", "vector", "matrix", "matrix_i8"] = "matrix_i8"
    sorted_reset: Literal["fused", "relabel"] = "fused"

    def __post_init__(self):
        if self.step_kernel not in ("auto", "classic", "wide", "unpacked"):
            raise ValueError(f"step_kernel {self.step_kernel!r}")
        if self.reward_path == "table":
            raise ValueError("reward_path='table' (the precomputed logit table of round 1) was removed: it was slower "
                             "than the row-gather kernels at every batch size; use 'gather'")
        if self.reward_path not in ("gather", "auto"):
            raise ValueError(f"reward_path {self.reward_path!r}")
        if self.pm_kernel not in ("auto", "vector", "matrix", "matrix_i8"):
            raise ValueError(f"pm_kernel {self.pm_kernel!r}")
        if self.sorted_reset not in ("fused", "relabel"):
            raise ValueError(f"sorted_reset {self.sorted_reset!r}")

    @classmethod
    def names(cls) -> tuple:
        return tuple(f.name for f in fields(cls))

    def with_overrides(self, **kw) -> "KernelOptions":
        unknown = set(kw) - set(self.names())
        if unknown:
            raise TypeError(f"unexpected keyword argument(s) {sorted(unknown)}")
        return replace(self, **kw) if kw else self
```

Baseline: 30.54 billion.

## Pack episode row and weight index into one 32-bit word in packed step state

When the episode-row and coefficient-sample indices fit in 32 bits together, the packed step state stores them as one 4-byte word instead of an 8-byte pk_c pair. The budget is kept as an 8-bit remaining count in the hot word, with an escape to a side array. This cuts per-env state traffic in the packed k_step64 path, at the cost of extra branches and a spill array for large budgets. A wide fallback and a force-wide option are kept.

```diff
diff --git a/include/w2a.h b/include/w2a.h
--- a/include/w2a.h
+++ b/include/w2a.h
@@ -264,8 +264,11 @@
 enum { W2A_Q_LOCKSTEP = 6,
        W2A_Q_LOCKSTEP_DAY = 0, W2A_Q_PACKED_ELIGIBLE = 1, W2A_Q_PACKED_CURRENT = 2, W2A_Q_CANONICAL_CURRENT = 3,
        W2A_Q_LAST_ROLLOUT_KERNEL = 4 ,
-       W2A_Q_LAST_STEP_KERNEL = 5     };
+       W2A_Q_LAST_STEP_KERNEL = 5    ,
+       W2A_Q_EPISODE_WORD_BYTES = 7   };
 int w2a_query(w2a_env *env, int what);
+
+int w2a_set_episode_word(w2a_env *env, int force_wide);
 
 int w2a_invalidate(w2a_env *env, void *stream);
 
diff --git a/weather2alert_amd/_ffi.py b/weather2alert_amd/_ffi.py
--- a/weather2alert_amd/_ffi.py
+++ b/weather2alert_amd/_ffi.py
@@ -20,7 +20,7 @@
     "w2a_abi_version", "w2a_last_error", "w2a_state_bytes", "w2a_create", "w2a_destroy", "w2a_reset",
     "w2a_reset_device_rng", "w2a_set_autoreset", "w2a_step", "w2a_get_state", "w2a_read_status",
     "w2a_sort_workspace_bytes", "w2a_sort_episodes", "w2a_reset_device_rng_sorted", "w2a_observe", "w2a_rollout", "w2a_rollout_order_workspace_bytes", "w2a_rollout_order_attach", "w2a_rollout_order", "w2a_rollout_posterior_mean", "w2a_policy_actions", "w2a_set_semantics",
-    "w2a_group_workspace_bytes", "w2a_group_by_column", "w2a_posterior_mean_reward", "w2a_set_posterior_kernel", "w2a_invalidate", "w2a_query", "w2a_rollout_mfma_workspace_bytes", "w2a_rollout_mfma_prepare",
+    "w2a_group_workspace_bytes", "w2a_group_by_column", "w2a_posterior_mean_reward", "w2a_set_posterior_kernel", "w2a_set_episode_word", "w2a_invalidate", "w2a_query", "w2a_rollout_mfma_workspace_bytes", "w2a_rollout_mfma_prepare",
     "w2a_rollout_linear", "w2a_rollout_mlp", "w2a_rollout_linear_record", "w2a_rollout_mlp_record",
     "w2a_posterior_returns", "w2a_hindsight_workspace_bytes", "w2a_hindsight_optimum",
     "w2a_policy_gradient_workspace_bytes", "w2a_policy_gradient_linear",
@@ -41,6 +41,7 @@
     "w2a_q_gradient_mlp_workspace_bytes", "w2a_q_gradient_mlp",
 ]
 Q_LOCKSTEP_DAY, Q_PACKED_ELIGIBLE, Q_PACKED_CURRENT, Q_CANONICAL_CURRENT, Q_LAST_ROLLOUT_KERNEL, Q_LAST_STEP_KERNEL, Q_LOCKSTEP = 0, 1, 2, 3, 4, 5, 6
+Q_EPISODE_WORD_BYTES = 7
 ROLLOUT_KERNELS = {0: "k_rollout", 1: "k_rollout64", 2: "k_rollout_mfma", 3: "k_rollout_linear", 4: "k_rollout_mlp"}
 PM_KERNELS = {"vector": 0, "matrix": 1, "matrix_i8": 2}
 POLICY_KINDS = {"never": 0, "always": 1, "bernoulli": 2, "threshold": 3, "table": 4}
@@ -156,6 +157,8 @@
     lib.w2a_posterior_mean_reward.argtypes = [vp, vp, C.c_int, vp, vp]
     lib.w2a_set_posterior_kernel.restype = C.c_int
     lib.w2a_set_posterior_kernel.argtypes = [vp, C.c_int]
+    lib.w2a_set_episode_word.restype = C.c_int
+    lib.w2a_set_episode_word.argtypes = [vp, C.c_int]
     lib.w2a_rollout_mfma_workspace_bytes.restype = C.c_size_t
     lib.w2a_rollout_mfma_workspace_bytes.argtypes = [i64, i64, i32, i32]
     lib.w2a_rollout_mfma_prepare.restype = C.c_int
diff --git a/weather2alert_amd/build.py b/weather2alert_amd/build.py
--- a/weather2alert_amd/build.py
+++ b/weather2alert_amd/build.py
@@ -52,7 +52,8 @@
     return any(os.path.getmtime(d) > m for d in _dep_files())
 
 
-STEP_SOURCES = ("w2a_common.hip.h", "w2a_step.hip.h", "w2a_step64.hip.h", "w2a_step_dispatch.hip.h", "w2a_bookkeeping.h")
+STEP_SOURCES = ("w2a_common.hip.h", "w2a_step.hip.h", "w2a_step64.hip.h", "w2a_step_dispatch.hip.h", "w2a_bookkeeping.h",
+                "w2a_episode_word.h")
 
 
 def source_sha(files: tuple = STEP_SOURCES) -> str:
diff --git a/weather2alert_amd/csrc/w2a_common.hip.h b/weather2alert_amd/csrc/w2a_common.hip.h
--- a/weather2alert_amd/csrc/w2a_common.hip.h
+++ b/weather2alert_amd/csrc/w2a_common.hip.h
@@ -2,6 +2,7 @@
 #define W2A_COMMON_HIP_H
 
 #include "w2a_bookkeeping.h"
+#include "w2a_episode_word.h"
 
 #ifndef LANES
 #define LANES 4
@@ -52,9 +53,21 @@
   uint2 *pk_c;
   uint32_t *pk_day;
 };
+#define SAMPLE_BITS 12
+#define PACK_W(coef_col, sample) (((uint32_t)(coef_col) << SAMPLE_BITS) | (uint32_t)(sample))
+#define W_COL(y) ((y) >> SAMPLE_BITS)
+#define W_SAMPLE(y) ((y) & ((1u << SAMPLE_BITS) - 1u))
 #define W2A_PK_DAY_POISON 0xFFFFFFFFu
 #define PK_BUDGET_ESCAPE 0xFFFFu
 __device__ __forceinline__ uint32_t pk_budget16(uint32_t budget) { return budget < PK_BUDGET_ESCAPE ? budget : PK_BUDGET_ESCAPE; }
+#define PK_REM_ESCAPE 255u
+__device__ __forceinline__ uint32_t pk_rem8(int32_t remaining) {
+  return (uint32_t)remaining < PK_REM_ESCAPE ? (uint32_t)remaining : PK_REM_ESCAPE;
+}
+__device__ __forceinline__ uint32_t *pk_rem_of(const StateArrays &s, int64_t n) { return reinterpret_cast<uint32_t *>(s.pk_c) + n; }
+__device__ __forceinline__ uint32_t pk_narrow_word(uint32_t ep_row, uint32_t ep_w, uint32_t n_samples, int32_t kw) {
+  return (W_COL(ep_w) * n_samples + W_SAMPLE(ep_w)) | (ep_row << kw);
+}
 #define PK_USED(w) ((w) & 255u)
 #define PK_STREAK(w) (((w) >> 8) & 255u)
 #define PK_HIST(w) (((w) >> 16) & 0x3FFFu)
@@ -120,10 +133,6 @@
     if (idx == 4 * q + 3) x[q].w = v;
   }
 }
-#define SAMPLE_BITS 12
-#define PACK_W(coef_col, sample) (((uint32_t)(coef_col) << SAMPLE_BITS) | (uint32_t)(sample))
-#define W_COL(y) ((y) >> SAMPLE_BITS)
-#define W_SAMPLE(y) ((y) & ((1u << SAMPLE_BITS) - 1u))
 
 struct ResetCfg {
   uint64_t seed;
@@ -169,6 +178,7 @@
   int pm_kernel;
   int w_tail_used;
   uint32_t s64_launches;
+  EpisodeWord ew;
 };
 
 static thread_local char g_err[512] = "";
diff --git a/weather2alert_amd/csrc/w2a_episode_word.h b/weather2alert_amd/csrc/w2a_episode_word.h
--- /dev/null
+++ b/weather2alert_amd/csrc/w2a_episode_word.h
@@ -0,0 +1,25 @@
+#ifndef W2A_EPISODE_WORD_H
+#define W2A_EPISODE_WORD_H
+
+#include <stdint.h>
+
+static inline int ew_bits(uint64_t v) {
+  int b = 0;
+  while (v) { ++b; v >>= 1; }
+  return b;
+}
+
+struct EpisodeWord {
+  int narrow;
+  int kw, kx;
+};
+
+static inline EpisodeWord ew_choose(int32_t S, int32_t n_samples, int32_t S_w, int32_t Y, bool force_wide) {
+  EpisodeWord w;
+  w.kw = ew_bits((uint64_t)S * (uint64_t)n_samples - 1u);
+  w.kx = ew_bits((uint64_t)S_w * (uint64_t)Y - 1u);
+  w.narrow = (!force_wide && w.kw + w.kx <= 32 && w.kw < 32) ? 1 : 0;
+  return w;
+}
+
+#endif
diff --git a/weather2alert_amd/csrc/w2a_kernels.hip b/weather2alert_amd/csrc/w2a_kernels.hip
--- a/weather2alert_amd/csrc/w2a_kernels.hip
+++ b/weather2alert_amd/csrc/w2a_kernels.hip
@@ -117,10 +117,12 @@
   w2a_env *env;
   hipStream_t s;
   void pack_state() {
-    hipLaunchKernelGGL(k_pack_state, dim3((unsigned)((env->n + 255) / 256)), dim3(256), 0, s, env->st, env->n);
+    hipLaunchKernelGGL(k_pack_state, dim3((unsigned)((env->n + 255) / 256)), dim3(256), 0, s, env->st, env->n,
+                       env->ew.narrow ? env->ew.kw : -1, env->tb.n_samples);
   }
   void unpack_state(int32_t n_days) {
-    hipLaunchKernelGGL(k_unpack_state, dim3((unsigned)((env->n + 255) / 256)), dim3(256), 0, s, env->st, env->n, n_days);
+    hipLaunchKernelGGL(k_unpack_state, dim3((unsigned)((env->n + 255) / 256)), dim3(256), 0, s, env->st, env->n, n_days,
+                       env->ew.narrow ? env->ew.kw : -1);
   }
   void poison_mirror() {
     const int64_t tiles = (env->n + 63) / 64;
@@ -216,6 +218,7 @@
   h->st.pk_c = reinterpret_cast<uint2 *>((char *)h->st.pk_hot + align256(8 * (size_t)num_envs));
   h->st.pk_day = reinterpret_cast<uint32_t *>((char *)h->st.pk_c + align256(8 * (size_t)num_envs));
   bk_init(h->bk, t->T <= 255 && t->S < 65536 && t->n_samples <= 1024 && (int64_t)t->S_w * t->Y < (1 << 22), -1);
+  h->ew = ew_choose(t->S, t->n_samples, t->S_w, t->Y, false);
   h->status = status;
   h->has_autoreset = 0;
   h->perm = nullptr;
@@ -581,6 +584,14 @@
   return W2A_OK;
 }
 
+int w2a_set_episode_word(w2a_env *env, int force_wide) {
+  if (!env) return fail(W2A_ERR_ARG, "w2a_set_episode_word: NULL handle");
+  if (env->bk.pk_valid || env->bk.graph_packed)
+    return fail(W2A_ERR_STATE, "w2a_set_episode_word: the packed form of the state is in use; call it right after w2a_create");
+  env->ew = ew_choose(env->tb.S, env->tb.n_samples, env->tb.S_w, env->tb.Y, force_wide != 0);
+  return W2A_OK;
+}
+
 int w2a_observe(w2a_env *env, float *obs, void *stream) {
   if (!env || !obs) return fail(W2A_ERR_ARG, "w2a_observe: NULL argument");
   ResetArgs a;
@@ -1033,6 +1044,7 @@
     case W2A_Q_CANONICAL_CURRENT: return env->bk.canon_valid;
     case W2A_Q_LAST_ROLLOUT_KERNEL: return env->bk.last_rollout_kernel;
     case W2A_Q_LAST_STEP_KERNEL: return env->bk.last_step_kernel;
+    case W2A_Q_EPISODE_WORD_BYTES: return env->ew.narrow ? 4 : 8;
     default: return fail(W2A_ERR_ARG, "w2a_query: unknown item");
   }
 }
diff --git a/weather2alert_amd/csrc/w2a_step.hip.h b/weather2alert_amd/csrc/w2a_step.hip.h
--- a/weather2alert_amd/csrc/w2a_step.hip.h
+++ b/weather2alert_amd/csrc/w2a_step.hip.h
@@ -19,6 +19,7 @@
   int32_t skip_finished;
   int32_t next_step;
   uint32_t walk_rev;
+  int32_t pk_kw;
 };
 
 #ifndef W2A_MIN_WAVES
diff --git a/weather2alert_amd/csrc/w2a_step64.hip.h b/weather2alert_amd/csrc/w2a_step64.hip.h
--- a/weather2alert_amd/csrc/w2a_step64.hip.h
+++ b/weather2alert_amd/csrc/w2a_step64.hip.h
@@ -97,7 +97,7 @@
   return 8u * per_xcd - 1u - b;
 #endif
 }
-template <bool WRITE_OBS, bool REWARD_GIVEN, bool PACKED, bool AUTORESET = false, bool FIXES = false>
+template <bool WRITE_OBS, bool REWARD_GIVEN, bool PACKED, bool AUTORESET = false, bool FIXES = false, bool NARROW = false>
 __device__ __forceinline__ void s64_tile(const StepArgs &a, S64WaveT<FIXES> &sw, const int lane, const int64_t wave_env0,
                                          const bool valid, const uint32_t e, const u3 h, const u3 c, const int32_t act,
                                          const int4 so) {
@@ -107,6 +107,9 @@
   const int32_t budget = d.budget;
   const bool done = d.done;
   const bool restart_in = AUTORESET && a.next_step && D1_FIN(h.b);
+  const uint32_t pk0 = NARROW ? pk_rem8(budget - (int32_t)used2) : used2;
+  if (NARROW && (uint32_t)budget >= PK_REM_ESCAPE && valid && !restart_in && !(a.skip_finished && D1_FIN(h.b)))
+    pk_rem_of(a.st, a.n)[e] = (uint32_t)(budget - (int32_t)used2);
   const uint32_t fx = FIXES ? a.tb.fixes : 0u;
   const bool fix_obs = FIXES && WRITE_OBS && (fx & W2A_FIX_OBS);
   uint32_t need_eff = actual;
@@ -114,7 +117,7 @@
     need_eff = (a.tb.gate_bits[t * (uint32_t)a.tb.gate_words + (c.b >> 5)] >> (c.b & 31u)) & 1u;
   {
     const uint32_t day_row = t * (uint32_t)(a.tb.S_w * a.tb.Y) + c.b;
-    const uint32_t wrow = W_COL(c.c) * (uint32_t)a.tb.n_samples + W_SAMPLE(c.c);
+    const uint32_t wrow = NARROW ? c.c : W_COL(c.c) * (uint32_t)a.tb.n_samples + W_SAMPLE(c.c);
     sw.desc[lane] = make_uint2((day_row * (ROWF / 4)) | ((fix_obs && !done) ? 0x80000000u : 0u),
                                (wrow * (2 * ROWF / 4)) | (need_eff << 31));
     sw.rt[lane] = runtime_fields(d, (fx & W2A_FIX_LAG) != 0u);
@@ -271,12 +274,12 @@
   h2.b = pack_d1(hist2, ndays, done ? 1u : 0u);
   h2.c = __float_as_uint(ret);
 #if W2A_S64_SC1 & 2
-  if (PACKED) st8_sc1(&a.st.pk_hot[e], v2u{pk_pack_hot(used2, streak2, hist2, done ? 1u : 0u), h2.c});
+  if (PACKED) st8_sc1(&a.st.pk_hot[e], v2u{pk_pack_hot(pk0, streak2, hist2, done ? 1u : 0u), h2.c});
   else st12_sc1(&a.st.hot3[e], v3u{h2.a, h2.b, h2.c});
   if (!REWARD_GIVEN) st4_sc1(&a.reward[e], __float_as_uint(r));
   st1_sc1(&a.done[e], done ? 1u : 0u);
 #else
-  if (PACKED) a.st.pk_hot[e] = make_uint2(pk_pack_hot(used2, streak2, hist2, done ? 1u : 0u), h2.c);
+  if (PACKED) a.st.pk_hot[e] = make_uint2(pk_pack_hot(pk0, streak2, hist2, done ? 1u : 0u), h2.c);
   else a.st.hot3[e] = h2;
   if (!REWARD_GIVEN) a.reward[e] = r;
   a.done[e] = done ? 1 : 0;
@@ -296,7 +299,11 @@
         if (ep.bad) atomicOr(a.status, (int)W2A_ST_BAD_EPISODE);
         store_episode(a.st, e, make_uint4(ep.ep_row, ep.ep_w, (uint32_t)ep.sticky, cold.w + 1),
                       make_uint4(pack_d0(0, 0, 0, 0, 0), pack_d1(0, ep.ndays, 0), __float_as_uint(0.0f), (uint32_t)ep.budget));
-        if (PACKED) {
+        if (PACKED && NARROW) {
+          a.st.pk_hot[e] = make_uint2(pk_pack_hot(pk_rem8(ep.budget), 0u, 0u, 0u), __float_as_uint(0.0f));
+          reinterpret_cast<uint32_t *>(a.st.pk_c)[e] = pk_narrow_word(ep.ep_row, ep.ep_w, (uint32_t)a.tb.n_samples, a.pk_kw);
+          pk_rem_of(a.st, a.n)[e] = (uint32_t)ep.budget;
+        } else if (PACKED) {
           a.st.pk_hot[e] = make_uint2(pk_pack_hot(0u, 0u, 0u, 0u), __float_as_uint(0.0f));
           a.st.pk_c[e] = make_uint2(pk_budget16((uint32_t)ep.budget) | (W_COL(ep.ep_w) << 16),
                                     (ep.ep_row & 0x3FFFFFu) | (W_SAMPLE(ep.ep_w) << 22));
@@ -331,7 +338,29 @@
   }
 }
 
+template <bool NARROW>
 __device__ __forceinline__ void s64_load_packed(const StepArgs &a, uint32_t e, uint32_t day, u3 &h, u3 &c, int32_t &act) {
+  if (NARROW) {
+    const uint32_t *ew = reinterpret_cast<const uint32_t *>(a.st.pk_c);
+#if W2A_S64_NT_STATE & 4
+    const v2u phv = __builtin_nontemporal_load(reinterpret_cast<const v2u *>(&a.st.pk_hot[e]));
+    const uint2 ph = make_uint2(phv.x, phv.y);
+    const uint32_t w = __builtin_nontemporal_load(&ew[e]);
+#else
+    const uint2 ph = a.st.pk_hot[e];
+    const uint32_t w = ew[e];
+#endif
+    const uint32_t used = 0u;
+    c.a = PK_USED(ph.x);
+    if (c.a == PK_REM_ESCAPE) c.a = pk_rem_of(a.st, a.n)[e];
+    h.a = pack_d0(day, used, PK_STREAK(ph.x), PK_HIST(ph.x) & 1u, 0u);
+    h.b = pack_d1(PK_HIST(ph.x), (uint32_t)a.uni_nd, PK_FIN(ph.x));
+    h.c = ph.y;
+    c.b = w >> a.pk_kw;
+    c.c = w & ((1u << a.pk_kw) - 1u);
+    act = load_action(a, e);
+    return;
+  }
 #if W2A_S64_NT_STATE & 4
   const v2u phv = __builtin_nontemporal_load(reinterpret_cast<const v2u *>(&a.st.pk_hot[e]));
   const v2u pcv = __builtin_nontemporal_load(reinterpret_cast<const v2u *>(&a.st.pk_c[e]));
@@ -365,7 +394,7 @@
   act = load_action(a, e);
 }
 
-template <bool WRITE_OBS, bool REWARD_GIVEN, bool PACKED = false, bool AUTORESET = false, bool FIXES = false>
+template <bool WRITE_OBS, bool REWARD_GIVEN, bool PACKED = false, bool AUTORESET = false, bool FIXES = false, bool NARROW = false>
 __global__ __launch_bounds__(BLOCK, FIXES ? 3 : W2A_S64_MIN_WAVES) void k_step64(const StepArgs a) {
   __shared__ __attribute__((aligned(16))) S64WaveT<FIXES> s_w[S64_WAVES];
   const int tid = threadIdx.x;
@@ -394,7 +423,7 @@
   int32_t an;
   {
     const int64_t env = wave_env0 + lane;
-    if (PACKED) s64_load_packed(a, (uint32_t)(env < a.n ? env : a.n - 1), dayn, hn, cn, an);
+    if (PACKED) s64_load_packed<NARROW>(a, (uint32_t)(env < a.n ? env : a.n - 1), dayn, hn, cn, an);
     else s64_load_state(a, (uint32_t)(env < a.n ? env : a.n - 1), hn, cn, an);
   }
   int4 so = make_int4(-1, -1, -1, -1);
@@ -412,31 +441,40 @@
       const int64_t en = env + S64_ENVS;
       if (PACKED) {
         dayn = a.st.pk_day[(env0 + S64_ENVS) >> 6];
-        s64_load_packed(a, (uint32_t)(en < a.n ? en : a.n - 1), dayn == W2A_PK_DAY_POISON ? 0u : dayn, hn, cn, an);
+        s64_load_packed<NARROW>(a, (uint32_t)(en < a.n ? en : a.n - 1), dayn == W2A_PK_DAY_POISON ? 0u : dayn, hn, cn, an);
       } else s64_load_state(a, (uint32_t)(en < a.n ? en : a.n - 1), hn, cn, an);
     }
-    s64_tile<WRITE_OBS, REWARD_GIVEN, PACKED, AUTORESET, FIXES>(a, sw, lane, env0, valid, e, h, c, act, so);
+    s64_tile<WRITE_OBS, REWARD_GIVEN, PACKED, AUTORESET, FIXES, PACKED && NARROW>(a, sw, lane, env0, valid, e, h, c, act, so);
     __builtin_amdgcn_fence(__ATOMIC_RELEASE, "wavefront");
     __builtin_amdgcn_wave_barrier();
     __builtin_amdgcn_fence(__ATOMIC_ACQUIRE, "wavefront");
   }
 }
 
-__global__ void k_pack_state(StateArrays st, int64_t n) {
+__global__ void k_pack_state(StateArrays st, int64_t n, int32_t pk_kw, int32_t n_samples) {
   const int64_t i = (int64_t)blockIdx.x * blockDim.x + threadIdx.x;
   if (i >= n) return;
   const u3 h = st.hot3[i];
   const u3 c = st.stepc[i];
-  st.pk_hot[i] = make_uint2(pk_pack_hot(D0_USED(h.a), D0_STREAK(h.a), D1_HIST(h.b), D1_FIN(h.b)), h.c);
-  st.pk_c[i] = make_uint2(pk_budget16(c.a) | (W_COL(c.c) << 16), (c.b & 0x3FFFFFu) | (W_SAMPLE(c.c) << 22));
+  if (pk_kw >= 0) {
+    const int32_t rem = (int32_t)c.a - (int32_t)D0_USED(h.a);
+    st.pk_hot[i] = make_uint2(pk_pack_hot(pk_rem8(rem), D0_STREAK(h.a), D1_HIST(h.b), D1_FIN(h.b)), h.c);
+    reinterpret_cast<uint32_t *>(st.pk_c)[i] = pk_narrow_word(c.b, c.c, (uint32_t)n_samples, pk_kw);
+    pk_rem_of(st, n)[i] = (uint32_t)rem;
+  } else {
+    st.pk_hot[i] = make_uint2(pk_pack_hot(D0_USED(h.a), D0_STREAK(h.a), D1_HIST(h.b), D1_FIN(h.b)), h.c);
+    st.pk_c[i] = make_uint2(pk_budget16(c.a) | (W_COL(c.c) << 16), (c.b & 0x3FFFFFu) | (W_SAMPLE(c.c) << 22));
+  }
   if ((i & 63) == 0) st.pk_day[i >> 6] = D0_T(h.a);
 }
-__global__ void k_unpack_state(StateArrays st, int64_t n, int32_t n_days) {
+__global__ void k_unpack_state(StateArrays st, int64_t n, int32_t n_days, int32_t pk_kw) {
   const int64_t i = (int64_t)blockIdx.x * blockDim.x + threadIdx.x;
   if (i >= n) return;
   const uint2 ph = st.pk_hot[i];
   const uint32_t t = st.pk_day[i >> 6];
-  const uint32_t used = PK_USED(ph.x), hist = PK_HIST(ph.x), fin = PK_FIN(ph.x), last = hist & 1u;
+  const uint32_t hist = PK_HIST(ph.x), fin = PK_FIN(ph.x), last = hist & 1u;
+  uint32_t used = PK_USED(ph.x);
+  if (pk_kw >= 0) used = (uint32_t)((int32_t)st.stepc[i].a - (int32_t)(used == PK_REM_ESCAPE ? pk_rem_of(st, n)[i] : used));
   const uint32_t atb = ((t > 0 || fin) && (int32_t)(used - last) == (int32_t)st.stepc[i].a) ? 1u : 0u;
   u3 h;
   h.a = pack_d0(t, used, PK_STREAK(ph.x), last, atb);
diff --git a/weather2alert_amd/csrc/w2a_step_dispatch.hip.h b/weather2alert_amd/csrc/w2a_step_dispatch.hip.h
--- a/weather2alert_amd/csrc/w2a_step_dispatch.hip.h
+++ b/weather2alert_amd/csrc/w2a_step_dispatch.hip.h
@@ -49,19 +49,27 @@
     const int64_t tiles = (env->n + per_wg - 1) / per_wg;
     dim3 grid64((unsigned)(((tiles + 7) / 8) * 8));
     a.walk_rev = env->s64_launches++ & 1u;
+    a.pk_kw = -1;
     if (plan.kernel == W2A_BK_STEP_PACKED) {
       a.uni_nd = plan.uni_nd;
-      if (autoreset) {
-        if (env->tb.fixes) {
-          if (no_obs) hipLaunchKernelGGL((k_step64<false, false, true, true, true>), grid64, block, 0, s, a);
-          else hipLaunchKernelGGL((k_step64<true, false, true, true, true>), grid64, block, 0, s, a);
-        } else if (no_obs) hipLaunchKernelGGL((k_step64<false, false, true, true>), grid64, block, 0, s, a);
-        else hipLaunchKernelGGL((k_step64<true, false, true, true>), grid64, block, 0, s, a);
-      } else if (env->tb.fixes) {
-        if (no_obs) hipLaunchKernelGGL((k_step64<false, false, true, false, true>), grid64, block, 0, s, a);
-        else hipLaunchKernelGGL((k_step64<true, false, true, false, true>), grid64, block, 0, s, a);
-      } else if (no_obs) hipLaunchKernelGGL((k_step64<false, false, true>), grid64, block, 0, s, a);
-      else hipLaunchKernelGGL((k_step64<true, false, true>), grid64, block, 0, s, a);
+      a.pk_kw = env->ew.narrow ? env->ew.kw : -1;
+#define W2A_LAUNCH_PK(NW)                                                                                                \
+      do {                                                                                                               \
+        if (autoreset) {   \
+          if (env->tb.fixes) {                                                                                           \
+            if (no_obs) hipLaunchKernelGGL((k_step64<false, false, true, true, true, NW>), grid64, block, 0, s, a);      \
+            else hipLaunchKernelGGL((k_step64<true, false, true, true, true, NW>), grid64, block, 0, s, a);              \
+          } else if (no_obs) hipLaunchKernelGGL((k_step64<false, false, true, true, false, NW>), grid64, block, 0, s, a); \
+          else hipLaunchKernelGGL((k_step64<true, false, true, true, false, NW>), grid64, block, 0, s, a);               \
+        } else if (env->tb.fixes) {   \
+          if (no_obs) hipLaunchKernelGGL((k_step64<false, false, true, false, true, NW>), grid64, block, 0, s, a);       \
+          else hipLaunchKernelGGL((k_step64<true, false, true, false, true, NW>), grid64, block, 0, s, a);               \
+        } else if (no_obs) hipLaunchKernelGGL((k_step64<false, false, true, false, false, NW>), grid64, block, 0, s, a); \
+        else hipLaunchKernelGGL((k_step64<true, false, true, false, false, NW>), grid64, block, 0, s, a);                \
+      } while (0)
+      if (env->ew.narrow) W2A_LAUNCH_PK(true);
+      else W2A_LAUNCH_PK(false);
+#undef W2A_LAUNCH_PK
       W2A_STEP_TRY(hipGetLastError());
       bk_end_call(env->bk, dv);
       return W2A_OK;
diff --git a/weather2alert_amd/env.py b/weather2alert_amd/env.py
--- a/weather2alert_amd/env.py
+++ b/weather2alert_amd/env.py
@@ -156,6 +156,8 @@
         if reward_mode == "posterior_mean" and self.pm_kernel_choice is not None:
             _ffi.check(self._lib.w2a_set_posterior_kernel(h, _ffi.PM_KERNELS[self.pm_kernel_choice]),
                        "w2a_set_posterior_kernel")
+        if self.kernel.force_wide_episode_word:
+            _ffi.check(self._lib.w2a_set_episode_word(h, 1), "w2a_set_episode_word")
         self._dev_index = self.device.index if self.device.index is not None else torch.cuda.current_device()
         self._obs_ptr = self._obs.data_ptr() if self.write_obs else None
         self._rew_ptr, self._done_ptr = self._reward.data_ptr(), self._done.data_ptr()
@@ -230,14 +232,14 @@
                             (_ffi.STEP_NO_CAPTURE if host_driven else 0) |
                             (_ffi.STEP_REWARD_GIVEN if self._pm else 0) |
                             (_ffi.STEP_CLASSIC if self.step_kernel == "classic" else 0) |
-                            (_ffi.STEP_WIDE if self.step_kernel == "wide" else 0) |
-                            (_ffi.STEP_UNPACKED if self.step_kernel == "unpacked" else 0) |
+                            (_ffi.STEP_WIDE if self.step_kernel in ("wide", "wide_unpacked") else 0) |
+                            (_ffi.STEP_UNPACKED if self.step_kernel in ("unpacked", "wide_unpacked") else 0) |
                             (_ffi.STEP_AUTORESET if self._dev_auto else 0) |
                             (_ffi.STEP_NEXT_STEP if self._dev_auto and self.autoreset == "next_step" else 0))
 
     @property
     def step_kernel_name(self) -> str:
-        wide = self._pm or self.step_kernel == "wide" or (self.step_kernel in ("auto", "unpacked") and
+        wide = self._pm or self.step_kernel in ("wide", "wide_unpacked") or (self.step_kernel in ("auto", "unpacked") and
                                                           self.num_envs >= _ffi.S64_MIN_ENVS)
         return "k_step64" if (wide and self.step_kernel != "classic") else "k_step"
 
@@ -250,6 +252,10 @@
     def packed_state(self) -> bool:
         return bool(self._lib.w2a_query(self._h, _ffi.Q_PACKED_CURRENT)) and not bool(
             self._lib.w2a_query(self._h, _ffi.Q_CANONICAL_CURRENT))
+
+    @property
+    def episode_word_bytes(self) -> int:
+        return int(self._lib.w2a_query(self._h, _ffi.Q_EPISODE_WORD_BYTES))
 
     @property
     def last_rollout_kernel(self) -> str | None:
diff --git a/weather2alert_amd/options.py b/weather2alert_amd/options.py
--- a/weather2alert_amd/options.py
+++ b/weather2alert_amd/options.py
@@ -6,16 +6,17 @@
 
 @dataclass(frozen=True)
 class KernelOptions:
-    step_kernel: Literal["auto", "classic", "wide", "unpacked"] = "auto"
+    step_kernel: Literal["auto", "classic", "wide", "unpacked", "wide_unpacked"] = "auto"
     write_obs: bool = True
     reward_path: Literal["gather", "auto", "table"] = "gather"
     rollout_order: bool = True
     rollout_mfma: bool = True
     pm_kernel: Literal["auto", "vector", "matrix", "matrix_i8"] = "matrix_i8"
     sorted_reset: Literal["fused", "relabel"] = "fused"
+    force_wide_episode_word: bool = False
 
     def __post_init__(self):
-        if self.step_kernel not in ("auto", "classic", "wide", "unpacked"):
+        if self.step_kernel not in ("auto", "classic", "wide", "unpacked", "wide_unpacked"):
             raise ValueError(f"step_kernel {self.step_kernel!r}")
         if self.reward_path == "table":
             raise ValueError("reward_path='table' (the precomputed logit table of round 1) was removed: it was slower "
```

After: 31.03 billion, median of 6. +1.6%, better.
